# pauxy-qmc/pauxy

Measured on AMD Instinct MI355X. Metric: walker_steps_per_sec, higher is better.
Workload: dtype f64; 1 GPU; generic Cholesky AFQMC: Nbasis=100, Nchol=500, RHF trial 25+25 electrons, 256 walkers/GPU, dt=0.005, reortho/10, comb/5, energy/10 (BASELINE configs[2]); walkers_total=256, rng=device-philox, population_control=device comb (one rank)

## Files before the change

### pauxy_amd/csrc/afq_api.hip

```cpp
#include <algorithm>
#include <cmath>
#include <complex>
#include <cstdio>
#include <cstdlib>
#include <cstring>
#include "afq_internal.h"

namespace {

template <class T> int dev_alloc(afq_handle *h, T **p, size_t n) {
    if (*p) { hipFree(*p); *p = nullptr; }
    if (n == 0) return AFQ_OK;
    hipError_t e = hipMalloc((void **)p, n * sizeof(T));
    if (e != hipSuccess) { h->err = std::string("hipMalloc: ") + hipGetErrorString(e); return AFQ_ENOMEM; }
    return AFQ_OK;
}

template <class T> int dev_upload(afq_handle *h, T **p, const void *src, size_t n) {
    int rc = dev_alloc(h, p, n);
    if (rc) return rc;
    if (n) AFQ_HIP(h, hipMemcpy(*p, src, n * sizeof(T), hipMemcpyHostToDevice));
    return AFQ_OK;
}

// ... 573 lines not shown
            for (double &v : pt) v = -v;
            if ((rc = dev_upload(h, &h->msd_psicT_neg, pt.data(), kkp * M))) return rc;
        }
    }
    return AFQ_OK;
}

int afq_set_propagator(afq_handle *h, const double *BH1, const double *mf_shift, double dt, int exp_order,
                       int flags) {
    if (h) { h->greens_valid = false; h->gsum_only = false; }
    if (!h || !BH1 || !mf_shift || dt <= 0 || exp_order < 0) return AFQ_EINVAL;
    if (!h->kind) AFQ_FAIL(h, AFQ_ESTATE, "set the system before the propagator");
    hipSetDevice(h->device);
    int rc;
    if ((rc = dev_upload(h, &h->BH1, BH1, (size_t)2 * h->M * h->M))) return rc;
    h->bh1_real = true;
    h->bh1_same = memcmp(BH1, BH1 + (size_t)2 * h->M * h->M, sizeof(double) * 2 * h->M * h->M) == 0;
    for (size_t i = 0, n = (size_t)2 * h->M * h->M; i < n && h->bh1_real; ++i) h->bh1_real = BH1[2 * i + 1] == 0.0;
    if ((rc = dev_upload(h, &h->mf_shift, mf_shift, (size_t)h->K))) return rc;
    if (h->kind == AFQ_SYS_UEG && (rc = k_ueg_fast_propagator(h, BH1))) return rc;
    h->dt = dt; h->sqrt_dt = std::pow(dt, 0.5); h->exp_order = exp_order;
    if (flags & AFQ_PROP_FREE_PROJECTION) flags &= ~AFQ_PROP_FORCE_BIAS;
    const int old_nv = h->nv; const bool old_diag = h->vhs_diag;
    h->flags = flags;
    h->vhs_diag = h->kind == AFQ_SYS_HUBBARD;
    h->nv = (h->kind == AFQ_SYS_HUBBARD && (flags & AFQ_PROP_HUBBARD_SPIN)) ? 2 : 1;
    h->have_prop = true;
    if (h->nw && (old_nv != h->nv || old_diag != h->vhs_diag || !h->vhs)) {
        const size_t per = h->vhs_diag ? (size_t)2 * h->nv * h->M : (size_t)h->nv * h->M * h->M;
        if ((rc = dev_alloc(h, &h->vhs, per * h->nw))) return rc;
    }
    return AFQ_OK;
}

int afq_walkers_alloc(afq_handle *h, int nw) {
    if (h) { h->greens_valid = false; h->gsum_only = false; }
    if (!h || nw <= 0) return AFQ_EINVAL;
    if (!h->kind) AFQ_FAIL(h, AFQ_ESTATE, "set the system before allocating walkers");
    hipSetDevice(h->device);
    free_walkers(h);
    const size_t per = (size_t)h->M * h->nt, K = h->K, n = nw;
    int rc;
#define A_(ptr, cnt) if ((rc = dev_alloc(h, &(ptr), (cnt)))) return rc;
    A_(h->phi, per * n) A_(h->phi_t, per * n) A_(h->phi_t2, per * n)
    A_(h->weight, n) A_(h->unscaled, n) A_(h->detR, n) A_(h->log_detR, n)
    A_(h->ot, n) A_(h->ehyb, n) A_(h->phase, n) A_(h->eloc, n)
    A_(h->ghalf_all, per * n * h->ndet) A_(h->ovlp_old, n) A_(h->ovlp_new, n)
    h->ghalf = h->ghalf_all + (size_t)h->cur_det * n * per;
    if (h->ndet > 1) { A_(h->detd, n * h->ndet) A_(h->detd_a, n * h->ndet) A_(h->detw, n * h->ndet) A_(h->energy_all, 3 * n * h->ndet) }
    A_(h->xi, K * n) A_(h->xbar, K * n) A_(h->xs, K * n) A_(h->cmf, n) A_(h->cfb, n)
    A_(h->energy, 3 * n) A_(h->alive, n) A_(h->parent_ix, n)
    h->fb_split = 1;
    if (h->kind == AFQ_SYS_GENERIC) {
        const long tiles = (long)((nw + 31) / 32) * ((h->K + 31) / 32) * 2;
        int sp = (int)std::max(1L, std::min(8L, 1024 / std::max(1L, tiles)));
        if (nw > 32) {
            const long wgt = (long)((nw + 63) / 64) * ((h->K + 63) / 64) * 2;
            sp = (int)std::max(1L, std::min(16L, (512 + wgt - 1) / wgt));
        }
        if (h->rchol_same && h->rchol_real && h->ndet == 1 && h->na == h->nb && nw > 32 && sp > 1) sp = (sp + 1) / 2;
        const int nmax = std::max(h->na, h->nb) * h->M;
        while (sp > 1 && nmax / sp < 64) --sp;
        h->fb_split = sp;
        A_(h->vbias_all, (size_t)2 * sp * n * K * h->ndet)
        h->vbias = h->vbias_all + (size_t)h->cur_det * 2 * sp * n * K;
    } else if (h->kind == AFQ_SYS_UEG) {
        A_(h->vbias_all, n * K)
        h->vbias = h->vbias_all;
    }
    if (h->kind == AFQ_SYS_UEG) A_(h->G, (size_t)2 * h->M * h->M * n)
    {
        const size_t pv = h->kind == AFQ_SYS_HUBBARD ? (size_t)4 * h->M : (size_t)h->M * h->M;
        A_(h->vhs, pv * n)
    }
#undef A_
    AFQ_HIP(h, hipMalloc(&h->pack_tmp, std::max((size_t)nw * 2 * sizeof(int), (size_t)4096)));
    h->nw = nw;
    h->cap_frac = 0.0; h->cap_total = -1.0;
    {
        double sc0[AFQ_NSCAL] = {0};
        sc0[0] = (double)nw * k_comm_size(h);
        AFQ_HIP(h, hipMemcpy(h->scal, sc0, sizeof(sc0), hipMemcpyHostToDevice));
    }
    std::vector<double> one(nw, 1.0), zero2(2 * (size_t)nw, 0.0), one2(2 * (size_t)nw, 0.0);
    for (int i = 0; i < nw; ++i) one2[2 * i] = 1.0;
    AFQ_HIP(h, hipMemcpy(h->weight, one.data(), sizeof(double) * nw, hipMemcpyHostToDevice));
    AFQ_HIP(h, hipMemcpy(h->unscaled, one.data(), sizeof(double) * nw, hipMemcpyHostToDevice));
    AFQ_HIP(h, hipMemcpy(h->detR, one.data(), sizeof(double) * nw, hipMemcpyHostToDevice));
    AFQ_HIP(h, hipMemset(h->log_detR, 0, sizeof(double) * nw));
    AFQ_HIP(h, hipMemcpy(h->ot, one2.data(), sizeof(cplx) * nw, hipMemcpyHostToDevice));
    AFQ_HIP(h, hipMemcpy(h->phase, one2.data(), sizeof(cplx) * nw, hipMemcpyHostToDevice));
    AFQ_HIP(h, hipMemcpy(h->ehyb, zero2.data(), sizeof(cplx) * nw, hipMemcpyHostToDevice));
    AFQ_HIP(h, hipMemcpy(h->eloc, zero2.data(), sizeof(cplx) * nw, hipMemcpyHostToDevice));
    AFQ_HIP(h, hipMemset(h->phi, 0, sizeof(cplx) * per * n));
    AFQ_HIP(h, hipMemset(h->ghalf, 0, sizeof(cplx) * per * n));
    AFQ_HIP(h, hipMemset(h->energy, 0, sizeof(cplx) * 3 * n));
    AFQ_HIP(h, hipMemset(h->xi, 0, sizeof(double) * K * n));
    return AFQ_OK;
}

static int field_info(afq_handle *h, int field, void **base, size_t *bytes) {
    const size_t per = (size_t)h->M * h->nt;
    switch (field) {
    case AFQ_F_PHI: *base = h->phi; *bytes = per * sizeof(cplx); break;
    case AFQ_F_WEIGHT: *base = h->weight; *bytes = sizeof(double); break;
    case AFQ_F_UNSCALED_WEIGHT: *base = h->unscaled; *bytes = sizeof(double); break;
    case AFQ_F_OT: *base = h->ot; *bytes = sizeof(cplx); break;
    case AFQ_F_HYBRID_ENERGY: *base = h->ehyb; *bytes = sizeof(cplx); break;
    case AFQ_F_PHASE: *base = h->phase; *bytes = sizeof(cplx); break;
    case AFQ_F_DETR: *base = h->detR; *bytes = sizeof(double); break;
    case AFQ_F_ELOC: *base = h->eloc; *bytes = sizeof(cplx); break;
    case AFQ_F_GHALF: *base = h->ghalf; *bytes = per * sizeof(cplx); break;
    case AFQ_F_G: *base = h->G; *bytes = (size_t)2 * h->M * h->M * sizeof(cplx); break;
    case AFQ_F_XBAR: *base = h->xbar; *bytes = (size_t)h->K * sizeof(cplx); break;
    case AFQ_F_XSHIFTED: *base = h->xs; *bytes = (size_t)h->K * sizeof(cplx); break;
    case AFQ_F_ENERGY: *base = h->energy; *bytes = 3 * sizeof(cplx); break;
    case AFQ_F_LOG_DETR: *base = h->log_detR; *bytes = sizeof(double); break;
    default: AFQ_FAIL(h, AFQ_EINVAL, "unknown walker field");
    }
    if (!*base) AFQ_FAIL(h, AFQ_ESTATE, "walker field not allocated (afq_walkers_alloc / afq_greens first)");
    return AFQ_OK;
}

static int ensure_spin_ghalf(afq_handle *h);

int afq_walkers_set(afq_handle *h, int field, const void *host, int first, int count) {
    if (h && (field == AFQ_F_PHI || field == AFQ_F_GHALF)) { h->greens_valid = false; h->gsum_only = false; ++h->ghalf_version; }
    if (!h || !host) return AFQ_EINVAL;
    if (!h->nw) AFQ_FAIL(h, AFQ_ESTATE, "no walkers allocated");
    if (first < 0 || count < 0 || first + count > h->nw) AFQ_FAIL(h, AFQ_EINVAL, "walker range out of bounds");
    hipSetDevice(h->device);
    void *base; size_t bytes;
    int rc = field_info(h, field, &base, &bytes);
    if (rc) return rc;
    AFQ_HIP(h, hipMemcpyAsync((char *)base + bytes * first, host, bytes * count, hipMemcpyHostToDevice, h->stream));
    AFQ_HIP(h, hipStreamSynchronize(h->stream));
    return AFQ_OK;
}

int afq_walkers_get(afq_handle *h, int field, void *host, int first, int count) {
    if (!h || !host) return AFQ_EINVAL;
    if (!h->nw) AFQ_FAIL(h, AFQ_ESTATE, "no walkers allocated");
    if (first < 0 || count < 0 || first + count > h->nw) AFQ_FAIL(h, AFQ_EINVAL, "walker range out of bounds");
    hipSetDevice(h->device);
    void *base; size_t bytes;
    int rc = field_info(h, field, &base, &bytes);
    if (rc) return rc;
    if (field == AFQ_F_GHALF && (rc = ensure_spin_ghalf(h))) return rc;
    AFQ_HIP(h, hipMemcpyAsync(host, (char *)base + bytes * first, bytes * count, hipMemcpyDeviceToHost, h->stream));
    AFQ_HIP(h, hipStreamSynchronize(h->stream));
    return AFQ_OK;
}

int afq_walkers_device_ptr(afq_handle *h, int field, void **dev_ptr, int64_t *bytes_per_walker) {
    if (!h || !dev_ptr) return AFQ_EINVAL;
    void *base; size_t bytes;
    int rc = field_info(h, field, &base, &bytes);
    if (rc) return rc;
    if (field == AFQ_F_GHALF && h->gsum_only) {
        hipSetDevice(h->device);
        if ((rc = ensure_spin_ghalf(h))) return rc;
    }
    h->greens_valid = false; h->gsum_only = false; h->greens_cache = false;
    *dev_ptr = base;
    if (bytes_per_walker) *bytes_per_walker = (int64_t)bytes;
    return AFQ_OK;
}

static int greens_any(afq_handle *h, cplx *det_out, bool with_ghalf);

static int need_ready(afq_handle *h, bool prop) {
    if (!h->kind || !h->have_trial || !h->nw) AFQ_FAIL(h, AFQ_ESTATE, "system, trial and walkers must be set");
    if (prop && !h->have_prop) AFQ_FAIL(h, AFQ_ESTATE, "propagator not set");
    if (h->prop_pending) AFQ_FAIL(h, AFQ_ESTATE, "a step is half done: afq_propagate_finish first");
    hipSetDevice(h->device);
    return AFQ_OK;
}

static int ensure_spin_ghalf(afq_handle *h) {
    if (!h->gsum_only) return AFQ_OK;
    h->gsum_only = false;
    const int rc = greens_any(h, h->ovlp_new, true);
    h->greens_valid = rc == AFQ_OK;
    return rc;
}

static int ensure_G(afq_handle *h) {
    if (!h->G) {
        int rc = dev_alloc(h, &h->G, (size_t)2 * h->M * h->M * h->nw);
        if (rc) return rc;
    }
    return AFQ_OK;
}

static int copy_out(afq_handle *h, void *host, const void *dev, size_t bytes) {
    if (!host) return AFQ_OK;
    AFQ_HIP(h, hipMemcpyAsync(host, dev, bytes, hipMemcpyDeviceToHost, h->stream));
    AFQ_HIP(h, hipStreamSynchronize(h->stream));
    return AFQ_OK;
}

int afq_greens(afq_handle *h, int want_G, double *ovlp_out) {
    AFQ_API(h, "afq_greens");
    if (h) { h->greens_valid = false; h->gsum_only = false; }
    if (!h) return AFQ_EINVAL;
    int rc = need_ready(h, false);
    if (rc) return rc;
    {
        PhaseTimer t(h, T_GREENS);
        if ((rc = greens_any(h, h->ovlp_old, true))) return rc;
        if (want_G || h->kind == AFQ_SYS_UEG) {
            if ((rc = ensure_G(h))) return rc;
            if ((rc = k_full_G(h))) return rc;
        }
    }
    return copy_out(h, ovlp_out, h->ovlp_old, sizeof(cplx) * h->nw);
}

int afq_inverse_overlap(afq_handle *h, double *oinv_out, double *ovlp_out) {
    if (h) { h->greens_valid = false; h->gsum_only = false; }
    if (!h || !oinv_out) return AFQ_EINVAL;
    int rc = need_ready(h, false);
    if (rc) return rc;
    if (h->ndet > 1) AFQ_FAIL(h, AFQ_EUNSUPPORTED, "inverse overlaps: single-determinant trials");
    const size_t nmax = h->na > h->nb ? h->na : h->nb, n = (size_t)h->nw * 2 * nmax * nmax;
    cplx *tmp = nullptr;
    if ((rc = dev_alloc(h, &tmp, n))) return rc;
    AFQ_HIP(h, hipMemsetAsync(tmp, 0, sizeof(cplx) * n, h->stream));
    if ((rc = k_alive(h))) { dev_free(tmp); return rc; }
    std::vector<int> ones(h->nw, 1);
    AFQ_HIP(h, hipMemcpyAsync(h->alive, ones.data(), sizeof(int) * h->nw, hipMemcpyHostToDevice, h->stream));
    rc = k_inverse_overlap(h, tmp, h->ovlp_new);
    if (!rc) rc = copy_out(h, oinv_out, tmp, sizeof(cplx) * n);
    if (!rc && ovlp_out) rc = copy_out(h, ovlp_out, h->ovlp_new, sizeof(cplx) * h->nw);
    dev_free(tmp);
    if (!rc) rc = k_alive(h);
    return rc;
}

int afq_calc_overlap(afq_handle *h, double *ovlp_out) {
    AFQ_API(h, "afq_calc_overlap");
    if (h) { h->greens_valid = false; h->gsum_only = false; }
    if (!h) return AFQ_EINVAL;
    int rc = need_ready(h, false);
    if (rc) return rc;
    {
        PhaseTimer t(h, T_OVLP);
        if ((rc = greens_any(h, h->ovlp_new, false))) return rc;
    }
    return copy_out(h, ovlp_out, h->ovlp_new, sizeof(cplx) * h->nw);
}

static int greens_any(afq_handle *h, cplx *det_out, bool with_ghalf) {
    int rc;
    if (h->ndet <= 1) return with_ghalf ? k_greens(h, det_out) : k_overlap(h, det_out);
    for (int d = 0; d < h->ndet; ++d) {
        select_det(h, d);
        cplx *dd = h->detd + (size_t)d * h->nw;
        h->det_a_out = with_ghalf ? h->detd_a + (size_t)d * h->nw : nullptr;
        rc = with_ghalf ? k_greens(h, dd) : k_overlap(h, dd);
        h->det_a_out = nullptr;
        if (rc) { select_det(h, 0); return rc; }
    }
    select_det(h, 0);
    return k_msd_combine(h, det_out, with_ghalf);
}

static int force_bias(afq_handle *h, bool with_xbar = true) {
    int rc;
    if (h->flags & AFQ_PROP_FORCE_BIAS) {
        if (h->kind == AFQ_SYS_GENERIC) {
            h->msd_fb_gbar = false;
            if (k_msd_gbar_wanted(h) && !(h->msd_fb_mode == 0 && k_msd_vbias_current(h))) {
                if ((rc = k_force_bias_msd_gbar(h))) return rc;
                h->msd_fb_gbar = true;
            } else {
                for (int d = 0; d < h->ndet; ++d) {
                    select_det(h, d);
                    if ((rc = k_force_bias_generic(h))) { select_det(h, 0); return rc; }
                }
                select_det(h, 0);
            }
        }
        else if (h->kind == AFQ_SYS_UEG) { if ((rc = k_vbias_ueg(h))) return rc; }
    }
    return with_xbar ? k_xbar(h) : AFQ_OK;
}

static int build_vhs(afq_handle *h) {
    if (h->kind == AFQ_SYS_GENERIC) return k_vhs_generic(h);
    if (h->kind == AFQ_SYS_HUBBARD) return k_vhs_hubbard(h);
    return k_vhs_ueg(h);
}

static int local_energy(afq_handle *h);
static int local_energy_dets(afq_handle *h);

static int apply_exp(afq_handle *h, const cplx *vhs) {
    if (h->vhs_diag) return k_apply_exponential_diag(h, vhs);
    return k_apply_exponential(h, vhs);
}

int afq_propagate(afq_handle *h, const double *xi, double eshift_re, double eshift_im) {
    const int rc = afq_propagate_begin(h, xi);
    return rc ? rc : afq_propagate_finish(h, eshift_re, eshift_im);
}

int afq_propagate_begin(afq_handle *h, const double *xi) {
    AFQ_API(h, "afq_propagate");
    if (!h) return AFQ_EINVAL;
    int rc = need_ready(h, true);
    if (rc) return rc;
    if (h->hirsch) AFQ_FAIL(h, AFQ_ESTATE, "discrete Hirsch propagator set: use afq_propagate_hirsch");
    const bool hubbard_fused = h->vhs_diag;
    const bool hubbard_fused_fields = hubbard_fused && h->K == h->M;
    if (xi) {
        if ((rc = k_alive(h))) return rc;
        AFQ_HIP(h, hipMemcpyAsync(h->xi, xi, sizeof(double) * (size_t)h->nw * h->K, hipMemcpyHostToDevice, h->stream));
    } else if (k_prop_fused_supported(h) || k_ueg_fast_supported(h) || hubbard_fused_fields) {
        h->rng_inline = true;
        h->rng_inline_counter = h->rng_counter++;
    } else {
        if ((rc = k_rng_normal(h))) return rc;
    }
    const bool fp = (h->flags & AFQ_PROP_FREE_PROJECTION) != 0;
    if (!fp || (h->flags & AFQ_PROP_FORCE_BIAS)) {
        PhaseTimer t(h, T_GREENS);
        const bool sum_ok = h->gsum_only && (h->flags & AFQ_PROP_HYBRID) && !h->rdm_on &&
                            (h->kind == AFQ_SYS_GENERIC ||
                             (h->kind == AFQ_SYS_HUBBARD && h->gdiag && h->gdiag_version == h->ghalf_version));
        if (h->greens_valid || sum_ok) std::swap(h->ovlp_old, h->ovlp_new);
        else if ((rc = greens_any(h, h->ovlp_old, true))) return rc;
        h->greens_valid = false; h->gsum_only = false;
        const bool le = !fp && !(h->flags & AFQ_PROP_HYBRID);
        if ((h->kind == AFQ_SYS_UEG && ((h->flags & AFQ_PROP_FORCE_BIAS) || le) && !k_ueg_fast_supported(h)) ||
            (h->rdm_on && h->ndet == 1)) {
            if ((rc = ensure_G(h))) return rc;
            if ((rc = k_full_G(h))) return rc;
        }
        if (le) {
            PhaseTimer te(h, T_ENERGY);
            if (h->ndet > 1) { if ((rc = local_energy_dets(h))) return rc; }
            else if ((rc = local_energy(h))) return rc;
        }
    }
    if (k_ueg_fast_supported(h)) {
        { PhaseTimer t(h, T_EXP); if ((rc = k_ueg_step(h))) return rc; }
        h->prop_pending = true;
        return AFQ_OK;
    }
    if (hubbard_fused) {
        cplx *fac = h->vhs + (size_t)h->nw * h->nv * h->M;
        const bool fields_make_factors = hubbard_fused_fields;
        {
            PhaseTimer t(h, T_FB);
            if ((rc = force_bias(h, false))) return rc;
            if ((rc = k_xbar_fields(h, fields_make_factors ? fac : nullptr))) return rc;
        }
        if (!fields_make_factors) {
            { PhaseTimer t(h, T_VHS); if ((rc = build_vhs(h))) return rc; }
            { PhaseTimer t(h, T_EXP); if ((rc = k_exp_diag_factors(h, h->vhs, fac))) return rc; }
        }
        if (h->rng_inline) AFQ_FAIL(h, AFQ_ESTATE, "internal: the inline field draw of this step was not consumed by the field kernel");
        { PhaseTimer t(h, T_ONEBODY); if ((rc = k_onebody(h, fac))) return rc; }
        { PhaseTimer t(h, T_ONEBODY); if ((rc = k_onebody(h))) return rc; }
        h->prop_pending = true;
        return AFQ_OK;
    }
    const bool fused = k_prop_fused_supported(h);
    h->closed_large = !fused && h->kind == AFQ_SYS_GENERIC && h->nv == 1 && h->bh1_same && h->na == h->nb && h->na > 0 &&
                      h->M > 128 && h->nt > 32 && h->nw >= 64;
    struct ClosedLargeOff { afq_handle *h; ~ClosedLargeOff() { h->closed_large = false; } } closed_large_off{h};
    if (h->closed_large && (rc = k_closed_flags(h))) return rc;
    if (!fused) { PhaseTimer t(h, T_ONEBODY); if ((rc = k_onebody(h))) return rc; }
    {
        PhaseTimer t(h, T_FB);
        if ((rc = force_bias(h, false))) return rc;
        if ((rc = k_xbar_fields(h))) return rc;
    }
    h->vhs_upper = fused && h->hs_sym;
    { PhaseTimer t(h, T_VHS); rc = build_vhs(h); }
    if (rc) { h->vhs_upper = false; return rc; }
    if (fused) {
        PhaseTimer t(h, T_EXP);
        rc = k_prop_fused(h);
        h->vhs_upper = false;
        if (rc) return rc;
    } else {
        { PhaseTimer t(h, T_EXP); if ((rc = apply_exp(h, h->vhs))) return rc; }
        { PhaseTimer t(h, T_ONEBODY); if ((rc = k_onebody(h))) return rc; }
        if (h->closed_large && (rc = k_closed_copy_beta(h))) return rc;
    }
    h->prop_pending = true;
    return AFQ_OK;
}

int afq_propagate_finish(afq_handle *h, double eshift_re, double eshift_im) {
    AFQ_API(h, "afq_propagate");
    if (!h) return AFQ_EINVAL;
    if (!h->prop_pending) AFQ_FAIL(h, AFQ_ESTATE, "afq_propagate_finish without afq_propagate_begin");
    hipSetDevice(h->device);
    h->prop_pending = false;
    int rc;
    const bool fp = (h->flags & AFQ_PROP_FREE_PROJECTION) != 0;
    {
        PhaseTimer t(h, T_OVLP);
        const bool le_msd = h->ndet > 1 && !fp && !(h->flags & AFQ_PROP_HYBRID);
        h->fuse_weight_done = false;
        h->fuse_weight_req = h->ndet == 1 && !le_msd;
        h->fuse_eshift = cmake(eshift_re, eshift_im);
        if (h->greens_cache && !fp) {
            const bool fb_sum = h->kind == AFQ_SYS_GENERIC && k_fb_use_sum(h);
            const bool fb_diag = h->kind == AFQ_SYS_HUBBARD && !h->hirsch && h->psicT && k_greens_big_supported(h);
            h->ghalf_skip_store = h->fuse_est_req && h->ndet == 1 && (fb_sum || fb_diag) &&
                                  (h->flags & AFQ_PROP_HYBRID) && (h->flags & AFQ_PROP_FORCE_BIAS) && !h->rdm_on &&
                                  h->nbp == 0 && h->psi_stride == 0;
            h->ghalf_skipped = false;
            rc = greens_any(h, h->ovlp_new, true);
            h->fuse_weight_req = false;
            h->ghalf_skip_store = false;
            if (rc) return rc;
            h->greens_valid = !h->ghalf_skipped;
            h->gsum_only = h->ghalf_skipped;
        } else {
            rc = greens_any(h, h->ovlp_new, false);
            h->fuse_weight_req = false;
            if (rc) return rc;
        }
        if (h->ndet > 1 && !fp && !(h->flags & AFQ_PROP_HYBRID)) {
            if ((rc = k_msd_energy_combine(h))) return rc;
        }
        if ((rc = k_update_weight(h, cmake(eshift_re, eshift_im)))) return rc;
        if (h->nbp > 0 && !fp && (rc = k_bp_push(h))) return rc;
    }
    if (h->fuse_est_req) {
        h->fuse_est_req = false;
        h->est_acc_pending = true;
    }
    return AFQ_OK;
}

int afq_estimates_fuse_next(afq_handle *h) {
    if (!h) return AFQ_EINVAL;
    if (!h->nw) AFQ_FAIL(h, AFQ_ESTATE, "no walkers");
    if (h->rdm_on) AFQ_FAIL(h, AFQ_EUNSUPPORTED, "afq_estimates_fuse_next with the one-body RDM accumulation on");
    if (h->hirsch) AFQ_FAIL(h, AFQ_EUNSUPPORTED, "afq_estimates_fuse_next: continuous propagator only");
    hipSetDevice(h->device);
    if (!h->est_acc) {
        int rc = dev_alloc(h, &h->est_acc, (size_t)6 * h->nw);
        if (rc) return rc;
        AFQ_HIP(h, hipMemsetAsync(h->est_acc, 0, sizeof(double) * 6 * h->nw, h->stream));
    }
    h->fuse_est_req = true;
    return AFQ_OK;
}

int afq_set_log_shift(afq_handle *h, int on, double log_shift, double detR_shift) {
    AFQ_API(h, "afq_set_log_shift");
    if (!h) return AFQ_EINVAL;
    if (on && h->ndet > 1) AFQ_FAIL(h, AFQ_EUNSUPPORTED, "use_log_shift: single-determinant walkers only");
    h->log_shift_on = on != 0;
    h->log_shift = on ? log_shift : 0.0;
    h->detR_shift = on ? detR_shift : 0.0;
    return AFQ_OK;
}

int afq_log_ovlp_sums(afq_handle *h, double *sums3) {
    AFQ_API(h, "afq_log_ovlp_sums");
    if (!h || !sums3) return AFQ_EINVAL;
    int rc = need_ready(h, false);
    if (rc) return rc;
    return k_log_ovlp_sums(h, sums3);
}

int afq_reortho(afq_handle *h, double *detR_out) {
    AFQ_API(h, "afq_reortho");
    if (!h) return AFQ_EINVAL;
    int rc = need_ready(h, false);
    if (rc) { h->greens_valid = false; h->gsum_only = false; return rc; }
    const bool keep = (h->greens_valid || h->gsum_only) && h->ndet == 1;
    const bool sum_only = h->gsum_only;
    h->greens_valid = false; h->gsum_only = false;
    bool scaled = false;
    { PhaseTimer t(h, T_QR); if ((rc = k_reortho(h, keep ? h->ovlp_new : nullptr, &scaled))) return rc; }
    if (keep) {
        if (!scaled && (rc = k_scale_by_inverse(h, h->ovlp_new, h->detR))) return rc;
        h->greens_valid = !sum_only; h->gsum_only = sum_only;
    }
    if (h->log_shift_on && (rc = k_log_shift_reortho(h))) return rc;
    return copy_out(h, detR_out, h->detR, sizeof(double) * h->nw);
}

static int local_energy_dets(afq_handle *h) {
    cplx *final_e = h->energy;
    int rc = AFQ_OK;
    for (int d = 0; d < h->ndet && !rc; ++d) {
        select_det(h, d);
        h->energy = h->energy_all + (size_t)d * 3 * h->nw;
        rc = k_energy_generic(h);
    }
    h->energy = final_e;
    select_det(h, 0);
    return rc;
}

static int local_energy(afq_handle *h) {
    if (h->kind == AFQ_SYS_GENERIC && h->ndet > 1) {
        int rc = local_energy_dets(h);
        if (rc) return rc;
        return k_msd_energy_combine(h);
    }
    if (h->kind == AFQ_SYS_GENERIC) return k_energy_generic(h);
    if (h->kind == AFQ_SYS_HUBBARD) return k_energy_hubbard(h);
    if (!h->G) AFQ_FAIL(h, AFQ_ESTATE, "afq_greens must run before afq_local_energy");
    return k_energy_ueg(h);
}

int afq_local_energy(afq_handle *h, double *E_out) {
    AFQ_API(h, "afq_local_energy");
    if (!h) return AFQ_EINVAL;
    int rc = need_ready(h, false);
    if (rc) return rc;
    if (!h->rH1 && h->kind != AFQ_SYS_UEG) AFQ_FAIL(h, AFQ_ESTATE, "half-rotated H1 missing (set trial)");
    if ((rc = ensure_spin_ghalf(h))) return rc;
    { PhaseTimer t(h, T_ENERGY); if ((rc = local_energy(h))) return rc; }
    return copy_out(h, E_out, h->energy, sizeof(cplx) * 3 * h->nw);
}

int afq_set_exchange_algorithm(afq_handle *h, int mode) {
    if (!h || mode < 0 || mode > 2) return AFQ_EINVAL;
    h->exx_mode = mode;
    return AFQ_OK;
}

int afq_set_msd_force_bias(afq_handle *h, int mode) {
    if (!h || mode < 0 || mode > 2) return AFQ_EINVAL;
    h->msd_fb_mode = mode;
    return AFQ_OK;
}

int afq_msd_force_bias(afq_handle *h, int *mode) {
    if (!h || !mode) return AFQ_EINVAL;
    if (h->kind != AFQ_SYS_GENERIC || !h->have_trial || !h->nw) AFQ_FAIL(h, AFQ_ESTATE, "generic system, trial and walkers must be set");
    *mode = h->ndet <= 1 ? 0 : k_msd_gbar_wanted(h) ? 2 : 1;
    return AFQ_OK;
}

int afq_exchange_algorithm(afq_handle *h, int *mode) {
    if (!h || !mode) return AFQ_EINVAL;
    if (h->kind != AFQ_SYS_GENERIC || !h->have_trial) AFQ_FAIL(h, AFQ_ESTATE, "generic system and trial must be set");
    *mode = k_exchange_uses_quadratic(h) ? 2 : 1;
    return AFQ_OK;
}

int afq_force_bias(afq_handle *h, double *xbar_out) {
    if (!h) return AFQ_EINVAL;
    int rc = need_ready(h, true);
    if (rc) return rc;
    if ((rc = force_bias(h))) return rc;
    return copy_out(h, xbar_out, h->xbar, sizeof(cplx) * (size_t)h->nw * h->K);
}

int afq_shift_fields(afq_handle *h, const double *xi, const double *xbar, double *xs_out, double *cmf_out,
                     double *cfb_out) {
    if (!h || !xi || !xbar) return AFQ_EINVAL;
    int rc = need_ready(h, true);
    if (rc) return rc;
    const size_t n = (size_t)h->nw * h->K;
    AFQ_HIP(h, hipMemcpyAsync(h->xi, xi, sizeof(double) * n, hipMemcpyHostToDevice, h->stream));
    AFQ_HIP(h, hipMemcpyAsync(h->xbar, xbar, sizeof(cplx) * n, hipMemcpyHostToDevice, h->stream));
    if ((rc = k_fields_explicit(h, h->xi, h->xbar, h->xs, h->cmf, h->cfb))) return rc;
    if ((rc = copy_out(h, xs_out, h->xs, sizeof(cplx) * n))) return rc;
    if ((rc = copy_out(h, cmf_out, h->cmf, sizeof(cplx) * h->nw))) return rc;
    return copy_out(h, cfb_out, h->cfb, sizeof(cplx) * h->nw);
}

int afq_vhs_count(afq_handle *h, int *nv) {
    if (!h || !nv) return AFQ_EINVAL;
    *nv = h->nv;
    return AFQ_OK;
}

int afq_vhs(afq_handle *h, const double *xs, double *vhs_out) {
    if (!h || !xs || !vhs_out) return AFQ_EINVAL;
    int rc = need_ready(h, true);
    if (rc) return rc;
    const size_t n = (size_t)h->nw * h->K;
    AFQ_HIP(h, hipMemcpyAsync(h->xs, xs, sizeof(cplx) * n, hipMemcpyHostToDevice, h->stream));
    if ((rc = build_vhs(h))) return rc;
    const size_t mm = (size_t)h->M * h->M;
    if (!h->vhs_diag) return copy_out(h, vhs_out, h->vhs, sizeof(cplx) * mm * h->nv * h->nw);
    std::vector<double> d((size_t)2 * h->nw * h->nv * h->M);
    if ((rc = copy_out(h, d.data(), h->vhs, sizeof(cplx) * (size_t)h->nw * h->nv * h->M))) return rc;
    std::memset(vhs_out, 0, sizeof(cplx) * mm * h->nv * h->nw);
    for (size_t b = 0; b < (size_t)h->nw * h->nv; ++b)
        for (int p = 0; p < h->M; ++p) {
            vhs_out[2 * (b * mm + (size_t)p * h->M + p)] = d[2 * (b * h->M + p)];
            vhs_out[2 * (b * mm + (size_t)p * h->M + p) + 1] = d[2 * (b * h->M + p) + 1];
        }
    return AFQ_OK;
}

int afq_apply_exponential(afq_handle *h, const double *vhs) {
    if (h) { h->greens_valid = false; h->gsum_only = false; }
    if (!h || !vhs) return AFQ_EINVAL;
    int rc = need_ready(h, true);
    if (rc) return rc;
    if ((rc = k_alive(h))) return rc;
    const size_t mm = (size_t)h->M * h->M;
    if (!h->vhs_diag) {
        AFQ_HIP(h, hipMemcpyAsync(h->vhs, vhs, sizeof(cplx) * mm * h->nv * h->nw, hipMemcpyHostToDevice, h->stream));
    } else {
        std::vector<double> d((size_t)2 * h->nw * h->nv * h->M);
        for (size_t b = 0; b < (size_t)h->nw * h->nv; ++b)
            for (int p = 0; p < h->M; ++p) {
                d[2 * (b * h->M + p)] = vhs[2 * (b * mm + (size_t)p * h->M + p)];
                d[2 * (b * h->M + p) + 1] = vhs[2 * (b * mm + (size_t)p * h->M + p) + 1];
            }
        AFQ_HIP(h, hipMemcpy(h->vhs, d.data(), sizeof(double) * d.size(), hipMemcpyHostToDevice));
    }
    if ((rc = apply_exp(h, h->vhs))) return rc;
    return afq_sync(h);
}

int afq_kinetic(afq_handle *h) {
    if (h) { h->greens_valid = false; h->gsum_only = false; }
    if (!h) return AFQ_EINVAL;
    int rc = need_ready(h, true);
    if (rc) return rc;
    if ((rc = k_alive(h))) return rc;
    if ((rc = k_onebody(h))) return rc;
    return afq_sync(h);
}

int afq_set_weight_cap(afq_handle *h, double frac, double total_weight) {
    if (!h) return AFQ_EINVAL;
    h->cap_frac = frac > 0.0 ? frac : 0.0;
    h->cap_total = total_weight;
    return AFQ_OK;
}

int afq_cap_weights(afq_handle *h, double frac, double total_weight) {
    if (!h) return AFQ_EINVAL;
    int rc = need_ready(h, false);
    if (rc) return rc;
    return k_cap_weights(h, frac, total_weight);
}

int afq_popcontrol_comb(afq_handle *h, double r, double target_weight, int32_t *parent_ix,
                        double *total_weight_out) {
    if (h) h->scal_cache_valid = false;
    AFQ_API(h, "afq_popcontrol_comb");
    if (!h) return AFQ_EINVAL;
    int rc = need_ready(h, false);
    if (rc) { h->greens_valid = false; h->gsum_only = false; return rc; }
    const int nranks = k_comm_size(h);
    if (h->nw * nranks == 1) return AFQ_OK;
    const bool keep = h->greens_valid && h->ndet == 1;
    h->greens_valid = false; h->gsum_only = false;
    if ((rc = k_comb(h, r, target_weight, keep))) return rc;
    h->greens_valid = keep; h->gsum_only = false;
    if (!parent_ix && !total_weight_out) return AFQ_OK;
    double sc[8];
    if ((rc = copy_out(h, sc, h->scal, sizeof(sc)))) return rc;
    if (total_weight_out) *total_weight_out = sc[0];
    if (sc[1] < 0) AFQ_FAIL(h, AFQ_EWEIGHT, "total walker weight below 1e-8");
    if (sc[3] != 0.0) AFQ_FAIL(h, AFQ_EOVERFLOW, "more walkers moved between two ranks than the exchange slots hold");
    if (sc[6] != 0.0) AFQ_FAIL(h, AFQ_ECOMM, "communicator: a peer rank never signalled (the wait budget of afq_comm_set_timeout ran out on the device)");
    if (!parent_ix) return AFQ_OK;
    if (h->comm) return afq_comm_parent_ix(h, parent_ix);
    return copy_out(h, parent_ix, h->parent_ix, sizeof(int) * h->nw);
}

int afq_walkers_scale_weights(afq_handle *h, double scale) {
    if (!h || scale == 0.0) return AFQ_EINVAL;
    int rc = need_ready(h, false);
    if (rc) return rc;
    return k_scale_weights(h, scale);
}

int afq_walkers_reset_weights(afq_handle *h) {
    if (!h) return AFQ_EINVAL;
    int rc = need_ready(h, false);
    if (rc) return rc;
    return k_reset_weights(h);
}
// ... 889 lines not shown
```

### pauxy_amd/csrc/afq_internal.h

```cpp
#pragma once
#include <hip/hip_runtime.h>
#include <stdint.h>
#include <cstdlib>
#include <string>
#include <vector>
#include "../../include/afqmc_hip.h"

typedef double2 cplx;

__host__ __device__ inline cplx cmake(double r, double i) { return make_double2(r, i); }
__host__ __device__ inline cplx cadd(cplx a, cplx b) { return cmake(a.x + b.x, a.y + b.y); }
__host__ __device__ inline cplx csub(cplx a, cplx b) { return cmake(a.x - b.x, a.y - b.y); }
__host__ __device__ inline cplx cmul(cplx a, cplx b) {
    return cmake(a.x * b.x - a.y * b.y, a.x * b.y + a.y * b.x);
}
__host__ __device__ inline cplx cconj(cplx a) { return cmake(a.x, -a.y); }
__host__ __device__ inline cplx cscale(cplx a, double s) { return cmake(a.x * s, a.y * s); }
__host__ __device__ inline void cfma(cplx &a, cplx b, cplx c) {
    a.x = fma(b.x, c.x, a.x); a.x = fma(-b.y, c.y, a.x);
    a.y = fma(b.x, c.y, a.y); a.y = fma(b.y, c.x, a.y);
}
__host__ __device__ inline double cabs2(cplx a) { return a.x * a.x + a.y * a.y; }
__device__ inline cplx cdiv(cplx a, cplx b) {
    if (fabs(b.x) >= fabs(b.y)) {
        double r = b.y / b.x, d = b.x + b.y * r;
        return cmake((a.x + a.y * r) / d, (a.y - a.x * r) / d);
    } else {
        double r = b.x / b.y, d = b.x * r + b.y;
        return cmake((a.x * r + a.y) / d, (a.y * r - a.x) / d);
    }
}

#define AFQ_NSCAL 12
enum { AFQ_HS_HERMITIAN = 1, AFQ_HS_GENERAL = 2 };
enum { T_GREENS = 0, T_ONEBODY, T_FB, T_VHS, T_EXP, T_OVLP, T_QR, T_ENERGY, T_COUNT };

#define AFQ_NCOUNTERS 8

struct afq_handle {
    int device = 0;
    hipStream_t stream = nullptr;
    std::string err;

    int kind = 0;
    int M = 0, K = 0, na = 0, nb = 0, nt = 0;
    double ecore = 0.0;
    double *hs_pot = nullptr;
    bool hs_sym = false;
    double *L_full = nullptr;
    int2 *hs_pair = nullptr;
    int hs_cplx = 0;
    double *hs_pot_im = nullptr;
    int2 *hs_pair_im = nullptr;
    long ld_hs_im = 0;
    cplx *L_full_c = nullptr;
    long ld_hs = 0, ld_rc = 0;
    bool rchol_real = true;
    double *rchol_re = nullptr;
    double *rchol_im = nullptr;
    double *rchol_frag[2] = {nullptr, nullptr};
    double *rchol_frag_im[2] = {nullptr, nullptr};
    void *atil[2] = {nullptr, nullptr};
    bool atil_unavailable = false;
    bool rchol_same = false;
    int exx_mode = 0;
    cplx *exq_y = nullptr;
    size_t exq_y_len = 0;
    cplx *H1 = nullptr;
    cplx *rH1 = nullptr;
    double U = 0.0;
    int nq = 0;
    int64_t nnzA = 0, nnzB = 0;
    int64_t *iA_colptr = nullptr, *iA_row = nullptr; cplx *iA_val = nullptr;
    int64_t *iB_colptr = nullptr, *iB_row = nullptr; cplx *iB_val = nullptr;
    int64_t *iA_rowptr = nullptr, *iA_col = nullptr; cplx *iA_rval = nullptr;
    int64_t *iB_rowptr = nullptr, *iB_col = nullptr; cplx *iB_rval = nullptr;
    int ell_len = 0; int *ell_row = nullptr; cplx *ell_val = nullptr;
    int ueg_nrows = 0; int *ueg_rmap = nullptr; int *ueg_rows = nullptr;
    int *ueg_kp = nullptr, *ueg_pm = nullptr, *ueg_koff = nullptr, *ueg_poff = nullptr;
    int64_t *kpq_off = nullptr, *kpq_i = nullptr, *kpq_kpq = nullptr;
    int64_t *pmq_off = nullptr, *pmq_i = nullptr, *pmq_pmq = nullptr;
    double *vqvec = nullptr; double vol = 1.0; double *H1diag = nullptr;
    void *ueg_fast = nullptr;

    bool have_trial = false;
    cplx *psi = nullptr;
    cplx *psic = nullptr;
    cplx *psicT = nullptr;
    long psi_stride = 0;
    bool psi_real = false;
    bool psi_closed = false;
    unsigned long long *closed_bad = nullptr;
    unsigned long long closed_epoch = 0, closed_checked_version = 0;
    unsigned long long closed_epoch_pub = 0;
    bool exx_open_hint = false;
    int *closed_w = nullptr;
    int closed_w_n = 0;
    bool closed_large = false;

    struct DetOps {
        cplx *psi = nullptr, *psic = nullptr, *rH1 = nullptr;
        double *rchol_re = nullptr, *rchol_im = nullptr;
        double *rchol_frag[2] = {nullptr, nullptr}, *rchol_frag_im[2] = {nullptr, nullptr};
        void *atil[2] = {nullptr, nullptr};
        bool rchol_same = false;
        unsigned long long vbias_version = 0;
    };
    int ndet = 1, cur_det = 0;
    std::vector<DetOps> dets;
    cplx *coeffs = nullptr;
    cplx *detd = nullptr;
    cplx *detd_a = nullptr;
    cplx *det_a_out = nullptr;
    cplx *detw = nullptr;
    cplx *ghalf_all = nullptr;
    cplx *vbias_all = nullptr;
    cplx *energy_all = nullptr;
    int msd_fb_mode = 0;
    bool msd_fb_gbar = false;
    cplx *msd_psicT = nullptr;
    cplx *msd_gs = nullptr;
    cplx *msd_S = nullptr;
    double *hs_pk = nullptr;
    cplx *msd_psicT_neg = nullptr;
    cplx *msd_D = nullptr;
    double *hs_pk_im = nullptr;

    int nbp = 0;
    cplx *bp_hist = nullptr;
    int *bp_n = nullptr;
    int *bp_flag = nullptr;
    double *bp_cos = nullptr;
    cplx *bp_ph = nullptr;
    cplx *phi_old = nullptr;
    cplx *phi_bp = nullptr;
    cplx *BH1dag = nullptr;
    cplx *bp_xs = nullptr;
    cplx *bp_est = nullptr;
    int bpo_two = 0, bpo_ekt = 0;
    int bpo_nL = 0;
    cplx *bpo_h1 = nullptr;
    cplx *bpo_L = nullptr;
    cplx *bpo_wt = nullptr;
    cplx *bpo_out = nullptr;
    cplx *bpo_ws = nullptr;
    size_t bpo_ws_len = 0;
    int bpo_nc = 0, bpo_ncy = 0;
    int it_nmax = 0, it_neqlb = 0, it_stable = 1, it_restore = 0;
    cplx *it_ws = nullptr;
    size_t it_ws_len = 0;

    bool hirsch = false;
    cplx hs_delta[2][2];
    cplx hs_wfac[2];
    cplx hs_auxf[2][2];
    cplx hs_gamma;
    bool hs_charge = false;
    bool hs_direct = false;
    double *hs_fbfac = nullptr;
    cplx *hs_oinv = nullptr;
    double *hs_u = nullptr;
    int *hs_fields = nullptr;
    int *hs_used = nullptr;
    int *hs_alive0 = nullptr;

    bool have_prop = false;
    cplx *BH1 = nullptr;
    double cap_frac = 0.0, cap_total = -1.0;
    bool vhs_upper = false;
    bool bh1_same = false;
    bool bh1_real = false;
    cplx *mf_shift = nullptr;
    double dt = 0.0, sqrt_dt = 0.0;
    int exp_order = 6;
    int flags = AFQ_PROP_HYBRID | AFQ_PROP_FORCE_BIAS;
    int nv = 1;
    bool vhs_diag = false;

    int nw = 0;
    cplx *phi = nullptr;
    cplx *phi_t = nullptr;
    cplx *phi_t2 = nullptr;
    double *weight = nullptr, *unscaled = nullptr, *detR = nullptr;
    double *log_detR = nullptr;
    bool log_shift_on = false;
    double log_shift = 0.0, detR_shift = 0.0;
    cplx *ot = nullptr, *ehyb = nullptr, *phase = nullptr, *eloc = nullptr;
    cplx *ghalf = nullptr;
    cplx *G = nullptr;
    cplx *ovlp_old = nullptr, *ovlp_new = nullptr;
    double *xi = nullptr;
    int fb_split = 1;
    cplx *vbias = nullptr;
    cplx *ghalf_sum = nullptr;
    unsigned long long ghalf_version = 1, gsum_version = 0;
    unsigned long long vbias_version = 0;
    cplx *gdiag = nullptr;
    int gdiag_parts = 0;
    unsigned long long gdiag_version = 0;
    cplx *xbar = nullptr, *xs = nullptr;
    cplx *cmf = nullptr, *cfb = nullptr;
    cplx *vhs = nullptr;
    cplx *lu_ws = nullptr;
    cplx *big_ws = nullptr;
    cplx *big_ws2 = nullptr;
    cplx *detm = nullptr;
    int *dete = nullptr;
    double *qr_logd = nullptr;
    int *qr_fail = nullptr;
    cplx *energy = nullptr;
    cplx *exx_part = nullptr;
    int64_t exx_part_len = 0;
    double *gfrag = nullptr;
    size_t gfrag_bytes = 0;
    bool prop_pending = false;
    double *est_stage = nullptr;
    unsigned long long est_seq = 0;
    double scal_cache[AFQ_NSCAL] = {0};
    bool scal_cache_valid = false;
    bool est_pending = false;
    unsigned ktrace_mask = 0;
    std::vector<hipEvent_t> ktrace_ev[AFQ_K_COUNT];
    double issued_flops[AFQ_K_COUNT] = {0, 0, 0, 0, 0};
    double prop_issued_open = 0.0, prop_issued_closed = 0.0;
    int ktrace_used[AFQ_K_COUNT] = {0, 0, 0, 0, 0};
    int ktrace_stride[AFQ_K_COUNT] = {1, 1, 1, 1, 1}, ktrace_seen[AFQ_K_COUNT] = {0, 0, 0, 0, 0};
    bool ltrace_on = false, ltrace_open = false;
    std::vector<hipEvent_t> ltrace_ev;
    std::vector<const char *> ltrace_name;
    int *gj_flag = nullptr;
    cplx *estimates = nullptr;
    bool rdm_on = false;
    double *rdm_acc = nullptr;
    unsigned long long *counters = nullptr;
    int *alive = nullptr;
    int *parent_ix = nullptr;
    double *scal = nullptr;
    void *pack_tmp = nullptr;
    void *zero_page = nullptr;
    bool greens_valid = false;
    bool greens_cache = true;

    bool fuse_weight_req = false, fuse_weight_done = false;
    double *est_acc = nullptr;
    bool fuse_est_req = false, est_acc_pending = false;
    bool gsum_only = false, ghalf_skip_store = false, ghalf_skipped = false;
    cplx fuse_eshift;

    uint64_t rng_seed = 0, rng_stream = 0, rng_counter = 0;
    bool rng_inline = false;
    uint64_t rng_inline_counter = 0;

    const char *crumb_name[64] = {nullptr};
    const char *crumb_api = "";
    volatile unsigned long long n_launch = 0;
    bool debug_sync = false;
    bool debug_markers = false;
    volatile unsigned long long *retired = nullptr;

    void *comm = nullptr;

    bool timers_on = false;
    double t_ms[T_COUNT] = {0};
    hipEvent_t ev0 = nullptr, ev1 = nullptr;
    double last_energy_ms = 0.0;
};

#define AFQ_HIP(h, call)                                                        \
    do {                                                                        \
        hipError_t e_ = (call);                                                 \
        if (e_ != hipSuccess) {                                                 \
            (h)->err = std::string(#call) + ": " + hipGetErrorString(e_);       \
            return AFQ_EHIP;                                                    \
        }                                                                       \
    } while (0)

void afq_launch_trace_mark(afq_handle *h, const char *name);
inline void afq_note_launch(afq_handle *h, const char *name) {
    h->crumb_name[h->n_launch & 63] = name;
    h->n_launch = h->n_launch + 1;
    if (h->ltrace_on) afq_launch_trace_mark(h, name);
}
hipError_t afq_post_launch(afq_handle *h);
#define AFQ_LAUNCH(h, kern, ...) do { afq_note_launch((h), #kern); hipLaunchKernelGGL(kern, __VA_ARGS__); } while (0)
#define AFQ_POST(h)                                                              \
    do {                                                                        \
        hipError_t e_ = afq_post_launch(h);                                     \
        if (e_ != hipSuccess) {                                                 \
            (h)->err = std::string("kernel ") + (h)->crumb_name[((h)->n_launch - 1) & 63] + ": " + hipGetErrorString(e_); \
            return AFQ_EHIP;                                                    \
        }                                                                       \
    } while (0)
#define AFQ_GEMM(h, call) AFQ_GEMM_AS(h, __func__, call)
#define AFQ_GEMM_AS(h, name, call)                                              \
    do {                                                                        \
        afq_note_launch((h), name);                                             \
        hipError_t e_ = (call);                                                 \
        if (e_ == hipSuccess) e_ = afq_post_launch(h);                          \
        if (e_ != hipSuccess) {                                                 \
            (h)->err = std::string("GEMM of ") + __func__ + ": " + hipGetErrorString(e_); \
            return AFQ_EHIP;                                                    \
        }                                                                       \
    } while (0)

#define AFQ_MAX_DEVICES 16
inline hipError_t afq_raise_lds(const void *kern, size_t lds, size_t (&set)[AFQ_MAX_DEVICES]) {
    int d = 0;
    if (hipGetDevice(&d) != hipSuccess || d < 0 || d >= AFQ_MAX_DEVICES) d = -1;
    if (d >= 0 && lds <= set[d]) return hipSuccess;
    hipError_t e = hipFuncSetAttribute(kern, hipFuncAttributeMaxDynamicSharedMemorySize, (int)lds);
    if (e == hipSuccess && d >= 0) set[d] = lds;
    return e;
}

#define AFQ_FAIL(h, code, msg) do { (h)->err = (msg); return (code); } while (0)

struct PhaseTimer {
    afq_handle *h; int slot;
    PhaseTimer(afq_handle *h_, int s) : h(h_), slot(s) {
        if (h->timers_on) hipEventRecord(h->ev0, h->stream);
    }
    ~PhaseTimer() {
        if (h->timers_on) {
            hipEventRecord(h->ev1, h->stream);
            hipEventSynchronize(h->ev1);
            float ms = 0; hipEventElapsedTime(&ms, h->ev0, h->ev1);
            h->t_ms[slot] += ms;
        }
    }
};

struct KernelTrace {
    afq_handle *h; int kind, idx;
    KernelTrace(afq_handle *h_, int k) : h(h_), kind(k), idx(-1) {
        if (!(h->ktrace_mask >> k & 1) || h->ktrace_used[k] >= 4096) return;
        if (h->ktrace_seen[k]++ % h->ktrace_stride[k]) return;
        idx = h->ktrace_used[k];
        std::vector<hipEvent_t> &ev = h->ktrace_ev[k];
        while ((int)ev.size() < 2 * idx + 2) { hipEvent_t e; hipEventCreate(&e); ev.push_back(e); }
        hipEventRecord(ev[2 * idx], h->stream);
    }
    ~KernelTrace() {
        if (idx < 0) return;
        hipEventRecord(h->ktrace_ev[kind][2 * idx + 1], h->stream);
        h->ktrace_used[kind] = idx + 1;
    }
};

int k_onebody(afq_handle *h, const cplx *rowscale = nullptr);
int k_force_bias_generic(afq_handle *h);
bool k_msd_vbias_current(afq_handle *h);
bool k_msd_gbar_wanted(afq_handle *h);
int k_force_bias_msd_gbar(afq_handle *h);
bool k_fb_use_sum(afq_handle *h);
int k_vhs_generic(afq_handle *h);
int k_apply_exponential(afq_handle *h, const cplx *vhs);
int k_full_G(afq_handle *h);
int k_prop_fused_supported(afq_handle *h);
int k_prop_fused(afq_handle *h);
int k_hirsch_alive(afq_handle *h, int mode);
int k_hirsch_kinetic(afq_handle *h);
int k_hirsch_two_body(afq_handle *h);
int k_hirsch_eshift(afq_handle *h, double fac);
int k_hirsch_free(afq_handle *h, double eshift);
int k_rng_uniform(afq_handle *h, double *u, long n);
int k_energy_full_g(afq_handle *h, const cplx *G_dev, int ng, cplx *E_dev);
int k_fullg_expand(afq_handle *h);
int k_bp_observables(afq_handle *h, int restore, cplx *two_out, cplx *fock_out);
int k_itcf_fields(afq_handle *h, cplx *xs, int t);
int k_itcf_generic_b(afq_handle *h, const cplx *vhs, const cplx *BT2, const cplx *BT2inv, cplx *B, cplx *Binv, cplx *ws,
                     cplx *detm, int *dete);
int k_itcf_hirsch_b(afq_handle *h, int t, const cplx *BT2, const cplx *BT2inv, cplx *B, cplx *Binv, double *f);
int k_itcf_mul(afq_handle *h, const cplx *A, const cplx *B, cplx *C);
int k_itcf_propagate(afq_handle *h, const cplx *B, const cplx *src, cplx *dst);
int k_itcf_projectors(afq_handle *h, const cplx *G, cplx *P, cplx *Q);
int k_itcf_weights(afq_handle *h, int restore, cplx *wfac, cplx *denom);
int k_itcf_accumulate(afq_handle *h, const cplx *Ggr, const cplx *Gls, const cplx *wfac, cplx *spgf_tau);
int k_greens_big_supported(afq_handle *h);
struct WeightArgs;
int k_greens_big(afq_handle *h, cplx *ghalf, cplx *det, cplx *oinv = nullptr, const WeightArgs *wa = nullptr);
int k_reortho_big(afq_handle *h);
int k_gj_inverse(afq_handle *h, cplx *O, int n, int batch, cplx *detm, int *dete);
int k_alive(afq_handle *h);
int k_greens(afq_handle *h, cplx *det_out);
int k_overlap(afq_handle *h, cplx *det_out);
int k_inverse_overlap(afq_handle *h, cplx *oinv, cplx *det_out);
int k_fields(afq_handle *h);
int k_fields_explicit(afq_handle *h, const double *xi_d, const cplx *xbar_d, cplx *xs_d, cplx *cmf_d, cplx *cfb_d);
int k_xbar(afq_handle *h);
int k_bp_push(afq_handle *h);
int k_bp_fields(afq_handle *h, int i);
int k_bp_init(afq_handle *h, const cplx *phi0_dev);
int k_conj_copy(afq_handle *h, const cplx *src, cplx *dst, long n);
int k_conj_transpose(afq_handle *h, const cplx *A, cplx *At);
int k_bp_accumulate(afq_handle *h, int restore, int with_energy);
int k_bp_reset(afq_handle *h, bool first);
int k_bp_hirsch_step(afq_handle *h, int i);
int k_xbar_fields(afq_handle *h, cplx *hubbard_factors = nullptr);
int k_msd_combine(afq_handle *h, cplx *det_out, bool skip_small);
int k_msd_energy_combine(afq_handle *h);
int k_update_weight(afq_handle *h, cplx eshift);
int k_reortho(afq_handle *h, cplx *keep = nullptr, bool *keep_done = nullptr);
int k_cap_weights(afq_handle *h, double frac, double total_weight);
int k_comb(afq_handle *h, double r, double target, bool with_greens = false);
int k_clone_pairs(afq_handle *h, bool with_greens, bool reset_weights = false);
int k_closed_flags(afq_handle *h);
int k_closed_copy_beta(afq_handle *h);
int k_scale_by_inverse(afq_handle *h, cplx *x, const double *d);
int k_log_shift_reortho(afq_handle *h);
int k_log_ovlp_sums(afq_handle *h, double *out3);
int k_scale_weights(afq_handle *h, double scale);
int k_reset_weights(afq_handle *h, bool after_comb = false);
struct EstPublish {
    double *host_out = nullptr;
    unsigned long long *host_seq = nullptr;
    unsigned long long seq = 0;
    const double *scal = nullptr;
    const unsigned long long *closed_bad = nullptr;
    int nest = 0, zero = 0;
};
int k_estimates(afq_handle *h, int have_energy, bool fold_only = false, const EstPublish *pub = nullptr);
int k_rdm_accumulate(afq_handle *h);
int k_rng_normal(afq_handle *h);
int k_rng_normal_into(afq_handle *h, double *out_d, long n);
int k_philox_raw(afq_handle *h, const unsigned int *in_d, unsigned int *out_d, int n);
int k_ueg_fast_system(afq_handle *h, int M, int nq, const int64_t *Acp, const int64_t *Arow, const double *Aval,
                      const int64_t *Bcp, const int64_t *Brow, const double *Bval);
int k_ueg_fast_trial(afq_handle *h, const double *psi);
int k_ueg_fast_propagator(afq_handle *h, const double *BH1);
int k_ueg_fast_supported(afq_handle *h);
int k_ueg_fields(afq_handle *h);
int k_prop_ueg(afq_handle *h);
int k_ueg_step(afq_handle *h);
void k_ueg_fast_free(afq_handle *h);
int k_comm_size(afq_handle *h);
void k_comm_destroy(afq_handle *h);
int k_comm_popcontrol(afq_handle *h, double r, double target, bool with_greens);
int k_energy_generic(afq_handle *h);
int k_prepare_energy_operands(afq_handle *h, const double *rchol_host);
int k_exchange_uses_quadratic(afq_handle *h);
void k_free_atil(void *(&atil)[2]);
int k_vhs_hubbard(afq_handle *h);
int k_apply_exponential_diag(afq_handle *h, const cplx *vhs_diag);
int k_exp_diag_factors(afq_handle *h, const cplx *vhs_diag, cplx *out);
int k_energy_hubbard(afq_handle *h);
int k_vbias_ueg(afq_handle *h);
int k_vhs_ueg(afq_handle *h);
int k_energy_ueg(afq_handle *h);
```

### pauxy_amd/csrc/k_fused.hip

```cpp
#include <cstdlib>
#include <type_traits>

#include "mfma_gemm_wg.h"

#define PF_D 3
#ifndef PF_NW
#define PF_NW 8
#endif
#define PF_NT (64 * PF_NW)
#ifndef PF_LW
#define PF_LW PF_NW
#endif
#define PF_FPW (16 / PF_LW)

struct PropFusedArgs {
    int M, na, nb, nt, order;
    int vhs_upper;
    int same_b;
    int b_real;
    int rem4;
    int hyb;
    int symcols;
    int closed_try;
    int contig;
    const cplx *BH1;
    const cplx *vhs;
    cplx *phi;
    const int *alive;
    const void *zero16;
    unsigned long long *n_closed;
};

__device__ inline d2_t lds_read_c(unsigned addr) { return lds_read_b128(addr); }

template <int OFF> __device__ inline d2_t lds_read_off(unsigned addr) {
    d2_t v;
    asm volatile("ds_read_b128 %0, %1 offset:%2" : "=v"(v) : "v"(addr), "n"(OFF));
    return v;
}
__device__ __attribute__((always_inline)) inline d2_t lds_read_frag(unsigned base, int idx) {
    switch (idx) {
    case 0: return lds_read_off<0>(base);
    case 1: return lds_read_off<1024>(base);
    case 2: return lds_read_off<2048>(base);
    case 3: return lds_read_off<3072>(base);
    case 4: return lds_read_off<4096>(base);
    case 5: return lds_read_off<5120>(base);
    case 6: return lds_read_off<6144>(base);
    default: return lds_read_off<7168>(base);
    }
}

template <int OFF> __device__ inline double lds_read_re_off(unsigned addr) {
    double v;
    asm volatile("ds_read_b64 %0, %1 offset:%2" : "=v"(v) : "v"(addr), "n"(OFF));
    return v;
}
__device__ __attribute__((always_inline)) inline double lds_read_frag_re(unsigned base, int idx) {
    switch (idx) {
    case 0: return lds_read_re_off<0>(base);
    case 1: return lds_read_re_off<1024>(base);
    case 2: return lds_read_re_off<2048>(base);
    case 3: return lds_read_re_off<3072>(base);
    case 4: return lds_read_re_off<4096>(base);
    case 5: return lds_read_re_off<5120>(base);
    case 6: return lds_read_re_off<6144>(base);
    default: return lds_read_re_off<7168>(base);
    }
}

__device__ inline void lds_barrier() {
    asm volatile("s_waitcnt lgkmcnt(0)" ::: "memory");
    __builtin_amdgcn_s_barrier();
    asm volatile("" ::: "memory");
}

template <bool NARROW, int FULL>
__global__ __launch_bounds__(PF_NT) void prop_fused_kernel(PropFusedArgs a) {
    extern __shared__ __align__(16) unsigned char smem[];
    const int w = blockIdx.x;
    if (!a.alive[w]) return;
    const int tid = threadIdx.x, lane = tid & 63, wave = __builtin_amdgcn_readfirstlane(tid >> 6);
    const int lr = lane & 15, lk = lane >> 4;
    const int M = a.M, nt = a.nt;
    const int NCH = (M + 7) >> 3;
    const int nrt = (M + 15) >> 4;
    unsigned char *Tf = smem;
    unsigned char *ring = smem + (size_t)NCH * 8192;
    const unsigned tf_l = lds_addr(Tf), ring_l = lds_addr(ring);
    cplx *phi = a.phi + (long)w * M * nt;
    const cplx *vhs = a.vhs + (long)w * M * M;

    const int nob = a.same_b ? 1 : 2;
    const int nphase = 2 * nob + a.order;
    const int G = nphase * NCH;
    const long MM = (long)M * M;
    int gi = 0, gi_phase = 0, gi_c = 0, gi_slot = 0;
    const void *nsrc[PF_FPW];
    bool prepared = false;
    const bool refills = wave >= PF_NW - PF_LW;
    const int lw = wave - (PF_NW - PF_LW);
    const int p_row0 = (lw >> 1) * 16 + lr;
    const int p_kl = 2 * lk + (lw & 1);
    auto prepare = [&]() __attribute__((always_inline)) {
        if (!refills) { prepared = true; return; }
        const bool in_v = gi_phase >= nob && gi_phase < nob + a.order;
        const int spin = gi_phase < nob ? gi_phase : gi_phase - nob - a.order;
        const cplx *A = in_v ? vhs : a.BH1 + (spin == 1 ? MM : 0L);
        const bool sym_phase = a.vhs_upper && in_v;
        const bool live = gi < G;
        const int k = gi_c * 8 + p_kl;
#pragma unroll
        for (int t = 0; t < PF_FPW; ++t) {
            const int row = p_row0 + t * (PF_LW / 2) * 16;
            const int off = (sym_phase && k < row) ? k * M + row : row * M + k;
            nsrc[t] = (live && row < M && k < M) ? (const void *)(A + off) : a.zero16;
            asm volatile("" : "+v"(nsrc[t]));
        }
        ++gi;
        const bool wrap = gi_c + 1 == NCH;
        gi_c = wrap ? 0 : gi_c + 1;
        gi_phase += wrap ? 1 : 0;
        prepared = true;
    };
    auto issueA = [&]() __attribute__((always_inline)) {
        if (!refills) return;
        if (!prepared) prepare();
        unsigned char *dst = ring + (size_t)gi_slot * 16384;
#pragma unroll
        for (int t = 0; t < PF_FPW; ++t) glds16(nsrc[t], dst + (lw + t * PF_LW) * 1024);
        if (++gi_slot == PF_D) gi_slot = 0;
        prepared = false;
    };
    issueA(); issueA();
    prepare();
    bool closed = false;
    if (a.closed_try) {
        bool same = true;
        for (int p = tid >> 5; p < M; p += PF_NT / 32) {
            const int c = tid & 31;
            if (c < a.na) {
                const cplx x = phi[p * nt + c], y = phi[p * nt + a.na + c];
                same = same && __double_as_longlong(x.x) == __double_as_longlong(y.x) &&
                       __double_as_longlong(x.y) == __double_as_longlong(y.y);
            }
        }
        closed = __builtin_amdgcn_readfirstlane(__syncthreads_and(same ? 1 : 0)) != 0;
        if (closed && tid == 0) atomicAdd(a.n_closed, 1ULL);
    }
    const bool relayout = closed && a.contig;
    const int contig = relayout ? 0 : a.contig, hyb = relayout ? 0 : a.hyb;
    const int sym_n = (a.symcols && !relayout) ? a.na : 0;
    auto wcol = [&](const int c) -> int {
        if (!sym_n) return c;
        if (c < 16) return c;
        if (c < 32) return sym_n + (c - 16);
        if (c < 40) return 16 + (c - 32);
        if (c < 48) return sym_n + 16 + (c - 40);
        const int e = c - 48, extra = sym_n - 24;
        return e < extra ? 24 + e : sym_n + 24 + (e - extra);
    };

    for (int e = tid; e < NCH * 512; e += PF_NT) {
        const int j = e & 15, kk = (e >> 4) & 3, pb = (e >> 6) & 1, slot = (e >> 7) & 3, ch = e >> 9;
        const int p = ch * 8 + 2 * kk + pb, sp = contig ? 0 : slot >> 1, col = (contig ? slot : slot & 1) * 16 + j;
        const int ns_ = contig ? nt : sp ? a.nb : a.na, off_ = sp ? a.na : 0;
        const bool ok = p < M && col < ns_;
        const cplx v = phi[ok ? p * nt + off_ + wcol(col) : 0];
        ((d2_t *)Tf)[e] = ok ? (d2_t){v.x, v.y} : (d2_t){0.0, 0.0};
    }
    __syncthreads();

    auto t_ok = [&](int ti, int r) -> bool { return 2 * ti + (r >> 1) < NCH; };
    const unsigned t_lane = (unsigned)((lk & 1) * 1024 + ((lk >> 1) * 16 + lr) * 16);
    auto t_addr = [&](int ti, int r, int cs) -> unsigned {
        unsigned base = t_lane;
        asm volatile("" : "+v"(base));
        return base + (unsigned)(((2 * ti * 4 + cs) * 2) * 1024) + (unsigned)((r >> 1) * 8192 + (r & 1) * 512);
    };

    int ring_slot = 0;
    auto next_chunk = [&]() __attribute__((always_inline)) -> unsigned {
        asm volatile("s_waitcnt vmcnt(%0)" ::"n"((PF_D - 2) * PF_FPW) : "memory");
        __builtin_amdgcn_s_barrier();
        issueA();
        const unsigned sl = ring_l + ring_slot * 16384;
        if (++ring_slot == PF_D) ring_slot = 0;
        return sl;
    };
    auto next_chunk_sync = [&]() __attribute__((always_inline)) -> unsigned {
        asm volatile("s_waitcnt vmcnt(%0)" ::"n"((PF_D - 2) * PF_FPW) : "memory");
        __builtin_amdgcn_s_barrier();
        const unsigned sl = ring_l + ring_slot * 16384;
        ring_slot = ring_slot + 1 == PF_D ? 0 : ring_slot + 1;
        return sl;
    };

    auto one_body = [&](auto nsl_tag, int slot0, bool to_global, auto real_tag, const int rt) __attribute__((always_inline)) {
        constexpr int NSL = decltype(nsl_tag)::value;
        constexpr bool BR = decltype(real_tag)::value;
        constexpr int SS = (NARROW && FULL) ? 2 : 1;
        d4_t P1[NSL], P2[NSL], P3[NSL];
        bool cv[NSL];
#pragma unroll
        for (int j = 0; j < NSL; ++j) {
            P1[j] = (d4_t){0, 0, 0, 0}; P2[j] = (d4_t){0, 0, 0, 0}; P3[j] = (d4_t){0, 0, 0, 0};
            const int cs = slot0 + j * SS;
            cv[j] = rt < nrt && (cs & 1) < ((((cs >> 1) ? a.nb : a.na) + 15) >> 4);
        }
        auto load_frags = [&](unsigned sl, int c, d2_t (&av)[2], d2_t (&bv)[NSL][2]) {
            const unsigned abase = sl + rt * 2048 + lane * 16;
            const unsigned bbase = tf_l + (c * 4 + slot0) * 2048 + lane * 16;
#pragma unroll
            for (int ss = 0; ss < 2; ++ss) {
                if (BR) av[ss][0] = lds_read_frag_re(abase, ss);
                else av[ss] = lds_read_frag(abase, ss);
#pragma unroll
                for (int j = 0; j < NSL; ++j) bv[j][ss] = lds_read_frag(bbase, j * SS * 2 + ss);
            }
        };
        auto mfmas = [&](d2_t (&av)[2], d2_t (&bv)[NSL][2]) {
            __builtin_amdgcn_sched_barrier(0);
#pragma unroll
            for (int ss = 0; ss < 2; ++ss)
#pragma unroll
                for (int j = 0; j < NSL; ++j)
                    if (FULL || cv[j]) {
                        if (BR) {
                            P1[j] = mfma16(av[ss][0], bv[j][ss][0], P1[j]);
                            P2[j] = mfma16(av[ss][0], bv[j][ss][1], P2[j]);
                        } else {
                            P1[j] = mfma16(av[ss][0], bv[j][ss][0], P1[j]);
                            P2[j] = mfma16(av[ss][1], bv[j][ss][1], P2[j]);
                            P3[j] = mfma16(av[ss][0] + av[ss][1], bv[j][ss][0] + bv[j][ss][1], P3[j]);
                        }
                    }
            __builtin_amdgcn_sched_barrier(0);
            if (!prepared) prepare();
            asm volatile("s_waitcnt lgkmcnt(0)" ::: "memory");
        };
#if PF_NW == 8
        if (FULL) {
            constexpr int NR = 1 + NSL;
            constexpr int RPG = NSL > 1 ? (NR + NSL - 2) / (NSL > 1 ? NSL - 1 : 1) : NR;
            d2_t a0, a1, b0[NSL], b1[NSL];
            auto half = [&](d2_t &ax, d2_t (&bx)[NSL], d2_t &ay, d2_t (&by)[NSL], const unsigned abase, const unsigned bbase,
                            const int ys, const bool fetch, const bool refill) __attribute__((always_inline)) {
                __builtin_amdgcn_sched_barrier(0);
#pragma unroll
                for (int j = 0; j < NSL; ++j) {
                    if (BR) {
                        P1[j] = mfma16(ax[0], bx[j][0], P1[j]);
                        P2[j] = mfma16(ax[0], bx[j][1], P2[j]);
                    } else {
                        P1[j] = mfma16(ax[0], bx[j][0], P1[j]);
                        P2[j] = mfma16(ax[1], bx[j][1], P2[j]);
                        P3[j] = mfma16(ax[0] + ax[1], bx[j][0] + bx[j][1], P3[j]);
                    }
                    __builtin_amdgcn_sched_barrier(0);
                    if (j == 0 && refill) issueA();
                    if (j == 0 && !refill && !prepared) prepare();
                    if (fetch && (j < NSL - 1 || NSL == 1)) {
#pragma unroll
                        for (int q = 0; q < RPG; ++q) {
                            const int r = j * RPG + q;
                            if (r < NR) {
                                if (r == 0) {
                                    if (BR) ay[0] = lds_read_frag_re(abase, ys);
                                    else ay = lds_read_frag(abase, ys);
                                }
                                else by[r - 1] = lds_read_frag(bbase, (r - 1) * SS * 2 + ys);
                            }
                        }
                    }
                    __builtin_amdgcn_sched_barrier(0);
                }
                asm volatile("s_waitcnt lgkmcnt(0)" ::: "memory");
            };
            unsigned sl = next_chunk_sync();
            {
                const unsigned abase = sl + rt * 2048 + lane * 16, bbase = tf_l + slot0 * 2048 + lane * 16;
                if (BR) a0[0] = lds_read_frag_re(abase, 0);
                else a0 = lds_read_frag(abase, 0);
#pragma unroll
                for (int j = 0; j < NSL; ++j) b0[j] = lds_read_frag(bbase, j * SS * 2);
                __builtin_amdgcn_sched_barrier(0);
                issueA();
                asm volatile("s_waitcnt lgkmcnt(0)" ::: "memory");
            }
            for (int c = 0; c < NCH; ++c) {
                const bool more = c + 1 < NCH;
                half(a0, b0, a1, b1, sl + rt * 2048 + lane * 16, tf_l + (c * 4 + slot0) * 2048 + lane * 16, 1, true, false);
                if (more) sl = next_chunk_sync();
                half(a1, b1, a0, b0, sl + rt * 2048 + lane * 16, tf_l + ((c + 1) * 4 + slot0) * 2048 + lane * 16, 0, more, more);
            }
        } else
#endif
        {
#if PF_NW == 16
        d2_t avA[2], bvA[NSL][2];
        for (int c = 0; c < NCH; ++c) {
            load_frags(next_chunk(), c, avA, bvA);
            asm volatile("s_waitcnt lgkmcnt(0)" ::: "memory");
            mfmas(avA, bvA);
        }
#else
        d2_t avA[2], bvA[NSL][2], avB[2], bvB[NSL][2];
        load_frags(next_chunk(), 0, avA, bvA);
        asm volatile("s_waitcnt lgkmcnt(0)" ::: "memory");
        for (int c = 0; c < NCH; c += 2) {
            if (c + 1 < NCH) load_frags(next_chunk(), c + 1, avB, bvB);
            mfmas(avA, bvA);
            if (c + 1 < NCH) {
                if (c + 2 < NCH) load_frags(next_chunk(), c + 2, avA, bvA);
                mfmas(avB, bvB);
            }
        }
#endif
        }
        if (!to_global) __builtin_amdgcn_s_barrier();
        int lk_e = lk, lr_e = lr;
        asm volatile("" : "+v"(lk_e), "+v"(lr_e));
#pragma unroll
        for (int j = 0; j < NSL; ++j)
            if (cv[j]) {
                const int cs = slot0 + j * SS, sp = contig ? 0 : cs >> 1;
                const int ns_ = contig ? nt : sp ? a.nb : a.na, off_ = sp ? a.na : 0;
#pragma unroll
                for (int r = 0; r < 4; ++r) {
                    const double re = BR ? P1[j][r] : P1[j][r] - P2[j][r];
                    const double im = BR ? P2[j][r] : P3[j][r] - P1[j][r] - P2[j][r];
                    if (to_global) {
                        const int row = rt * 16 + lk_e + 4 * r, col = (contig ? cs : cs & 1) * 16 + lr_e;
                        if (row < M && col < ns_) phi[(long)row * nt + off_ + wcol(col)] = cmake(re, im);
                    } else if (t_ok(rt, r)) {
                        *(d2_t *)(Tf + t_addr(rt, r, cs)) = (d2_t){re, im};
                    }
                }
            }
    };
    auto one_body_col = [&](bool to_global, auto real_tag, auto rem_tag) __attribute__((always_inline)) {
        constexpr bool BR = decltype(real_tag)::value;
        constexpr bool REM = decltype(rem_tag)::value;
        constexpr int NI = 3;
        constexpr int NG = NI + (REM ? 1 : 0), NR = NI + 1 + (REM ? 1 : 0), RPG = (NR + NG - 2) / (NG - 1);
        const int c0 = wave & 3, r0 = (wave >> 2) * 3;
        const unsigned rem_t = (unsigned)((((12 * 4 + c0) * 2 + ((lane >> 4) & 1)) * 1024) + (((lane >> 5) * 16) + (lane & 15)) * 16);
        const unsigned rem_a = (unsigned)(6 * 2048 + ((lane >> 4) * 16 + (lane & 3)) * 16);
        d4_t P1[NI], P2[NI], P3[NI];
#pragma unroll
        for (int i = 0; i < NI; ++i) { P1[i] = (d4_t){0, 0, 0, 0}; P2[i] = (d4_t){0, 0, 0, 0}; P3[i] = (d4_t){0, 0, 0, 0}; }
        double Q1 = 0.0, Q2 = 0.0, Q3 = 0.0;
        d2_t a0[NI], a1[NI], b0, b1, q0 = (d2_t){0.0, 0.0}, q1 = (d2_t){0.0, 0.0};
        auto half = [&](d2_t (&ax)[NI], d2_t &bx, d2_t &qx, d2_t (&ay)[NI], d2_t &by, d2_t &qy, const unsigned abase,
                        const unsigned bbase, const unsigned qbase, const int ys, const bool fetch, const bool refill)
            __attribute__((always_inline)) {
            __builtin_amdgcn_sched_barrier(0);
#pragma unroll
            for (int gt = 0; gt < NG; ++gt) {
                if (REM && gt == 0) {
                    if (BR) {
                        Q1 = __builtin_amdgcn_mfma_f64_4x4x4f64(qx[0], bx[0], Q1, 0, 0, 0);
                        Q2 = __builtin_amdgcn_mfma_f64_4x4x4f64(qx[0], bx[1], Q2, 0, 0, 0);
                    } else {
                        Q1 = __builtin_amdgcn_mfma_f64_4x4x4f64(qx[0], bx[0], Q1, 0, 0, 0);
                        Q2 = __builtin_amdgcn_mfma_f64_4x4x4f64(qx[1], bx[1], Q2, 0, 0, 0);
                        Q3 = __builtin_amdgcn_mfma_f64_4x4x4f64(qx[0] + qx[1], bx[0] + bx[1], Q3, 0, 0, 0);
                    }
                } else {
                    const int i = REM ? gt - 1 : gt;
                    if (BR) {
                        P1[i] = mfma16(ax[i][0], bx[0], P1[i]);
                        P2[i] = mfma16(ax[i][0], bx[1], P2[i]);
                    } else {
                        P1[i] = mfma16(ax[i][0], bx[0], P1[i]);
                        P2[i] = mfma16(ax[i][1], bx[1], P2[i]);
                        P3[i] = mfma16(ax[i][0] + ax[i][1], bx[0] + bx[1], P3[i]);
                    }
                }
                __builtin_amdgcn_sched_barrier(0);
                if (gt == 0 && refill) issueA();
                if (gt == 0 && !refill && !prepared) prepare();
                if (fetch && gt < NG - 1) {
#pragma unroll
                    for (int q = 0; q < RPG; ++q) {
                        const int r = gt * RPG + q;
                        if (r < NR) {
                            if (r < NI) {
                                if (BR) ay[r][0] = lds_read_frag_re(abase, r * 2 + ys);
                                else ay[r] = lds_read_frag(abase, r * 2 + ys);
                            } else if (r == NI) {
                                by = lds_read_frag(bbase, ys);
                            } else {
                                if (BR) qy[0] = lds_read_frag_re(qbase, ys);
                                else qy = lds_read_frag(qbase, ys);
                            }
                        }
                    }
                }
                __builtin_amdgcn_sched_barrier(0);
            }
            asm volatile("s_waitcnt lgkmcnt(0)" ::: "memory");
        };
        unsigned sl = next_chunk_sync();
        {
            const unsigned abase = sl + r0 * 2048 + lane * 16, bbase = tf_l + c0 * 2048 + lane * 16;
#pragma unroll
            for (int i = 0; i < NI; ++i) {
                if (BR) a0[i][0] = lds_read_frag_re(abase, i * 2);
                else a0[i] = lds_read_frag(abase, i * 2);
            }
            b0 = lds_read_frag(bbase, 0);
            if (REM) {
                if (BR) q0[0] = lds_read_frag_re(sl + rem_a, 0);
                else q0 = lds_read_frag(sl + rem_a, 0);
            }
            __builtin_amdgcn_sched_barrier(0);
            issueA();
            asm volatile("s_waitcnt lgkmcnt(0)" ::: "memory");
        }
        for (int c = 0; c < NCH; ++c) {
            const bool more = c + 1 < NCH;
            half(a0, b0, q0, a1, b1, q1, sl + r0 * 2048 + lane * 16, tf_l + (c * 4 + c0) * 2048 + lane * 16, sl + rem_a, 1, true, false);
            if (more) sl = next_chunk_sync();
            half(a1, b1, q1, a0, b0, q0, sl + r0 * 2048 + lane * 16, tf_l + ((c + 1) * 4 + c0) * 2048 + lane * 16, sl + rem_a, 0, more, more);
        }
        int lk_e = lk, lr_e = lr, ln_e = lane;
        asm volatile("" : "+v"(lk_e), "+v"(lr_e), "+v"(ln_e));
        const int sp = contig ? 0 : c0 >> 1, ns_ = contig ? nt : sp ? a.nb : a.na, off_ = sp ? a.na : 0;
        const int cb = (contig ? c0 : c0 & 1) * 16;
#pragma unroll
        for (int i = 0; i < NI; ++i)
#pragma unroll
            for (int r = 0; r < 4; ++r) {
                const double re = BR ? P1[i][r] : P1[i][r] - P2[i][r];
                const double im = BR ? P2[i][r] : P3[i][r] - P1[i][r] - P2[i][r];
                if (to_global) {
                    const int row = (r0 + i) * 16 + lk_e + 4 * r, col = cb + lr_e;
                    if (row < M && col < ns_) phi[(long)row * nt + off_ + wcol(col)] = cmake(re, im);
                } else if (t_ok(r0 + i, r)) {
                    *(d2_t *)(Tf + t_addr(r0 + i, r, c0)) = (d2_t){re, im};
                }
            }
        if (!to_global) __builtin_amdgcn_s_barrier();
        if (REM) {
            const double re = BR ? Q1 : Q1 - Q2, im = BR ? Q2 : Q3 - Q1 - Q2;
            if (to_global) {
                const int row = 96 + (ln_e >> 4), col = cb + (ln_e & 15);
                if (row < M && col < ns_) phi[(long)row * nt + off_ + wcol(col)] = cmake(re, im);
            } else {
                *(d2_t *)(Tf + rem_t) = (d2_t){re, im};
            }
        }
    };
    auto one_body_stage = [&](bool to_global) __attribute__((always_inline)) {
        using I2 = std::integral_constant<int, 2>;
#if PF_NW == 8
        if constexpr (FULL == 7) {
            bool col_deal = a.rem4 && a.same_b;
            if (col_deal) {
                if (a.b_real) {
                    if (wave < 4) one_body_col(to_global, std::true_type{}, std::false_type{});
                    else one_body_col(to_global, std::true_type{}, std::true_type{});
                } else {
                    if (wave < 4) one_body_col(to_global, std::false_type{}, std::false_type{});
                    else one_body_col(to_global, std::false_type{}, std::true_type{});
                }
                return;
            }
        }
#endif
#if PF_NW == 16
        using I1 = std::integral_constant<int, 1>;
        const int rt = wave >> 1, h2 = wave & 1;
        if (a.same_b) {
            if (a.b_real) one_body(I2{}, 2 * h2, to_global, std::true_type{}, rt);
            else one_body(I2{}, 2 * h2, to_global, std::false_type{}, rt);
        } else if (a.b_real) {
            one_body(I1{}, h2, to_global, std::true_type{}, rt); one_body(I1{}, 2 + h2, to_global, std::true_type{}, rt);
        } else {
            one_body(I1{}, h2, to_global, std::false_type{}, rt); one_body(I1{}, 2 + h2, to_global, std::false_type{}, rt);
        }
#else
        if (NARROW && FULL) {
            using I1 = std::integral_constant<int, 1>;
            if (a.same_b) {
                if (a.b_real) one_body(I2{}, 0, to_global, std::true_type{}, wave);
                else one_body(I2{}, 0, to_global, std::false_type{}, wave);
            } else if (a.b_real) {
                one_body(I1{}, 0, to_global, std::true_type{}, wave); one_body(I1{}, 2, to_global, std::true_type{}, wave);
            } else {
                one_body(I1{}, 0, to_global, std::false_type{}, wave); one_body(I1{}, 2, to_global, std::false_type{}, wave);
            }
            return;
        }
        using I4 = std::integral_constant<int, 4>;
        if (a.same_b) {
            if (a.b_real) one_body(I4{}, 0, to_global, std::true_type{}, wave);
            else one_body(I4{}, 0, to_global, std::false_type{}, wave);
        } else if (a.b_real) {
            one_body(I2{}, 0, to_global, std::true_type{}, wave); one_body(I2{}, 2, to_global, std::true_type{}, wave);
        } else {
            one_body(I2{}, 0, to_global, std::false_type{}, wave); one_body(I2{}, 2, to_global, std::false_type{}, wave);
        }
#endif
    };

    one_body_stage(false);
    lds_barrier();

    auto taylor = [&](auto ni_tag, auto nj_tag, auto stag_tag, const int r0, const int c0, const int rcount,
                      auto rem_tag) __attribute__((always_inline)) {
        constexpr int NI = decltype(ni_tag)::value, NJ = decltype(nj_tag)::value;
        constexpr bool STAG = decltype(stag_tag)::value;
        constexpr bool REM = decltype(rem_tag)::value;
        static_assert(!REM || (FULL == 7 && NJ == 1), "row-remainder unit: waves 4-7 of the full wide deal");
        const unsigned rem_t = (unsigned)((((12 * 4 + c0) * 2 + ((lane >> 4) & 1)) * 1024) + (((lane >> 5) * 16) + (lane & 15)) * 16);
        const unsigned rem_a = (unsigned)(6 * 2048 + ((lane >> 4) * 16 + (lane & 3)) * 16);
        double RR = 0.0, RI = 0.0;
        if (REM) { const d2_t v = *(const d2_t *)(Tf + rem_t); RR = v[0]; RI = v[1]; }
        bool cv[NJ], rv[NI];
#pragma unroll
        for (int j = 0; j < NJ; ++j) {
            const int cs = c0 + j;
            cv[j] = (cs & 1) < ((((cs >> 1) ? a.nb : a.na) + 15) >> 4);
        }
#pragma unroll
        for (int i = 0; i < NI; ++i) rv[i] = i < rcount && r0 + i < nrt;
        d4_t SR[NI][NJ], SI[NI][NJ];
#pragma unroll
        for (int i = 0; i < NI; ++i)
#pragma unroll
            for (int j = 0; j < NJ; ++j)
#pragma unroll
                for (int r = 0; r < 4; ++r) {
                    d2_t v = (d2_t){0.0, 0.0};
                    if (cv[j] && rv[i] && t_ok(r0 + i, r)) v = *(const d2_t *)(Tf + t_addr(r0 + i, r, c0 + j));
                    SR[i][j][r] = v[0]; SI[i][j][r] = v[1];
                }
        auto load_frags = [&](unsigned sl, int c, d2_t (&av)[NI][2], d2_t (&bv)[NJ][2]) {
            const unsigned abase = sl + r0 * 2048 + lane * 16;
            const unsigned bbase = tf_l + (c * 4 + c0) * 2048 + lane * 16;
#pragma unroll
            for (int ss = 0; ss < 2; ++ss) {
#pragma unroll
                for (int i = 0; i < NI; ++i) av[i][ss] = lds_read_frag(abase, i * 2 + ss);
#pragma unroll
                for (int j = 0; j < NJ; ++j) bv[j][ss] = lds_read_frag(bbase, j * 2 + ss);
            }
        };
        for (int n = 1; n <= a.order; ++n) {
            double inv_n = 1.0 / n;
            asm volatile("" : "+v"(inv_n));
            d4_t P1[NI][NJ], P2[NI][NJ], P3[NI][NJ];
#pragma unroll
            for (int i = 0; i < NI; ++i)
#pragma unroll
                for (int j = 0; j < NJ; ++j) {
                    P1[i][j] = (d4_t){0, 0, 0, 0}; P2[i][j] = (d4_t){0, 0, 0, 0}; P3[i][j] = (d4_t){0, 0, 0, 0};
                }
            double Q1 = 0.0, Q2 = 0.0, Q3 = 0.0;
            auto mfma_ss = [&](d2_t (&av)[NI][2], d2_t (&bv)[NJ][2], const int ss) __attribute__((always_inline)) {
#pragma unroll
                for (int i = 0; i < NI; ++i)
#pragma unroll
                    for (int j = 0; j < NJ; ++j)
                        if (FULL || (cv[j] && rv[i])) {
                            P1[i][j] = mfma16(av[i][ss][0], bv[j][ss][0], P1[i][j]);
                            P2[i][j] = mfma16(av[i][ss][1], bv[j][ss][1], P2[i][j]);
                            P3[i][j] = mfma16(av[i][ss][0] + av[i][ss][1], bv[j][ss][0] + bv[j][ss][1], P3[i][j]);
                        }
            };
            auto mfmas = [&](d2_t (&av)[NI][2], d2_t (&bv)[NJ][2]) {
                __builtin_amdgcn_sched_barrier(0);
                mfma_ss(av, bv, 0);
                mfma_ss(av, bv, 1);
                __builtin_amdgcn_sched_barrier(0);
                if (!prepared) prepare();
                asm volatile("s_waitcnt lgkmcnt(0)" ::: "memory");
            };
#if PF_NW == 8
            if (FULL) {
                constexpr int NG = NI * NJ + (REM ? 1 : 0);
                constexpr int NR = NI + NJ + (REM ? 1 : 0);
                constexpr int RPG = NG > 1 ? (NR + NG - 2) / (NG > 1 ? NG - 1 : 1) : NR;
                d2_t a0[NI], b0[NJ], a1[NI], b1[NJ];
                d2_t q0 = (d2_t){0.0, 0.0}, q1 = (d2_t){0.0, 0.0};
                auto half = [&](d2_t (&ax)[NI], d2_t (&bx)[NJ], d2_t &qx, d2_t (&ay)[NI], d2_t (&by)[NJ], d2_t &qy,
                                const unsigned abase, const unsigned bbase, const unsigned qbase, const int ys,
                                const bool fetch, const bool refill) __attribute__((always_inline)) {
                    __builtin_amdgcn_sched_barrier(0);
#pragma unroll
                    for (int gt = 0; gt < NG; ++gt) {
                        if (REM && gt == 0) {
                            Q1 = __builtin_amdgcn_mfma_f64_4x4x4f64(qx[0], bx[0][0], Q1, 0, 0, 0);
                            Q2 = __builtin_amdgcn_mfma_f64_4x4x4f64(qx[1], bx[0][1], Q2, 0, 0, 0);
                            Q3 = __builtin_amdgcn_mfma_f64_4x4x4f64(qx[0] + qx[1], bx[0][0] + bx[0][1], Q3, 0, 0, 0);
                        }
                        const int g = REM ? (gt == 0 ? 0 : gt - 1) : gt;
                        const int i = g / NJ, j = g % NJ;
                        if (!(REM && gt == 0)) {
                        P1[i][j] = mfma16(ax[i][0], bx[j][0], P1[i][j]);
                        P2[i][j] = mfma16(ax[i][1], bx[j][1], P2[i][j]);
                        P3[i][j] = mfma16(ax[i][0] + ax[i][1], bx[j][0] + bx[j][1], P3[i][j]);
                        }
                        __builtin_amdgcn_sched_barrier(0);
                        if (gt == 0 && refill) issueA();
                        if (gt == 0 && !refill && !prepared) prepare();
                        if (fetch && (gt < NG - 1 || NG == 1)) {
#pragma unroll
                            for (int q = 0; q < RPG; ++q) {
                                const int r = gt * RPG + q;
                                if (r < NR) {
                                    if (r < NI) ay[r] = lds_read_frag(abase, r * 2 + ys);
                                    else if (r < NI + NJ) by[r - NI] = lds_read_frag(bbase, (r - NI) * 2 + ys);
                                    else qy = lds_read_frag(qbase, ys);
                                }
                            }
                        }
                        __builtin_amdgcn_sched_barrier(0);
                    }
                    asm volatile("s_waitcnt lgkmcnt(0)" ::: "memory");
                };
                unsigned sl = next_chunk_sync();
                {
                    const unsigned abase = sl + r0 * 2048 + lane * 16, bbase = tf_l + c0 * 2048 + lane * 16;
#pragma unroll
                    for (int i = 0; i < NI; ++i) a0[i] = lds_read_frag(abase, i * 2);
#pragma unroll
                    for (int j = 0; j < NJ; ++j) b0[j] = lds_read_frag(bbase, j * 2);
                    if (REM) q0 = lds_read_frag(sl + rem_a, 0);
                    __builtin_amdgcn_sched_barrier(0);
                    issueA();
                    asm volatile("s_waitcnt lgkmcnt(0)" ::: "memory");
                }
                for (int c = 0; c < NCH; ++c) {
                    const bool more = c + 1 < NCH;
                    half(a0, b0, q0, a1, b1, q1, sl + r0 * 2048 + lane * 16, tf_l + (c * 4 + c0) * 2048 + lane * 16, sl + rem_a, 1, true, false);
                    if (more) sl = next_chunk_sync();
                    half(a1, b1, q1, a0, b0, q0, sl + r0 * 2048 + lane * 16, tf_l + ((c + 1) * 4 + c0) * 2048 + lane * 16, sl + rem_a, 0, more, more);
                }
            } else
#endif
            {
#if PF_NW == 16
            d2_t avA[NI][2], bvA[NJ][2];
            for (int c = 0; c < NCH; ++c) {
                load_frags(next_chunk(), c, avA, bvA);
                asm volatile("s_waitcnt lgkmcnt(0)" ::: "memory");
                mfmas(avA, bvA);
            }
#else
            d2_t avA[NI][2], bvA[NJ][2], avB[NI][2], bvB[NJ][2];
            if (STAG) {
                auto half = [&](d2_t (&ax)[NI][2], d2_t (&bx)[NJ][2], d2_t (&ay)[NI][2], d2_t (&by)[NJ][2], const int c)
                    __attribute__((always_inline)) {
                    unsigned sl = 0;
                    if (c + 1 < NCH) sl = next_chunk();
                    __builtin_amdgcn_sched_barrier(0);
                    mfma_ss(ax, bx, 1);
                    __builtin_amdgcn_sched_barrier(0);
                    if (!prepared) prepare();
                    if (c + 1 < NCH) {
                        load_frags(sl, c + 1, ay, by);
                        asm volatile("s_waitcnt lgkmcnt(0)" ::: "memory");
                        __builtin_amdgcn_sched_barrier(0);
                        mfma_ss(ay, by, 0);
                        __builtin_amdgcn_sched_barrier(0);
                    }
                };
                load_frags(next_chunk(), 0, avA, bvA);
                asm volatile("s_waitcnt lgkmcnt(0)" ::: "memory");
                __builtin_amdgcn_sched_barrier(0);
                mfma_ss(avA, bvA, 0);
                __builtin_amdgcn_sched_barrier(0);
                for (int c = 0; c < NCH; c += 2) {
                    half(avA, bvA, avB, bvB, c);
                    if (c + 1 < NCH) half(avB, bvB, avA, bvA, c + 1);
                }
            } else {
                load_frags(next_chunk(), 0, avA, bvA);
                asm volatile("s_waitcnt lgkmcnt(0)" ::: "memory");
                for (int c = 0; c < NCH; c += 2) {
                    if (c + 1 < NCH) load_frags(next_chunk(), c + 1, avB, bvB);
                    mfmas(avA, bvA);
                    if (c + 1 < NCH) {
                        if (c + 2 < NCH) load_frags(next_chunk(), c + 2, avA, bvA);
                        mfmas(avB, bvB);
                    }
                }
            }
#endif
            }
            const bool store_first = PF_NW == 8 && FULL != 0 && 2 * (r0 + NI) <= NCH - 1;
            if (!store_first) __builtin_amdgcn_s_barrier();
            const bool last = n == a.order;
#pragma unroll
            for (int i = 0; i < NI; ++i)
#pragma unroll
                for (int j = 0; j < NJ; ++j)
                    if (FULL || (cv[j] && rv[i])) {
#pragma unroll
                        for (int r = 0; r < 4; ++r) {
                            const double re = (P1[i][j][r] - P2[i][j][r]) * inv_n;
                            const double im = (P3[i][j][r] - P1[i][j][r] - P2[i][j][r]) * inv_n;
                            SR[i][j][r] += re; SI[i][j][r] += im;
                            if (!last && t_ok(r0 + i, r)) *(d2_t *)(Tf + t_addr(r0 + i, r, c0 + j)) = (d2_t){re, im};
                        }
                    }
            if (last) {
#pragma unroll
                for (int i = 0; i < NI; ++i)
#pragma unroll
                    for (int j = 0; j < NJ; ++j)
                        if (FULL || (cv[j] && rv[i])) {
#pragma unroll
                            for (int r = 0; r < 4; ++r)
                                if (t_ok(r0 + i, r))
                                    *(d2_t *)(Tf + t_addr(r0 + i, r, c0 + j)) = (d2_t){SR[i][j][r], SI[i][j][r]};
                        }
            }
            if (store_first) __builtin_amdgcn_s_barrier();
            if (REM) {
                const double re = (Q1 - Q2) * inv_n, im = (Q3 - Q1 - Q2) * inv_n;
                RR += re; RI += im;
                *(d2_t *)(Tf + rem_t) = last ? (d2_t){RR, RI} : (d2_t){re, im};
            }
            asm volatile("s_waitcnt lgkmcnt(0)" ::: "memory");
        }
    };

    auto taylor_h = [&](auto hf_tag, auto rem_tag, auto nu_tag, const int r0, const int cf, const int cu, const int cr)
        __attribute__((always_inline)) {
        constexpr bool HF = decltype(hf_tag)::value;
        constexpr bool HR = decltype(rem_tag)::value;
        constexpr int NU = decltype(nu_tag)::value;
        constexpr int NI = 2, NRU = HR ? 2 : 0;
        static_assert(FULL == 7, "hybrid tiling: the full wide deal");
        const unsigned u_rd = (unsigned)((lane >> 4) * 256 + (lane & 3) * 16);
        const int ui = lane >> 4, ub = (lane >> 2) & 3;
        const unsigned u_wr = (unsigned)((ub >> 1) * 8192 + (ui & 1) * 1024 + ((2 * (ub & 1) + (ui >> 1)) * 16 + (lane & 3)) * 16);
        auto u_addr = [&](int ti, int u) -> unsigned {
            unsigned base = u_wr;
            asm volatile("" : "+v"(base));
            return base + (unsigned)((2 * ti * 4 + cu) * 2048 + u * 64);
        };
        const unsigned rem_a = (unsigned)(6 * 2048 + ((lane >> 4) * 16 + (lane & 3)) * 16);
        auto rem_t = [&](int t) -> unsigned {
            return (unsigned)((((12 * 4 + cr + t) * 2 + ((lane >> 4) & 1)) * 1024) + (((lane >> 5) * 16) + (lane & 15)) * 16);
        };
        d4_t SR[NI], SI[NI];
        double UR[NI][NU], UI[NI][NU], RR[2] = {0.0, 0.0}, RI[2] = {0.0, 0.0};
#pragma unroll
        for (int i = 0; i < NI; ++i) {
#pragma unroll
            for (int r = 0; r < 4; ++r) {
                d2_t v = (d2_t){0.0, 0.0};
                if (HF) v = *(const d2_t *)(Tf + t_addr(r0 + i, r, cf));
                SR[i][r] = v[0]; SI[i][r] = v[1];
            }
#pragma unroll
            for (int u = 0; u < NU; ++u) { const d2_t v = *(const d2_t *)(Tf + u_addr(r0 + i, u)); UR[i][u] = v[0]; UI[i][u] = v[1]; }
        }
        if (HR) {
#pragma unroll
            for (int t = 0; t < 2; ++t) { const d2_t v = *(const d2_t *)(Tf + rem_t(t)); RR[t] = v[0]; RI[t] = v[1]; }
        }
        struct Frag { d2_t a[NI]; d2_t bf; d2_t bu[NU]; d2_t q; d2_t br[2]; };
        constexpr int NG = NI * NU + NRU + (HF ? NI : 0);
        constexpr int NR = NI + NU + (HF ? 1 : 0) + (HR ? 3 : 0);
        constexpr int NGAP = HF ? NG - 1 : NG - 3;
        constexpr int RPG = (NR + NGAP - 1) / NGAP;
        for (int n = 1; n <= a.order; ++n) {
            double inv_n = 1.0 / n;
            asm volatile("" : "+v"(inv_n));
            d4_t P1[NI], P2[NI], P3[NI];
            double U1[NI][NU], U2[NI][NU], U3[NI][NU], Q1[2] = {0.0, 0.0}, Q2[2] = {0.0, 0.0}, Q3[2] = {0.0, 0.0};
#pragma unroll
            for (int i = 0; i < NI; ++i) {
                P1[i] = (d4_t){0, 0, 0, 0}; P2[i] = (d4_t){0, 0, 0, 0}; P3[i] = (d4_t){0, 0, 0, 0};
#pragma unroll
                for (int u = 0; u < NU; ++u) { U1[i][u] = 0.0; U2[i][u] = 0.0; U3[i][u] = 0.0; }
            }
            auto read_one = [&](Frag &f, const int r, const unsigned sl, const int c, const int ys) __attribute__((always_inline)) {
                const unsigned abase = sl + r0 * 2048 + lane * 16;
                if (r < NI) { f.a[r] = lds_read_frag(abase, r * 2 + ys); return; }
                if (r < NI + NU) {
                    const int u = r - NI;
                    const unsigned ubase = tf_l + (c * 4 + cu) * 2048 + u_rd + ys * 1024;
                    f.bu[u] = u == 0 ? lds_read_off<0>(ubase) : u == 1 ? lds_read_off<64>(ubase) : lds_read_off<128>(ubase);
                    return;
                }
                int k = r - NI - NU;
                if (HF) {
                    if (k == 0) { f.bf = lds_read_frag(tf_l + (c * 4 + cf) * 2048 + lane * 16, ys); return; }
                    --k;
                }
                if (HR) {
                    if (k == 0) f.q = lds_read_frag(sl + rem_a, ys);
                    else f.br[k - 1] = lds_read_frag(tf_l + (c * 4 + cr + k - 1) * 2048 + lane * 16, ys);
                }
            };
            auto half = [&](Frag &x, Frag &y, const unsigned sl, const int c, const int ys, const bool fetch, const bool refill)
                __attribute__((always_inline)) {
                __builtin_amdgcn_sched_barrier(0);
#pragma unroll
                for (int g = 0; g < NG; ++g) {
                    if (g < NI * NU) {
                        const int i = g / NU, u = g % NU;
                        U1[i][u] = __builtin_amdgcn_mfma_f64_4x4x4f64(x.a[i][0], x.bu[u][0], U1[i][u], 0, 0, 0);
                        U2[i][u] = __builtin_amdgcn_mfma_f64_4x4x4f64(x.a[i][1], x.bu[u][1], U2[i][u], 0, 0, 0);
                        U3[i][u] = __builtin_amdgcn_mfma_f64_4x4x4f64(x.a[i][0] + x.a[i][1], x.bu[u][0] + x.bu[u][1], U3[i][u], 0, 0, 0);
                    } else if (g < NI * NU + NRU) {
                        const int t = g - NI * NU;
                        Q1[t] = __builtin_amdgcn_mfma_f64_4x4x4f64(x.q[0], x.br[t][0], Q1[t], 0, 0, 0);
                        Q2[t] = __builtin_amdgcn_mfma_f64_4x4x4f64(x.q[1], x.br[t][1], Q2[t], 0, 0, 0);
                        Q3[t] = __builtin_amdgcn_mfma_f64_4x4x4f64(x.q[0] + x.q[1], x.br[t][0] + x.br[t][1], Q3[t], 0, 0, 0);
                    } else {
                        const int i = g - NI * NU - NRU;
                        P1[i] = mfma16(x.a[i][0], x.bf[0], P1[i]);
                        P2[i] = mfma16(x.a[i][1], x.bf[1], P2[i]);
                        P3[i] = mfma16(x.a[i][0] + x.a[i][1], x.bf[0] + x.bf[1], P3[i]);
                    }
                    __builtin_amdgcn_sched_barrier(0);
                    if (g == 0 && refill) issueA();
                    if (g == 0 && !refill && !prepared) prepare();
                    if (fetch && g < NGAP) {
#pragma unroll
                        for (int q = 0; q < RPG; ++q)
                            if (g * RPG + q < NR) read_one(y, g * RPG + q, sl, c, ys);
                    }
                    __builtin_amdgcn_sched_barrier(0);
                }
                asm volatile("s_waitcnt lgkmcnt(0)" ::: "memory");
            };
            Frag f0, f1;
            f0.q = (d2_t){0.0, 0.0}; f1.q = (d2_t){0.0, 0.0};
            unsigned sl = next_chunk_sync();
#pragma unroll
            for (int r = 0; r < NR; ++r) read_one(f0, r, sl, 0, 0);
            __builtin_amdgcn_sched_barrier(0);
            issueA();
            asm volatile("s_waitcnt lgkmcnt(0)" ::: "memory");
            for (int c = 0; c < NCH; ++c) {
                const bool more = c + 1 < NCH;
                half(f0, f1, sl, c, 1, true, false);
                if (more) sl = next_chunk_sync();
                half(f1, f0, sl, c + 1, 0, more, more);
            }
            const bool last = n == a.order;
#pragma unroll
            for (int i = 0; i < NI; ++i) {
                if (HF) {
#pragma unroll
                    for (int r = 0; r < 4; ++r) {
                        const double re = (P1[i][r] - P2[i][r]) * inv_n, im = (P3[i][r] - P1[i][r] - P2[i][r]) * inv_n;
                        SR[i][r] += re; SI[i][r] += im;
                        *(d2_t *)(Tf + t_addr(r0 + i, r, cf)) = last ? (d2_t){SR[i][r], SI[i][r]} : (d2_t){re, im};
                    }
                }
#pragma unroll
                for (int u = 0; u < NU; ++u) {
                    const double re = (U1[i][u] - U2[i][u]) * inv_n, im = (U3[i][u] - U1[i][u] - U2[i][u]) * inv_n;
                    UR[i][u] += re; UI[i][u] += im;
                    *(d2_t *)(Tf + u_addr(r0 + i, u)) = last ? (d2_t){UR[i][u], UI[i][u]} : (d2_t){re, im};
                }
            }
            __builtin_amdgcn_s_barrier();
            if (HR) {
#pragma unroll
                for (int t = 0; t < 2; ++t) {
                    const double re = (Q1[t] - Q2[t]) * inv_n, im = (Q3[t] - Q1[t] - Q2[t]) * inv_n;
                    RR[t] += re; RI[t] += im;
                    *(d2_t *)(Tf + rem_t(t)) = last ? (d2_t){RR[t], RI[t]} : (d2_t){re, im};
                }
            }
            asm volatile("s_waitcnt lgkmcnt(0)" ::: "memory");
        }
    };

    auto mirror_spin = [&]() __attribute__((always_inline)) {
        lds_barrier();
        for (int e = tid; e < NCH * 256; e += PF_NT) {
            const int ch = e >> 8, i = e & 255;
            ((d2_t *)Tf)[ch * 512 + 256 + i] = ((const d2_t *)Tf)[ch * 512 + i];
        }
        asm volatile("s_waitcnt lgkmcnt(0)" ::: "memory");
    };
#if PF_NW == 16
    {
        using I1 = std::integral_constant<int, 1>;
        using I2 = std::integral_constant<int, 2>;
        const int g = wave >> 2;
        if (g & 1) taylor(I2{}, I1{}, std::true_type{}, 2 * g, wave & 3, g == 3 ? 1 : 2, std::false_type{});
        else taylor(I2{}, I1{}, std::false_type{}, 2 * g, wave & 3, 2, std::false_type{});
    }
#else
    if (NARROW && FULL) {
        using I1 = std::integral_constant<int, 1>;
        using I2 = std::integral_constant<int, 2>;
        if (closed) {
            taylor(I1{}, I1{}, std::false_type{}, wave < 6 ? wave : wave - 6, 0, 1, std::false_type{});
            mirror_spin();
        }
        else if (wave < 4) taylor(I2{}, I1{}, std::false_type{}, 2 * (wave & 1), 2 * (wave >> 1), 2, std::false_type{});
        else taylor(I1{}, I1{}, std::false_type{}, 4 + (wave & 1), 2 * ((wave - 4) >> 1), 1, std::false_type{});
    }
    else if (NARROW) {
        using I1 = std::integral_constant<int, 1>;
        using I2 = std::integral_constant<int, 2>;
        if (wave < 4) taylor(I2{}, I1{}, std::false_type{}, 2 * (wave & 1), 2 * (wave >> 1), 2, std::false_type{});
        else if (nrt <= 6) taylor(I2{}, I1{}, std::true_type{}, 4 + (wave & 1), 2 * ((wave - 4) >> 1), 1, std::false_type{});
        else taylor(I2{}, I1{}, std::true_type{}, (wave & 1) ? 6 : 4, 2 * ((wave - 4) >> 1), (wave & 1) ? 1 : 2, std::false_type{});
    }
    else if (FULL == 7 && contig) {
        if constexpr (FULL == 7) {
            using I1 = std::integral_constant<int, 1>;
            using I2 = std::integral_constant<int, 2>;
            auto deal = [&](auto nu) __attribute__((always_inline)) {
                if (wave == 0 || wave == 2) taylor(I2{}, I2{}, std::false_type{}, wave, 0, 2, std::false_type{});
                else if (wave == 1 || wave == 3) taylor_h(std::true_type{}, std::false_type{}, nu, wave - 1, 2, 3, 0);
                else if (wave == 4 || wave == 6) taylor(I1{}, I1{}, std::true_type{}, 4, (wave - 4) >> 1, 1, std::true_type{});
                else if (wave == 5) taylor(I1{}, I2{}, std::true_type{}, 5, 0, 1, std::false_type{});
                else taylor_h(std::true_type{}, std::true_type{}, nu, 4, 2, 3, 2);
            };
            if (hyb == 2) deal(I2{});
            else deal(I1{});
        }
    }
    else if (FULL >= 5 && closed) {
        using I1 = std::integral_constant<int, 1>;
        using I2 = std::integral_constant<int, 2>;
        const int cs = wave & 1;
        if (wave < 4) taylor(I2{}, I1{}, std::false_type{}, 2 * (wave >> 1), cs, 2, std::false_type{});
        else if constexpr (FULL == 7) {
            if (a.rem4) {
                if (wave < 6) taylor(I1{}, I1{}, std::true_type{}, 4, cs, 1, std::true_type{});
                else taylor(I1{}, I1{}, std::true_type{}, 5, cs, 1, std::false_type{});
            } else {
                if (wave < 6) taylor(I2{}, I1{}, std::true_type{}, 4, cs, 2, std::false_type{});
                else taylor(I1{}, I1{}, std::true_type{}, 6, cs, 1, std::false_type{});
            }
        }
        else taylor(I1{}, I1{}, std::true_type{}, (FULL == 6 && wave >= 6) ? 5 : 4, cs, 1, std::false_type{});
        mirror_spin();
    }
    else if (wave < 4) taylor(std::integral_constant<int, 2>{}, std::integral_constant<int, 2>{}, std::false_type{}, 2 * (wave >> 1), 2 * (wave & 1), 2, std::false_type{});
    else if constexpr (FULL == 7) {
        if (a.rem4) taylor(std::integral_constant<int, 2>{}, std::integral_constant<int, 1>{}, std::true_type{}, 4, wave - 4, 2, std::true_type{});
        else taylor(std::integral_constant<int, 3>{}, std::integral_constant<int, 1>{}, std::true_type{}, 4, wave - 4, 3, std::false_type{});
    }
    else if (FULL >= 5) taylor(std::integral_constant<int, FULL >= 5 ? FULL - 4 : 1>{}, std::integral_constant<int, 1>{}, std::true_type{}, 4, wave - 4, FULL - 4, std::false_type{});
    else taylor(std::integral_constant<int, 3>{}, std::integral_constant<int, 1>{}, std::true_type{}, 4, wave - 4, 3, std::false_type{});
#endif
    if (a.order == 0) lds_barrier();

    one_body_stage(true);
    asm volatile("s_waitcnt vmcnt(0)" ::: "memory");
}

int k_prop_fused_supported(afq_handle *h) {
    return !h->vhs_diag && h->nv == 1 && h->M <= 104 && h->na <= 32 && h->nb <= 32 && h->nb > 0;
}

int k_prop_fused(afq_handle *h) {
    PropFusedArgs a;
    a.M = h->M; a.na = h->na; a.nb = h->nb; a.nt = h->nt; a.order = h->exp_order;
    a.vhs_upper = h->vhs_upper ? 1 : 0;
    a.same_b = h->bh1_same ? 1 : 0;
    a.b_real = h->bh1_real ? 1 : 0;
    a.rem4 = (h->M > 96 && h->M <= 100) ? 1 : 0;
    a.hyb = 0;
    a.contig = 0; a.symcols = 0;
    if (a.rem4 && a.same_b && h->na > 16 && h->nb > 16 && h->nt > 48 && h->nt <= 56 && PF_NW == 8) {
        a.contig = 1;
        a.hyb = (h->nt - 48 + 3) / 4;
    }
    a.symcols = (a.contig && h->na == h->nb) ? 1 : 0;
    a.closed_try = 0;
    a.BH1 = h->BH1; a.vhs = h->vhs; a.phi = h->phi; a.alive = h->alive; a.zero16 = h->zero_page;
    a.n_closed = h->counters + 3;
    const int NCH = (h->M + 7) / 8;
    const size_t lds = (size_t)NCH * 8192 + (size_t)PF_D * 16384;
    static size_t lds_set[6][AFQ_MAX_DEVICES] = {{0}, {0}, {0}, {0}, {0}, {0}};
    const bool narrow = h->na <= 16 && h->nb <= 16;
    KernelTrace kt(h, AFQ_K_PROPAGATOR);
    {
        const int nrt_ = (h->M + 15) / 16, ct = (h->na + 15) / 16 + (h->nb + 15) / 16;
        const double ksteps = 2.0 * NCH;
        const double per_pass = ksteps * (2048.0 * (a.rem4 ? nrt_ - 1 : nrt_) * ct + 512.0 * (a.rem4 ? ct : 0));
        const double taylor_pass = a.contig ? ksteps * (2048.0 * (nrt_ - 1) * 3 + 512.0 * (nrt_ - 1) * a.hyb + 512.0 * 4) : per_pass;
        h->issued_flops[AFQ_K_PROPAGATOR] = (3.0 * h->exp_order * taylor_pass + 2.0 * (a.b_real ? 2.0 : 3.0) * per_pass) * h->nw;
        h->prop_issued_open = h->issued_flops[AFQ_K_PROPAGATOR] / h->nw;
        const int cta = (h->na + 15) / 16;
        const double closed_pass = ksteps * (2048.0 * (a.rem4 ? nrt_ - 1 : nrt_) * cta + 512.0 * (a.rem4 ? cta : 0));
        h->prop_issued_closed = 3.0 * h->exp_order * closed_pass + 2.0 * (a.b_real ? 2.0 : 3.0) * per_pass;
    }
    const int nrt = (h->M + 15) / 16;
    const bool nofull = PF_NW != 8;
    const int full = nofull ? 0 : narrow ? (nrt == 6 ? 6 : 0) : (nrt >= 5 && h->na > 16 && h->nb > 16 ? nrt : 0);
    a.closed_try = (a.same_b && h->na == h->nb && h->exp_order > 0 && full != 0 && PF_NW == 8 &&
                    (!a.contig || a.symcols)) ? 1 : 0;
#define PF_LAUNCH_(NARROW_, FULL_, SLOT_)                                                                     \
    do {                                                                                                      \
        AFQ_HIP(h, afq_raise_lds((const void *)prop_fused_kernel<NARROW_, FULL_>, lds, lds_set[SLOT_]));      \
        AFQ_LAUNCH(h, (prop_fused_kernel<NARROW_, FULL_>), dim3(h->nw), dim3(PF_NT), lds, h->stream, a);      \
    } while (0)
    if (narrow && full) PF_LAUNCH_(true, 6, 0);
    else if (narrow) PF_LAUNCH_(true, 0, 1);
    else if (full == 7) PF_LAUNCH_(false, 7, 2);
    else if (full == 6) PF_LAUNCH_(false, 6, 3);
    else if (full == 5) PF_LAUNCH_(false, 5, 4);
    else PF_LAUNCH_(false, 0, 5);
#undef PF_LAUNCH_
    AFQ_POST(h);
    return AFQ_OK;
}
```

### pauxy_amd/csrc/k_small.hip

```cpp
#include <cstdlib>
#include <cstring>
#include <type_traits>
#include "mfma_gemm.h"
#include "gj_wave.h"
#include "lds_dma.h"

#include "block_scan.h"
#define NTHR 256

__global__ void alive_kernel(const double *weight, int *alive, int nw) {
    const int w = blockIdx.x * blockDim.x + threadIdx.x;
    if (w < nw) alive[w] = fabs(weight[w]) > 1e-8 ? 1 : 0;
}

int k_alive(afq_handle *h) {
    AFQ_LAUNCH(h, alive_kernel, dim3((h->nw + 255) / 256), dim3(256), 0, h->stream, h->weight,
                       h->alive, h->nw);
    AFQ_POST(h);
    return AFQ_OK;
}

__device__ inline void lu_factor(cplx *O, int n, int *perm, int *piv_s, cplx *ph, double *la) {
    const int tid = threadIdx.x;
    for (int i = tid; i < n; i += NTHR) perm[i] = i;
    if (tid == 0) { *ph = cmake(1.0, 0.0); *la = 0.0; }
    __syncthreads();
    for (int k = 0; k < n; ++k) {
        if (tid < 64) {
            double best = -1.0; int bi = k;
            for (int i = k + tid; i < n; i += 64) {
                const cplx v = O[(long)i * n + k];
                const double m = fabs(v.x) + fabs(v.y);
                if (m > best) { best = m; bi = i; }
            }
            for (int off = 32; off > 0; off >>= 1) {
                const double ob = __shfl_down(best, off);
                const int oi = __shfl_down(bi, off);
                if (ob > best || (ob == best && oi < bi)) { best = ob; bi = oi; }
            }
            if (tid == 0) *piv_s = bi;
        }
        __syncthreads();
        const int p = *piv_s;
        if (p != k) {
            for (int j = tid; j < n; j += NTHR) {
                const cplx t = O[(long)k * n + j];
                O[(long)k * n + j] = O[(long)p * n + j];
                O[(long)p * n + j] = t;
            }
            if (tid == 0) { const int t = perm[k]; perm[k] = perm[p]; perm[p] = t; }
        }
        __syncthreads();
        const cplx d = O[(long)k * n + k];
        if (tid == 0) {
            const double a = hypot(d.x, d.y);
            cplx u = cmake(d.x / a, d.y / a);
            if (p != k) u = cmake(-u.x, -u.y);
            *ph = cmul(*ph, u);
            *la += log(a);
        }
        for (int i = k + 1 + tid; i < n; i += NTHR) O[(long)i * n + k] = cdiv(O[(long)i * n + k], d);
        __syncthreads();
        const int m = n - k - 1;
        for (int e = tid; e < m * m; e += NTHR) {
            const int i = k + 1 + e / m, j = k + 1 + e % m;
            cplx v = O[(long)i * n + j];
            const cplx l = O[(long)i * n + k], u = O[(long)k * n + j];
            v.x = fma(-l.x, u.x, v.x); v.x = fma(l.y, u.y, v.x);
            v.y = fma(-l.x, u.y, v.y); v.y = fma(-l.y, u.x, v.y);
            O[(long)i * n + j] = v;
        }
        __syncthreads();
    }
}

struct GreensArgs {
    int M, na, nb, nt, nw;
    const cplx *phi, *psi;
    long psi_stride;
    cplx *ghalf;
    cplx *gsum;
    cplx *oinv;
    cplx *det;
    cplx *det_a;
    cplx *ws;
    int o_in_lds;
    int only_alive;
    const int *alive;
    int psi_real;
    int skip_spin;
    int psi_closed;
    unsigned long long *closed_bad;
    unsigned long long closed_epoch;
    unsigned long long *counters;
};

__global__ __launch_bounds__(NTHR) void greens_kernel(GreensArgs a) {
    extern __shared__ __align__(16) unsigned char smem[];
    __shared__ int perm[256];
    __shared__ int piv_s;
    __shared__ cplx ph_s;
    __shared__ double la_s;
    const int w = blockIdx.x, tid = threadIdx.x;
    if (a.only_alive && !a.alive[w]) return;
    const int M = a.M, nt = a.nt;
    const cplx *phi = a.phi + (long)w * M * nt;
    cplx phase = cmake(1.0, 0.0);
    double logabs = 0.0;
    for (int s = 0; s < 2; ++s) {
        const int n = s == 0 ? a.na : a.nb;
        const int off = s == 0 ? 0 : a.na;
        if (n == 0) continue;
        cplx *O = a.o_in_lds ? (cplx *)smem : a.ws + (long)w * ((a.na > a.nb ? a.na : a.nb) * (long)(a.na > a.nb ? a.na : a.nb));
        for (int e = tid; e < n * n; e += NTHR) {
            const int i = e / n, j = e % n;
            cplx acc = cmake(0.0, 0.0);
            for (int p = 0; p < M; ++p) {
                const cplx x = phi[(long)p * nt + off + i];
                const cplx y = a.psi[w * a.psi_stride + (long)p * nt + off + j];
                acc.x = fma(x.x, y.x, acc.x); acc.x = fma(x.y, y.y, acc.x);
                acc.y = fma(x.y, y.x, acc.y); acc.y = fma(-x.x, y.y, acc.y);
            }
            O[(long)i * n + j] = acc;
        }
        __syncthreads();
        lu_factor(O, n, perm, &piv_s, &ph_s, &la_s);
        if (tid == 0) { phase = cmul(phase, ph_s); logabs += la_s; }
        if (tid == 0 && s == 0 && a.det_a) { const double e0 = exp(logabs); a.det_a[w] = cmake(phase.x * e0, phase.y * e0); }
        if (a.ghalf) {
            cplx *gh = a.ghalf + ((long)w * nt + off) * M;
            for (int c = tid; c < M; c += NTHR) {
                for (int i = 0; i < n; ++i) {
                    cplx acc = phi[(long)c * nt + off + perm[i]];
                    for (int j = 0; j < i; ++j) {
                        const cplx l = O[(long)i * n + j], y = gh[(long)j * M + c];
                        acc.x = fma(-l.x, y.x, acc.x); acc.x = fma(l.y, y.y, acc.x);
                        acc.y = fma(-l.x, y.y, acc.y); acc.y = fma(-l.y, y.x, acc.y);
                    }
                    gh[(long)i * M + c] = acc;
                }
                for (int i = n - 1; i >= 0; --i) {
                    cplx acc = gh[(long)i * M + c];
                    for (int j = i + 1; j < n; ++j) {
                        const cplx u = O[(long)i * n + j], x = gh[(long)j * M + c];
                        acc.x = fma(-u.x, x.x, acc.x); acc.x = fma(u.y, x.y, acc.x);
                        acc.y = fma(-u.x, x.y, acc.y); acc.y = fma(-u.y, x.x, acc.y);
                    }
                    gh[(long)i * M + c] = cdiv(acc, O[(long)i * n + i]);
                }
            }
        }
        __syncthreads();
    }
    if (tid == 0) {
        const double e = exp(logabs);
        a.det[w] = cmake(phase.x * e, phase.y * e);
    }
}


#include "weight_update.h"


static WeightArgs weight_args(afq_handle *h, cplx eshift);
static WeightArgs no_weight_args() {
    WeightArgs a;
    memset(&a, 0, sizeof(a));
    return a;
}

__global__ void weight_kernel(WeightArgs a) {
    const int w = blockIdx.x * blockDim.x + threadIdx.x;
    if (w >= a.nw) return;
    weight_update_and_cap(a, w);
}

#define GS_KSMAX 32
template <bool INVERSE, bool WGJ>
__global__ __launch_bounds__(512) void greens_small_kernel(GreensArgs a, WeightArgs wa) {
    extern __shared__ __align__(16) unsigned char smem[];
    __shared__ cplx ph_s[2];
    __shared__ double la_s[2];
    __shared__ unsigned long long pmax_s[2][48];
    const int w = blockIdx.x, tid = threadIdx.x;
    if (a.only_alive && !a.alive[w]) return;
    const int g = __builtin_amdgcn_readfirstlane(tid >> 8), wave = __builtin_amdgcn_readfirstlane((tid >> 6) & 3);
    const int lane = tid & 63;
    unsigned long long *pmax = pmax_s[g];
    if ((tid & 255) < 48) pmax[tid & 255] = 0ull;
    const int M = a.M, nt = a.nt;
    const int nmax = a.na > a.nb ? a.na : a.nb;
    const int n = g == 0 ? a.na : a.nb, off = g == 0 ? 0 : a.na;
    cplx *O = (cplx *)smem + (long)g * (nmax * nmax + 2 * nmax);
    cplx *colk = O + nmax * nmax, *rowk = colk + nmax;
    int *piv = (int *)((cplx *)smem + 2L * (nmax * nmax + 2 * nmax)) + g * nmax;
    cplx *phi_l = (cplx *)smem + 2L * (nmax * nmax + 2 * nmax) + ((2 * nmax + 3) / 4 + 1);
    const cplx *phi_g = a.phi + (long)w * M * nt;
    const int lr = lane & 15, lk = lane >> 4;
    const int nt16 = (n + 15) >> 4;
    const int nks = (M + 3) >> 2;
    constexpr int NG = GS_KSMAX / 4;
    const int ng = (nks + 3) >> 2;
    const bool yreal = WGJ && a.psi_real != 0;
    const char *psi_w = (const char *)(a.psi + w * a.psi_stride);
    const bool has_tile = wave < nt16 * nt16;
    bool closed = false;
    auto phase01 = [&](auto yr_tag) __attribute__((always_inline)) {
        constexpr bool YR = decltype(yr_tag)::value;
        using y_t = typename std::conditional<YR, double, cplx>::type;
        y_t yf[GS_KSMAX];
        auto load_trial = [&](int tj, const int g0) __attribute__((always_inline)) {
            const int jb = tj * 16 + lr, jbc = jb < n ? jb : n - 1;
            const unsigned col = (unsigned)(off + jbc) * 16u, rowb = (unsigned)nt * 16u;
#pragma unroll
            for (int q = 0; q < 16; ++q) {
                const int ks = g0 * 4 + q, p = ks * 4 + lk;
                yf[ks] = *(const y_t *)(psi_w + ((unsigned)(p < M ? p : M - 1) * rowb + col));
            }
        };
        const int tj0 = has_tile ? wave % nt16 : 0;
        if (has_tile) {
            load_trial(tj0, 0);
            if (ng > 4) load_trial(tj0, 4);
        }
        __builtin_amdgcn_sched_barrier(0);
        {
            const unsigned total = (unsigned)(M * nt) * 16u;
            const int wave8 = __builtin_amdgcn_readfirstlane(tid >> 6);
            for (unsigned b0 = (unsigned)wave8 * 1024u; b0 < total; b0 += 8 * 1024u) {
                const unsigned bo = b0 + (unsigned)lane * 16u;
                if (bo < total) glds16((const char *)phi_g + bo, (char *)phi_l + b0);
            }
            asm volatile("s_waitcnt vmcnt(0)" ::: "memory");
        }
        __syncthreads();
        if (WGJ && a.psi_closed && a.gsum && !a.oinv && INVERSE) {
            int same = 1;
            const int na_ = a.na;
            for (int e = tid; e < M * na_; e += 512) {
                const int p_ = e / na_, i_ = e - p_ * na_;
                const cplx x = phi_l[p_ * nt + i_], y = phi_l[p_ * nt + na_ + i_];
                same &= (__double_as_longlong(x.x) == __double_as_longlong(y.x)) & (__double_as_longlong(x.y) == __double_as_longlong(y.y));
            }
            closed = __syncthreads_and(same) != 0;
            if (!closed && tid == 0 && a.closed_bad) atomicMax(a.closed_bad, a.closed_epoch);
            if (closed && tid == 0 && a.counters) atomicAdd(&a.counters[5], 1ull);
        }
        for (int t = wave; t < (closed && g == 1 ? 0 : nt16 * nt16); t += 4) {
            const int ti = t / nt16, tj = t % nt16;
            const int ia = ti * 16 + lr;
            const int iac = ia < n ? ia : n - 1;
            if (!WGJ && t != wave) {
                load_trial(tj, 0);
                if (ng > 4) load_trial(tj, 4);
            }
            d4_t accR = {0, 0, 0, 0}, accI = {0, 0, 0, 0}, acc3 = {0, 0, 0, 0};
            cplx xa[4], xb[4];
            const unsigned xcol = (unsigned)(off + iac), xrow = (unsigned)nt;
            auto readx = [&](cplx (&x)[4], const int gq) __attribute__((always_inline)) {
#pragma unroll
                for (int u = 0; u < 4; ++u) {
                    const int p = (gq * 4 + u) * 4 + lk;
                    x[u] = phi_l[xcol + (unsigned)(p < M ? p : M - 1) * xrow];
                }
            };
            auto mf = [&](const cplx (&x)[4], const int gq) __attribute__((always_inline)) {
                const bool last = gq == ng - 1;
#pragma unroll
                for (int u = 0; u < 4; ++u) {
                    const bool dead = last && (gq * 4 + u) * 4 + lk >= M;
                    if constexpr (YR) {
                        const double y = dead ? 0.0 : yf[gq * 4 + u];
                        accR = mfma16(x[u].x, y, accR);
                        acc3 = mfma16(x[u].y, y, acc3);
                    } else {
                        const cplx y = dead ? cmake(0.0, 0.0) : yf[gq * 4 + u];
                        accR = mfma16(x[u].x, y.x, accR);
                        accI = mfma16(x[u].y, y.y, accI);
                        acc3 = mfma16(x[u].x + x[u].y, y.x - y.y, acc3);
                    }
                }
            };
            readx(xa, 0);
#pragma unroll
            for (int gq = 0; gq < NG; gq += 2) {
                if (gq < ng) {
                    if (gq + 1 < ng) readx(xb, gq + 1);
                    mf(xa, gq);
                }
                if (gq + 1 < ng) {
                    if (gq + 2 < ng) readx(xa, gq + 2 < NG ? gq + 2 : 0);
                    mf(xb, gq + 1);
                }
            }
#pragma unroll
            for (int r = 0; r < 4; ++r) {
                const int i = ti * 16 + lk + 4 * r, j = tj * 16 + lr;
                if (i < n && j < n) O[i * n + j] = YR ? cmake(accR[r], acc3[r]) : cmake(accR[r] + accI[r], acc3[r] - accR[r] + accI[r]);
            }
            if (WGJ) break;
        }
    };
    if (yreal) phase01(std::true_type{});
    else phase01(std::false_type{});
    __syncthreads();
    __shared__ cplx gj_row[2][32], gj_piv[2][32];
    __shared__ int gj_prow[2][32];
    if (WGJ) {
        if (wave == g && !(closed && g == 1)) {
            cplx ph;
            int la;
            gj_wave32(O, n, lane, INVERSE, gj_row[g], gj_piv[g], gj_prow[g], ph, la);
            if (lane == 0) {
                ph_s[g] = ph; la_s[g] = (double)la;
                if (closed) { ph_s[1] = ph; la_s[1] = (double)la; }
            }
        }
    } else if (wave == 0) {
        cplx ph = cmake(1.0, 0.0);
        int la = 0;
        const int cw_shift = n <= 32 ? 5 : 6;
        const int cj = lane & ((1 << cw_shift) - 1), ri = lane >> cw_shift, rstep = 64 >> cw_shift;
        for (int k = 0; k < n; ++k) {
            unsigned long long mbits = 0;
            if (lane < n) {
                const cplx v = O[lane * n + k];
                colk[lane] = v;
                if (lane >= k) {
                    mbits = (unsigned long long)__double_as_longlong(fabs(v.x) + fabs(v.y));
                    atomicMax(&pmax[k], mbits);
                }
            }
            __builtin_amdgcn_wave_barrier();
            const unsigned long long mx = pmax[k];
            const unsigned long long hit = __ballot(lane >= k && lane < n && mbits == mx);
            const int p = hit ? __ffsll((long long)hit) - 1 : k;
            if (p != k) {
                for (int j = lane; j < n; j += 64) {
                    const cplx t = O[k * n + j];
                    O[k * n + j] = O[p * n + j];
                    O[p * n + j] = t;
                }
                if (lane == 0) { const cplx t = colk[k]; colk[k] = colk[p]; colk[p] = t; }
            }
            if (lane == 0) piv[k] = p;
            __builtin_amdgcn_wave_barrier();
            const cplx d = colk[k];
            ph = cmul(ph, p != k ? cmake(-d.x, -d.y) : d);
            {
                int e;
                (void)frexp(fmax(fabs(ph.x), fabs(ph.y)), &e);
                ph = cmake(ldexp(ph.x, -e), ldexp(ph.y, -e));
                la += e;
            }
            const double dn = 1.0 / (d.x * d.x + d.y * d.y);
            const cplx dinv = cmake(d.x * dn, -d.y * dn);
            for (int j = lane; j < n; j += 64) rowk[j] = cmul(O[k * n + j], dinv);
            __builtin_amdgcn_wave_barrier();
            if (n <= 32) {
                if (cj < n && (INVERSE || cj > k)) {
                    const cplx rk = rowk[cj];
                    cplx v[16], f[16];
#pragma unroll
                    for (int t = 0; t < 16; ++t) {
                        const int i = ri + 2 * t;
                        if (i < n) { v[t] = O[i * n + cj]; f[t] = colk[i]; }
                    }
#pragma unroll
                    for (int t = 0; t < 16; ++t) {
                        const int i = ri + 2 * t;
                        if (i < n && (INVERSE || i > k)) {
                            cplx o;
                            if (INVERSE && i == k) o = (cj == k) ? dinv : rk;
                            else if (INVERSE && cj == k) { const cplx m = cmul(f[t], dinv); o = cmake(-m.x, -m.y); }
                            else {
                                o = v[t];
                                o.x = fma(-f[t].x, rk.x, o.x); o.x = fma(f[t].y, rk.y, o.x);
                                o.y = fma(-f[t].x, rk.y, o.y); o.y = fma(-f[t].y, rk.x, o.y);
                            }
                            O[i * n + cj] = o;
                        }
                    }
                }
            } else if (INVERSE) {
                if (cj < n) {
                    const cplx rk = rowk[cj];
                    for (int i = ri; i < n; i += rstep) {
                        cplx v;
                        if (i == k) v = (cj == k) ? dinv : rk;
                        else {
                            const cplx f = colk[i];
                            if (cj == k) { const cplx t = cmul(f, dinv); v = cmake(-t.x, -t.y); }
                            else {
                                v = O[i * n + cj];
                                v.x = fma(-f.x, rk.x, v.x); v.x = fma(f.y, rk.y, v.x);
                                v.y = fma(-f.x, rk.y, v.y); v.y = fma(-f.y, rk.x, v.y);
                            }
                        }
                        O[i * n + cj] = v;
                    }
                }
            } else {
                if (cj < n && cj > k) {
                    const cplx rk = rowk[cj];
                    for (int i = k + 1 + ri; i < n; i += rstep) {
                        const cplx f = colk[i];
                        cplx v = O[i * n + cj];
                        v.x = fma(-f.x, rk.x, v.x); v.x = fma(f.y, rk.y, v.x);
                        v.y = fma(-f.x, rk.y, v.y); v.y = fma(-f.y, rk.x, v.y);
                        O[i * n + cj] = v;
                    }
                }
            }
            __builtin_amdgcn_wave_barrier();
        }
        if (INVERSE) {
            for (int k = n - 1; k >= 0; --k) {
                const int p = piv[k];
                if (p != k) {
                    for (int i = lane; i < n; i += 64) {
                        const cplx t = O[i * n + k];
                        O[i * n + k] = O[i * n + p];
                        O[i * n + p] = t;
                    }
                }
                __builtin_amdgcn_wave_barrier();
            }
        }
        if (lane == 0) { ph_s[g] = ph; la_s[g] = (double)la; }
    }
    __syncthreads();
    if (tid == 448) {
        const cplx p2 = cmul(ph_s[0], ph_s[1]);
        const int e = (int)(la_s[0] + la_s[1]);
        a.det[w] = cmake(ldexp(p2.x, e), ldexp(p2.y, e));
        if (a.det_a) a.det_a[w] = cmake(ldexp(ph_s[0].x, (int)la_s[0]), ldexp(ph_s[0].y, (int)la_s[0]));
        if (wa.weight) weight_update_and_cap(wa, w);
    }
    if (INVERSE && a.oinv) {
        cplx *oo = a.oinv + ((long)w * 2 + g) * nmax * nmax;
        for (int e = tid & 255; e < n * n; e += 256) oo[(e / n) * nmax + (e % n)] = O[e];
    }
    if (INVERSE && a.ghalf) {
        const bool both = a.gsum != nullptr;
        const int mt16 = (M + 15) >> 4, npair = (mt16 + 1) >> 1;
        const int first = both ? __builtin_amdgcn_readfirstlane(tid >> 6) : wave, stride = both ? 8 : 4;
        const int s_lo = both ? 0 : g, s_hi = both ? 2 : g + 1;
        const int nn = both ? a.na : n, nt16x = (nn + 15) >> 4;
        for (int it = first; nn > 0 && it < nt16x * npair; it += stride) {
            const int ti = it % nt16x, tc0 = 2 * (it / nt16x), tc1 = tc0 + 1;
            const bool two = tc1 < mt16;
            const int c0 = tc0 * 16 + lr, c1 = tc1 * 16 + lr;
            const int c0c = c0 < M ? c0 : M - 1, c1c = c1 < M ? c1 : M - 1;
            d4_t sra = {0, 0, 0, 0}, sia = {0, 0, 0, 0}, srb = {0, 0, 0, 0}, sib = {0, 0, 0, 0};
            for (int s = s_lo; s < (closed ? 1 : s_hi); ++s) {
                const int ns = s ? a.nb : a.na, offs = s ? a.na : 0;
                const cplx *Os = (const cplx *)smem + (long)s * (nmax * nmax + 2 * nmax);
                cplx *gh = a.ghalf + ((long)w * nt + offs) * M;
                const int nks3 = (ns + 3) >> 2;
                const int ia = ti * 16 + lr, iac = ia < ns ? ia : ns - 1;
                cplx xf[12];
#pragma unroll
                for (int ks = 0; ks < 12; ++ks) {
                    const int j = ks * 4 + lk, jc = j < ns ? j : ns - 1;
                    const cplx x = Os[iac * ns + jc];
                    xf[ks] = (ks < nks3 && j < ns && ia < ns) ? x : cmake(0.0, 0.0);
                }
                d4_t p1a = {0, 0, 0, 0}, p2a = {0, 0, 0, 0}, p3a = {0, 0, 0, 0};
                d4_t p1b = {0, 0, 0, 0}, p2b = {0, 0, 0, 0}, p3b = {0, 0, 0, 0};
#pragma unroll
                for (int ks = 0; ks < 12; ++ks) {
                    if (ks < nks3) {
                        const int j = ks * 4 + lk, jc = j < ns ? j : ns - 1;
                        const cplx y0 = phi_l[c0c * nt + offs + jc], y1 = phi_l[c1c * nt + offs + jc];
                        const cplx x = xf[ks];
                        const double xs = x.x + x.y;
                        p1a = mfma16(x.x, y0.x, p1a);
                        p2a = mfma16(x.y, y0.y, p2a);
                        p3a = mfma16(xs, y0.x + y0.y, p3a);
                        if (two) {
                            p1b = mfma16(x.x, y1.x, p1b);
                            p2b = mfma16(x.y, y1.y, p2b);
                            p3b = mfma16(xs, y1.x + y1.y, p3b);
                        }
                    }
                }
#pragma unroll
                for (int r = 0; r < 4; ++r) {
                    const int i = ti * 16 + lk + 4 * r;
                    const double ra = p1a[r] - p2a[r], ima = p3a[r] - p1a[r] - p2a[r];
                    const double rb = p1b[r] - p2b[r], imb = p3b[r] - p1b[r] - p2b[r];
                    if (i < ns && c0 < M && !a.skip_spin) gh[(long)i * M + c0] = cmake(ra, ima);
                    if (two && i < ns && c1 < M && !a.skip_spin) gh[(long)i * M + c1] = cmake(rb, imb);
                    sra[r] += ra; sia[r] += ima; srb[r] += rb; sib[r] += imb;
                    if (closed) {
                        cplx *ghb = gh + (long)a.na * M;
                        if (i < ns && c0 < M && !a.skip_spin) ghb[(long)i * M + c0] = cmake(ra, ima);
                        if (two && i < ns && c1 < M && !a.skip_spin) ghb[(long)i * M + c1] = cmake(rb, imb);
                        sra[r] += ra; sia[r] += ima; srb[r] += rb; sib[r] += imb;
                    }
                }
            }
            if (both) {
                cplx *gs = a.gsum + (long)w * a.na * M;
#pragma unroll
                for (int r = 0; r < 4; ++r) {
                    const int i = ti * 16 + lk + 4 * r;
                    if (i < a.na && c0 < M) gs[(long)i * M + c0] = cmake(sra[r], sia[r]);
                    if (two && i < a.na && c1 < M) gs[(long)i * M + c1] = cmake(srb[r], sib[r]);
                }
            }
        }
    }
}

template <bool INVERSE>
__global__ __launch_bounds__(512) void greens_tiny_kernel(GreensArgs a, WeightArgs wa) {
    extern __shared__ __align__(16) unsigned char smem[];
    __shared__ cplx O_l[2][64], oinv_l[2][64], piv_l[2][32];
    __shared__ int prow_l[2][32];
    __shared__ cplx ph_s[2];
    __shared__ int la_s[2];
    const int w = blockIdx.x, tid = threadIdx.x;
    if (a.only_alive && !a.alive[w]) return;
    const int M = a.M, nt = a.nt, na = a.na, nb = a.nb;
    cplx *phi_l = (cplx *)smem, *psi_l = phi_l + (long)M * nt;
    const int lane = tid & 63, wave8 = __builtin_amdgcn_readfirstlane(tid >> 6);
    {
        const unsigned total = (unsigned)(M * nt) * 16u;
        const char *phi_g = (const char *)(a.phi + (long)w * M * nt), *psi_g = (const char *)(a.psi + w * a.psi_stride);
        for (unsigned b0 = (unsigned)wave8 * 1024u; b0 < total; b0 += 8 * 1024u) {
            const unsigned bo = b0 + (unsigned)lane * 16u;
            if (bo < total) { glds16(phi_g + bo, (char *)phi_l + b0); glds16(psi_g + bo, (char *)psi_l + b0); }
        }
        asm volatile("s_waitcnt vmcnt(0)" ::: "memory");
    }
    __syncthreads();
    {
        const int o = tid >> 2, c4 = tid & 3;
        const int s = o >> 6, i = (o >> 3) & 7, j = o & 7;
        const int ns = s ? nb : na, off = s ? na : 0;
        const bool live = i < ns && j < ns;
        const int ic = off + (live ? i : 0), jc = off + (live ? j : 0);
        double ar = 0.0, ai = 0.0;
        const int nterm = (M - c4 + 3) >> 2;
        for (int t0 = 0; t0 < nterm; t0 += 8) {
            cplx x[8], y[8];
#pragma unroll
            for (int u = 0; u < 8; ++u) {
                const int p_ = c4 + 4 * (t0 + u), pc = p_ < M ? p_ : c4;
                x[u] = phi_l[pc * nt + ic]; y[u] = psi_l[pc * nt + jc];
                if (p_ >= M) x[u] = cmake(0.0, 0.0);
            }
#pragma unroll
            for (int u = 0; u < 8; ++u) {
                ar = fma(x[u].x, y[u].x, ar); ar = fma(x[u].y, y[u].y, ar);
                ai = fma(x[u].y, y[u].x, ai); ai = fma(-x[u].x, y[u].y, ai);
            }
        }
        ar += __shfl_xor(ar, 1); ai += __shfl_xor(ai, 1);
        ar += __shfl_xor(ar, 2); ai += __shfl_xor(ai, 2);
        if (c4 == 0) O_l[s][i * 8 + j] = live ? cmake(ar, ai) : cmake(i == j ? 1.0 : 0.0, 0.0);
        if (tid < 64) { piv_l[tid >> 5][tid & 31] = cmake(1.0, 0.0); prow_l[tid >> 5][tid & 31] = tid & 31; }
    }
    __syncthreads();
    if (wave8 < 2) {
        const int s = wave8, n = s ? nb : na;
        const int r = lane >> 3, c = lane & 7;
        cplx v = O_l[s][lane];
        double wx = v.x, wy = v.y;
        bool used = r >= n;
        int mystep = r;
#pragma unroll
        for (int k = 0; k < 8; ++k) {
            if (k < n) {
                const int src = (lane & 0x38) | k;
                const double fx = __shfl(wx, src), fy = __shfl(wy, src);
                const unsigned mb = (unsigned)__double2hiint(fabs(fx) + fabs(fy));
                const unsigned key = used ? 0u : ((((mb >> 5) + 1u) << 5) | (unsigned)(31 - r));
                const int p_ = 31 - (int)(gj_wave_max_u32(key) & 31u);
                const bool isp = r == p_;
                const double dx = __hiloint2double(__builtin_amdgcn_readlane(__double2hiint(fx), p_ * 8),
                                                   __builtin_amdgcn_readlane(__double2loint(fx), p_ * 8));
                const double dy = __hiloint2double(__builtin_amdgcn_readlane(__double2hiint(fy), p_ * 8),
                                                   __builtin_amdgcn_readlane(__double2loint(fy), p_ * 8));
                const double nn = fma(dx, dx, dy * dy);
                double dn = __builtin_amdgcn_rcp(nn);
                dn = fma(fma(-nn, dn, 1.0), dn, dn);
                dn = fma(fma(-nn, dn, 1.0), dn, dn);
                const double ix = dx * dn, iy = -dy * dn;
                const int psrc = p_ * 8 + c;
                double px = __shfl(wx, psrc), py = __shfl(wy, psrc);
                if (c == k) { px = 1.0; py = 0.0; }
                const double qx = fma(px, ix, -(py * iy)), qy = fma(px, iy, py * ix);
                if (isp) {
                    wx = qx; wy = qy; mystep = k;
                    if (c == 0) piv_l[s][k] = cmake(dx, dy);
                } else {
                    const double bx = c == k ? 0.0 : wx, by = c == k ? 0.0 : wy;
                    wx = fma(-fx, qx, bx); wx = fma(fy, qy, wx);
                    wy = fma(-fx, qy, by); wy = fma(-fy, qx, wy);
                }
                used = used || isp;
            }
        }
        if (c == 0 && r < n) prow_l[s][mystep] = r;
        __builtin_amdgcn_wave_barrier();
        if (INVERSE && r < n && c < n) oinv_l[s][mystep * 8 + prow_l[s][c]] = cmake(wx, wy);
        cplx ph;
        int la;
        gj_wave_det(n, lane, piv_l[s], prow_l[s], ph, la);
        if (lane == 0) { ph_s[s] = ph; la_s[s] = la; }
    }
    __syncthreads();
    if (tid == 448) {
        const cplx p2 = cmul(ph_s[0], ph_s[1]);
        const int e = la_s[0] + la_s[1];
        a.det[w] = cmake(ldexp(p2.x, e), ldexp(p2.y, e));
        if (a.det_a) a.det_a[w] = cmake(ldexp(ph_s[0].x, la_s[0]), ldexp(ph_s[0].y, la_s[0]));
        if (wa.weight) weight_update_and_cap(wa, w);
    }
    if (!INVERSE) return;
    const int nmax = na > nb ? na : nb;
    if (a.oinv) {
        cplx *oo = a.oinv + (long)w * 2 * nmax * nmax;
        for (int e = tid; e < 2 * nmax * nmax; e += 512) {
            const int s = e / (nmax * nmax), rem = e - s * nmax * nmax, i = rem / nmax, j = rem - i * nmax;
            const int ns = s ? nb : na;
            if (i < ns && j < ns) oo[e] = oinv_l[s][i * 8 + j];
        }
    }
    if (!a.ghalf) return;
    auto ghalf_of = [&](const int s, const int i, const int q) {
        const int ns = s ? nb : na, off = s ? na : 0;
        double gr = 0.0, gi = 0.0;
        cplx x[8], y[8];
#pragma unroll
        for (int j = 0; j < 8; ++j) {
            const int jc = j < ns ? j : 0;
            x[j] = oinv_l[s][i * 8 + jc]; y[j] = phi_l[q * nt + off + jc];
            if (j >= ns) x[j] = cmake(0.0, 0.0);
        }
#pragma unroll
        for (int j = 0; j < 8; ++j) {
            gr = fma(x[j].x, y[j].x, gr); gr = fma(-x[j].y, y[j].y, gr);
            gi = fma(x[j].x, y[j].y, gi); gi = fma(x[j].y, y[j].x, gi);
        }
        return cmake(gr, gi);
    };
    cplx *gh = a.ghalf + (long)w * nt * M;
    if (a.gsum) {
        cplx *gs = a.gsum + (long)w * na * M;
        for (int e = tid; e < na * M; e += 512) {
            const int i = e / M, q = e - i * M;
            const cplx ga = ghalf_of(0, i, q), gb = ghalf_of(1, i, q);
            if (!a.skip_spin) { gh[e] = ga; gh[(long)na * M + e] = gb; }
            gs[e] = cmake(ga.x + gb.x, ga.y + gb.y);
        }
    } else {
        for (int e = tid; e < nt * M; e += 512) {
            const int ii = e / M, q = e - ii * M;
            const int s = ii < na ? 0 : 1;
            gh[e] = ghalf_of(s, ii - (s ? na : 0), q);
        }
    }
}

static int launch_greens(afq_handle *h, cplx *ghalf, cplx *det, int only_alive, cplx *oinv = nullptr) {
    GreensArgs a;
    a.oinv = oinv; a.gsum = nullptr;
    if (ghalf) ++h->ghalf_version;
    a.M = h->M; a.na = h->na; a.nb = h->nb; a.nt = h->nt; a.nw = h->nw;
    a.phi = h->phi; a.psi = h->psi; a.psi_stride = h->psi_stride; a.ghalf = ghalf; a.det = det; a.ws = h->lu_ws;
    a.det_a = h->det_a_out;
    a.psi_real = h->psi_real && h->psi_stride == 0 && h->ndet <= 1;
    a.psi_closed = h->psi_closed && h->psi_stride == 0 && h->ndet <= 1;
    a.closed_bad = nullptr; a.closed_epoch = 0; a.counters = h->counters;
    if (ghalf == h->ghalf) h->closed_checked_version = 0;
    a.skip_spin = 0;
    const int nmax = h->na > h->nb ? h->na : h->nb;
    if (nmax > 256) AFQ_FAIL(h, AFQ_EUNSUPPORTED, "more than 256 electrons per spin");
    if (k_greens_big_supported(h)) {
        if (h->fuse_weight_req && det == h->ovlp_new && !only_alive && !oinv && h->ndet <= 1) {
            const WeightArgs wa = weight_args(h, h->fuse_eshift);
            h->fuse_weight_done = true;
            h->fuse_weight_req = false;
            return k_greens_big(h, ghalf, det, oinv, &wa);
        }
        return k_greens_big(h, ghalf, det, oinv);
    }
    const size_t lds_small = sizeof(cplx) * (2 * ((size_t)nmax * nmax + 2 * nmax) + ((2 * nmax + 3) / 4 + 1) + (size_t)h->M * h->nt);
    if (nmax <= 45 && h->M <= 4 * GS_KSMAX && lds_small <= 160 * 1024) {
        a.o_in_lds = 1; a.only_alive = only_alive; a.alive = h->alive;
        WeightArgs wa = no_weight_args();
        if (h->fuse_weight_req && det == h->ovlp_new && !only_alive && !oinv) {
            wa = weight_args(h, h->fuse_eshift);
            h->fuse_weight_done = true;
        }
        h->fuse_weight_req = false;
        if (h->M > 4 * GS_KSMAX) AFQ_FAIL(h, AFQ_EUNSUPPORTED, "fast Green's kernel supports M <= 128");
        const size_t lds = sizeof(cplx) * (2 * ((size_t)nmax * nmax + 2 * nmax) + ((2 * nmax + 3) / 4 + 1) +
                                           (size_t)h->M * h->nt);
        static size_t lds_set[4][AFQ_MAX_DEVICES] = {{0}};
        const bool wgj = nmax <= 32;
        const size_t lds_tiny = sizeof(cplx) * 2 * (size_t)h->M * h->nt;
        static size_t lds_set_tiny[2][AFQ_MAX_DEVICES] = {{0}};
        const bool tiny = nmax <= 8 && h->nt >= 1 && lds_tiny <= 150 * 1024;
        if (ghalf || oinv) {
            const bool want_sum = ghalf && ghalf == h->ghalf && !only_alive && k_fb_use_sum(h) && h->psi_stride == 0;
            if (want_sum) {
                if (!h->ghalf_sum) AFQ_HIP(h, hipMalloc(&h->ghalf_sum, sizeof(cplx) * (size_t)h->na * h->M * h->nw));
                a.gsum = h->ghalf_sum;
                if (h->ghalf_skip_store && (wgj || tiny) && !oinv) { a.skip_spin = 1; h->ghalf_skipped = true; }
            }
            if (want_sum && wgj && !tiny && a.psi_closed && !oinv) {
                a.closed_bad = h->closed_bad; a.closed_epoch = ++h->closed_epoch;
                h->closed_checked_version = h->ghalf_version;
            }
            KernelTrace kt(h, AFQ_K_GREENS);
            if (tiny) {
                AFQ_HIP(h, afq_raise_lds((const void *)greens_tiny_kernel<true>, lds_tiny, lds_set_tiny[0]));
                AFQ_LAUNCH(h, (greens_tiny_kernel<true>), dim3(h->nw), dim3(512), lds_tiny, h->stream, a, wa);
            } else if (wgj) {
                AFQ_HIP(h, afq_raise_lds((const void *)greens_small_kernel<true, true>, lds, lds_set[0]));
                AFQ_LAUNCH(h, (greens_small_kernel<true, true>), dim3(h->nw), dim3(512), lds, h->stream, a, wa);
            } else {
                AFQ_HIP(h, afq_raise_lds((const void *)greens_small_kernel<true, false>, lds, lds_set[1]));
                AFQ_LAUNCH(h, (greens_small_kernel<true, false>), dim3(h->nw), dim3(512), lds, h->stream, a, wa);
            }
            if (want_sum) h->gsum_version = h->ghalf_version;
        } else if (tiny) {
            AFQ_HIP(h, afq_raise_lds((const void *)greens_tiny_kernel<false>, lds_tiny, lds_set_tiny[1]));
            AFQ_LAUNCH(h, (greens_tiny_kernel<false>), dim3(h->nw), dim3(512), lds_tiny, h->stream, a, wa);
        } else if (wgj) {
            AFQ_HIP(h, afq_raise_lds((const void *)greens_small_kernel<false, true>, lds, lds_set[2]));
            AFQ_LAUNCH(h, (greens_small_kernel<false, true>), dim3(h->nw), dim3(512), lds, h->stream, a, wa);
        } else {
            AFQ_HIP(h, afq_raise_lds((const void *)greens_small_kernel<false, false>, lds, lds_set[3]));
            AFQ_LAUNCH(h, (greens_small_kernel<false, false>), dim3(h->nw), dim3(512), lds, h->stream, a, wa);
        }
        AFQ_POST(h);
        return AFQ_OK;
    }
    if (oinv) AFQ_FAIL(h, AFQ_EUNSUPPORTED, "inverse overlaps: the walker and both overlap matrices must fit 160 KB of LDS (N <= 45) or N > 45");
    const size_t need = sizeof(cplx) * (size_t)nmax * nmax;
    a.o_in_lds = need <= 64 * 1024;
    a.only_alive = only_alive; a.alive = h->alive;
    if (!a.o_in_lds && !h->lu_ws)
        AFQ_HIP(h, hipMalloc(&h->lu_ws, sizeof(cplx) * (size_t)h->nw * nmax * nmax));
    a.ws = h->lu_ws;
    AFQ_LAUNCH(h, greens_kernel, dim3(h->nw), dim3(NTHR), a.o_in_lds ? need : 0, h->stream, a);
    AFQ_POST(h);
    return AFQ_OK;
}

int k_greens(afq_handle *h, cplx *det_out) { return launch_greens(h, h->ghalf, det_out, 0); }
int k_overlap(afq_handle *h, cplx *det_out) { return launch_greens(h, nullptr, det_out, 0); }
int k_inverse_overlap(afq_handle *h, cplx *oinv, cplx *det_out) {
    const int nmax = h->na > h->nb ? h->na : h->nb;
    if (!k_greens_big_supported(h) && (nmax > 45 || h->M > 4 * GS_KSMAX))
        AFQ_FAIL(h, AFQ_EUNSUPPORTED, "inverse overlaps: N <= 128 per spin (N <= 45: M <= 128)");
    return launch_greens(h, nullptr, det_out, 1, oinv);
}

struct XbarArgs {
    int kind, flags, M, K, na, nb, nt, nw, nsplit, nq;
    double sqrt_dt, U;
    const cplx *vbias, *mf, *ghalf, *psi;
    const cplx *psicT;
    const cplx *gdiag;
    int gparts;
    cplx *xbar;
    int ndet;
    long det_stride;
    const cplx *detw;
    cplx *hub_fac = nullptr;
    double hub_f = 0.0;
    int hub_spin = 0, hub_order = 0;
};

__device__ inline cplx xbar_value(const XbarArgs &a, int w, int n) {
    cplx out = cmake(0.0, 0.0);
    if (a.flags & AFQ_PROP_FORCE_BIAS) {
        if (a.kind == AFQ_SYS_GENERIC) {
            cplx v = cmake(0.0, 0.0);
            if (a.ndet > 1) {
                cplx num = cmake(0.0, 0.0), den = cmake(0.0, 0.0);
                for (int d = 0; d < a.ndet; ++d) {
                    const cplx wd = a.detw[(long)w * a.ndet + d];
                    if (wd.x == 0.0 && wd.y == 0.0) continue;
                    cplx x = cmake(0.0, 0.0);
                    const cplx *vb = a.vbias + (long)d * a.det_stride;
                    for (int b = 0; b < 2 * a.nsplit; ++b) x = cadd(x, vb[((long)b * a.nw + w) * a.K + n]);
                    cfma(num, wd, x);
                    den = cadd(den, wd);
                }
                v = cdiv(num, den);
            } else {
                const int nb2 = 2 * a.nsplit;
                const cplx *vb = a.vbias + (long)w * a.K + n;
                const long bs = (long)a.nw * a.K;
                int b = 0;
                for (; b + 3 < nb2; b += 4) {
                    const cplx t0 = vb[b * bs], t1 = vb[(b + 1) * bs], t2 = vb[(b + 2) * bs], t3 = vb[(b + 3) * bs];
                    v = cadd(cadd(cadd(cadd(v, t0), t1), t2), t3);
                }
                for (; b < nb2; ++b) v = cadd(v, vb[b * bs]);
            }
            const cplx m = a.mf[n];
            out = cmake(-a.sqrt_dt * (-v.y - m.x), -a.sqrt_dt * (v.x - m.y));
        } else if (a.kind == AFQ_SYS_HUBBARD) {
            cplx g[2] = {cmake(0.0, 0.0), cmake(0.0, 0.0)};
            if (a.gdiag) {
                for (int s = 0; s < 2; ++s)
                    for (int pt = 0; pt < a.gparts; ++pt) g[s] = cadd(g[s], a.gdiag[((long)(2 * w + s) * a.gparts + pt) * a.M + n]);
            } else
            for (int s = 0; s < 2; ++s) {
                const int ns = s == 0 ? a.na : a.nb, off = s == 0 ? 0 : a.na;
                for (int i = 0; i < ns; ++i) {
                    const cplx c = a.psicT ? a.psicT[(long)(off + i) * a.M + n] : cconj(a.psi[(long)n * a.nt + off + i]);
                    cfma(g[s], c, a.ghalf[((long)w * a.nt + off + i) * a.M + n]);
                }
            }
            const cplx m = a.mf[n];
            const double su = sqrt(a.U);
            cplx vb;
            if (a.flags & AFQ_PROP_HUBBARD_SPIN) {
                vb = cmake(su * (g[0].x - g[1].x), su * (g[0].y - g[1].y));
            } else {
                const cplx t = cadd(g[0], g[1]);
                vb = cmake(-su * t.y, su * t.x);
            }
            out = cmake(-a.sqrt_dt * (vb.x - m.x), -a.sqrt_dt * (vb.y - m.y));
        } else {
            const cplx v = a.vbias[(long)w * a.K + n];
            out = cmake(-a.sqrt_dt * v.x, -a.sqrt_dt * v.y);
        }
    }
    return out;
}

__global__ void xbar_kernel(XbarArgs a) {
    const int w = blockIdx.y;
    const int n = blockIdx.x * blockDim.x + threadIdx.x;
    if (n >= a.K) return;
    a.xbar[(long)w * a.K + n] = xbar_value(a, w, n);
}

static XbarArgs xbar_args(afq_handle *h) {
    XbarArgs a;
    a.kind = h->kind; a.flags = h->flags; a.M = h->M; a.K = h->K; a.na = h->na; a.nb = h->nb;
    a.nt = h->nt; a.nw = h->nw; a.nsplit = h->fb_split; a.nq = h->nq;
    a.sqrt_dt = h->sqrt_dt; a.U = h->U;
    a.vbias = h->vbias; a.mf = h->mf_shift; a.ghalf = h->ghalf; a.psi = h->psi; a.xbar = h->xbar;
    a.psicT = (h->ndet <= 1 && h->psi_stride == 0) ? h->psicT : nullptr;
    a.gdiag = (h->kind == AFQ_SYS_HUBBARD && h->gdiag && h->gdiag_version == h->ghalf_version) ? h->gdiag : nullptr;
    a.gparts = h->gdiag_parts;
    a.ndet = h->ndet; a.detw = h->detw; a.det_stride = (long)2 * h->fb_split * h->nw * h->K;
    if (h->ndet > 1) a.vbias = h->vbias_all;
    if (h->ndet > 1 && h->msd_fb_gbar && h->kind == AFQ_SYS_GENERIC) a.ndet = 1;
    return a;
}

int k_xbar(afq_handle *h) {
    const XbarArgs a = xbar_args(h);
    AFQ_LAUNCH(h, xbar_kernel, dim3((h->K + 127) / 128, h->nw), dim3(128), 0, h->stream, a);
    AFQ_POST(h);
    return AFQ_OK;
}

__global__ void msd_combine_kernel(const cplx *detd, const cplx *detd_a, const cplx *coeffs, cplx *detw, cplx *det_out, int nw,
                                   int ndet, int skip_small, unsigned long long *counters) {
    const int w = blockIdx.x * blockDim.x + threadIdx.x;
    if (w >= nw) return;
    cplx tot = cmake(0.0, 0.0);
    for (int d = 0; d < ndet; ++d) {
        cplx dd = detd[(long)d * nw + w];
        const double mag = hypot(dd.x, dd.y);
        bool skip = skip_small && mag < 1e-16;
        if (skip_small && detd_a) {
            const cplx da = detd_a[(long)d * nw + w];
            const double ma = hypot(da.x, da.y);
            skip = skip || ma < 1e-16;
        }
        if (!(mag == mag)) { skip = true; if (counters) atomicAdd(&counters[6], 1ull); }
        if (skip) dd = cmake(0.0, 0.0);
        const cplx wd = cmul(cconj(coeffs[d]), dd);
        detw[(long)w * ndet + d] = wd;
        tot = cadd(tot, wd);
    }
    det_out[w] = tot;
}

int k_msd_combine(afq_handle *h, cplx *det_out, bool skip_small) {
    AFQ_LAUNCH(h, msd_combine_kernel, dim3((h->nw + 127) / 128), dim3(128), 0, h->stream, h->detd,
                       skip_small ? h->detd_a : nullptr, h->coeffs, h->detw, det_out, h->nw, h->ndet, skip_small ? 1 : 0, h->counters);
    AFQ_POST(h);
    return AFQ_OK;
}

__global__ void msd_energy_combine_kernel(const cplx *energy_all, const cplx *detw, cplx *energy, int nw,
                                          int ndet) {
    const int w = blockIdx.x * blockDim.x + threadIdx.x;
    if (w >= nw) return;
    cplx num[3] = {cmake(0.0, 0.0), cmake(0.0, 0.0), cmake(0.0, 0.0)}, den = cmake(0.0, 0.0);
    for (int d = 0; d < ndet; ++d) {
        const cplx wd = detw[(long)w * ndet + d];
        if (wd.x == 0.0 && wd.y == 0.0) continue;
        for (int c = 0; c < 3; ++c) cfma(num[c], wd, energy_all[((long)d * nw + w) * 3 + c]);
        den = cadd(den, wd);
    }
    for (int c = 0; c < 3; ++c) energy[(long)w * 3 + c] = cdiv(num[c], den);
}

int k_msd_energy_combine(afq_handle *h) {
    AFQ_LAUNCH(h, msd_energy_combine_kernel, dim3((h->nw + 127) / 128), dim3(128), 0, h->stream,
                       h->energy_all, h->detw, h->energy, h->nw, h->ndet);
    AFQ_POST(h);
    return AFQ_OK;
}

#include "philox.h"

__device__ inline double block_sum(double v, double *red) {
    for (int off = 32; off > 0; off >>= 1) v += __shfl_down(v, off);
    const int wave = threadIdx.x >> 6, lane = threadIdx.x & 63;
    __syncthreads();
    if (lane == 0) red[wave] = v;
    __syncthreads();
    double t = 0.0;
    for (int i = 0; i < (int)(blockDim.x >> 6); ++i) t += red[i];
    return t;
}


template <bool FUSED>
__global__ __launch_bounds__(NTHR) void fields_kernel(int K, double sqrt_dt, const double *xi, cplx *xbar,
                                                      const cplx *mf, cplx *xs, cplx *cmf, cplx *cfb,
                                                      unsigned long long *counters, const int *alive, XbarArgs xa,
                                                      FieldRng rng) {
    __shared__ double red[NTHR / 64][8];
    const int w = blockIdx.x;
    if (rng.on) {
        const bool live = fabs(rng.weight[w]) > 1e-8;
        if (threadIdx.x == 0) rng.alive_out[w] = live ? 1 : 0;
        if (!live) return;
    } else if (alive && !alive[w]) return;
    double acc[7] = {0, 0, 0, 0, 0, 0, 0};
    auto element = [&](const long e, const int n, const double xdev, cplx b, const cplx mm) {
        const double ab = hypot(b.x, b.y);
        if (ab > 1.0) { b.x /= ab; b.y /= ab; acc[6] += 1.0; }
        const double x = rng.on ? xdev : xi[e];
        const cplx sft = cmake(x - b.x, -b.y);
        {
        xbar[e] = b;
        xs[e] = sft;
        }
        if (FUSED && xa.hub_fac) {
            auto taylor = [&](const cplx d) {
                cplx acc = cmake(1.0, 0.0), t = acc;
                for (int k = 1; k <= xa.hub_order; ++k) {
                    t = cmul(d, t);
                    t = cmake(t.x / k, t.y / k);
                    acc = cadd(acc, t);
                }
                return acc;
            };
            if (!xa.hub_spin) xa.hub_fac[(long)w * K + n] = taylor(cmake(-xa.hub_f * sft.y, xa.hub_f * sft.x));
            else {
                xa.hub_fac[((long)w * 2 + 0) * K + n] = taylor(cmake(-xa.hub_f * sft.x, -xa.hub_f * sft.y));
                xa.hub_fac[((long)w * 2 + 1) * K + n] = taylor(cmake(xa.hub_f * sft.x, xa.hub_f * sft.y));
            }
        }
        acc[0] += sft.x * mm.x - sft.y * mm.y;
        acc[1] += sft.x * mm.y + sft.y * mm.x;
        acc[2] += x * b.x; acc[3] += x * b.y;
        acc[4] += b.x * b.x - b.y * b.y;
        acc[5] += 2.0 * b.x * b.y;
    };
    const long e0 = (long)w * K;
    if (K <= NTHR) {
        const int n = threadIdx.x;
        if (n < K) {
            const cplx b = FUSED ? xbar_value(xa, w, n) : xbar[e0 + n];
            const cplx mm = mf[n];
            double xn[2] = {0.0, 0.0};
            if (rng.on) philox_normal_pair((e0 + n) >> 1, rng.seed, rng.stream, rng.counter, xn[0], xn[1]);
            element(e0 + n, n, xn[(e0 + n) & 1], b, mm);
        }
    } else {
        const bool flight = FUSED && xa.kind == AFQ_SYS_GENERIC && xa.ndet <= 1 && (xa.flags & AFQ_PROP_FORCE_BIAS) && !xa.hub_fac;
        for (long pr = (e0 >> 1) + threadIdx.x; pr <= ((e0 + K - 1) >> 1); pr += NTHR) {
            cplx bb[2] = {cmake(0.0, 0.0), cmake(0.0, 0.0)}, mm[2] = {cmake(0.0, 0.0), cmake(0.0, 0.0)};
            if (flight) {
                int nn[2];
#pragma unroll
                for (int m = 0; m < 2; ++m) {
                    const int n = (int)(2 * pr + m - e0);
                    nn[m] = n < 0 ? 0 : n >= K ? K - 1 : n;
                }
                const int nb2 = 2 * xa.nsplit;
                const long bs = (long)xa.nw * K;
                const cplx *vb0 = xa.vbias + (long)w * K + nn[0], *vb1 = xa.vbias + (long)w * K + nn[1];
                mm[0] = mf[nn[0]]; mm[1] = mf[nn[1]];
                cplx v0 = cmake(0.0, 0.0), v1 = cmake(0.0, 0.0);
                int b = 0;
                for (; b + 7 < nb2; b += 8) {
                    cplx t0[8], t1[8];
#pragma unroll
                    for (int j = 0; j < 8; ++j) { t0[j] = vb0[(b + j) * bs]; t1[j] = vb1[(b + j) * bs]; }
#pragma unroll
                    for (int j = 0; j < 8; ++j) { v0 = cadd(v0, t0[j]); v1 = cadd(v1, t1[j]); }
                }
                for (; b + 3 < nb2; b += 4) {
                    cplx t0[4], t1[4];
#pragma unroll
                    for (int j = 0; j < 4; ++j) { t0[j] = vb0[(b + j) * bs]; t1[j] = vb1[(b + j) * bs]; }
#pragma unroll
                    for (int j = 0; j < 4; ++j) { v0 = cadd(v0, t0[j]); v1 = cadd(v1, t1[j]); }
                }
                for (; b < nb2; ++b) { v0 = cadd(v0, vb0[b * bs]); v1 = cadd(v1, vb1[b * bs]); }
                bb[0] = cmake(-xa.sqrt_dt * (-v0.y - mm[0].x), -xa.sqrt_dt * (v0.x - mm[0].y));
                bb[1] = cmake(-xa.sqrt_dt * (-v1.y - mm[1].x), -xa.sqrt_dt * (v1.x - mm[1].y));
            } else
#pragma unroll
            for (int m = 0; m < 2; ++m) {
                const long e = 2 * pr + m;
                const int n = (int)(e - e0);
                if (n >= 0 && n < K) { bb[m] = FUSED ? xbar_value(xa, w, n) : xbar[e]; mm[m] = mf[n]; }
            }
            double xn[2] = {0.0, 0.0};
// ... 989 lines not shown
```

Measured before the change: 1.034 million walker-steps/s.

## Defer fused propagation and merge it into the following Green's function kernel

The fused exponential propagation is deferred out of propagate_begin and then run together with the small-N Gauss-Jordan Green's function computation, with the greens body moved into a shared header so both kernels can use it. The aim is to skip one kernel launch and the global round-trip of the propagated walker, since phi can stay in LDS and be written back from the greens kernel. This adds a deferred-state flag protocol with fallback paths, which raises the risk of ordering bugs when greens is not called on the expected path.

```diff
diff --git a/pauxy_amd/csrc/afq_api.hip b/pauxy_amd/csrc/afq_api.hip
--- a/pauxy_amd/csrc/afq_api.hip
+++ b/pauxy_amd/csrc/afq_api.hip
@@ -899,8 +899,12 @@
 }
 
 int afq_propagate(afq_handle *h, const double *xi, double eshift_re, double eshift_im) {
-    const int rc = afq_propagate_begin(h, xi);
-    return rc ? rc : afq_propagate_finish(h, eshift_re, eshift_im);
+    if (h) h->prop_defer_ok = true;
+    int rc = afq_propagate_begin(h, xi);
+    if (h) h->prop_defer_ok = false;
+    if (!rc) rc = afq_propagate_finish(h, eshift_re, eshift_im);
+    if (h && h->prop_deferred) { h->prop_deferred = false; h->vhs_upper = false; }
+    return rc;
 }
 
 int afq_propagate_begin(afq_handle *h, const double *xi) {
@@ -978,7 +982,10 @@
     h->vhs_upper = fused && h->hs_sym;
     { PhaseTimer t(h, T_VHS); rc = build_vhs(h); }
     if (rc) { h->vhs_upper = false; return rc; }
-    if (fused) {
+    if (fused && h->prop_defer_ok && k_prop_fused_greens_supported(h) && h->ndet == 1 && !fp && h->greens_cache &&
+        k_greens_wgj(h)) {
+        h->prop_deferred = true;
+    } else if (fused) {
         PhaseTimer t(h, T_EXP);
         rc = k_prop_fused(h);
         h->vhs_upper = false;
diff --git a/pauxy_amd/csrc/afq_internal.h b/pauxy_amd/csrc/afq_internal.h
--- a/pauxy_amd/csrc/afq_internal.h
+++ b/pauxy_amd/csrc/afq_internal.h
@@ -214,6 +214,8 @@
     double *gfrag = nullptr;
     size_t gfrag_bytes = 0;
     bool prop_pending = false;
+    bool prop_defer_ok = false;
+    bool prop_deferred = false;
     double *est_stage = nullptr;
     unsigned long long est_seq = 0;
     double scal_cache[AFQ_NSCAL] = {0};
@@ -358,6 +360,7 @@
 int k_full_G(afq_handle *h);
 int k_prop_fused_supported(afq_handle *h);
 int k_prop_fused(afq_handle *h);
+bool k_prop_fused_greens_supported(afq_handle *h);
 int k_hirsch_alive(afq_handle *h, int mode);
 int k_hirsch_kinetic(afq_handle *h);
 int k_hirsch_two_body(afq_handle *h);
@@ -383,6 +386,7 @@
 int k_gj_inverse(afq_handle *h, cplx *O, int n, int batch, cplx *detm, int *dete);
 int k_alive(afq_handle *h);
 int k_greens(afq_handle *h, cplx *det_out);
+bool k_greens_wgj(afq_handle *h);
 int k_overlap(afq_handle *h, cplx *det_out);
 int k_inverse_overlap(afq_handle *h, cplx *oinv, cplx *det_out);
 int k_fields(afq_handle *h);
diff --git a/pauxy_amd/csrc/greens_small.h b/pauxy_amd/csrc/greens_small.h
--- /dev/null
+++ b/pauxy_amd/csrc/greens_small.h
@@ -0,0 +1,386 @@
+#pragma once
+#include <type_traits>
+#include "mfma_gemm.h"
+#include "gj_wave.h"
+#include "lds_dma.h"
+#include "weight_update.h"
+
+struct GreensArgs {
+    int M, na, nb, nt, nw;
+    const cplx *phi, *psi;
+    long psi_stride;
+    cplx *ghalf;
+    cplx *gsum;
+    cplx *oinv;
+    cplx *det;
+    cplx *det_a;
+    cplx *ws;
+    int o_in_lds;
+    int only_alive;
+    const int *alive;
+    int psi_real;
+    int skip_spin;
+    int psi_closed;
+    unsigned long long *closed_bad;
+    unsigned long long closed_epoch;
+    unsigned long long *counters;
+};
+
+#define GS_KSMAX 32
+
+int k_prop_fused_deferred(afq_handle *h, const GreensArgs *ga, const WeightArgs *wa);
+
+__device__ inline cplx *greens_small_phi_l(unsigned char *smem, const GreensArgs &a) {
+    const int nmax = a.na > a.nb ? a.na : a.nb;
+    return (cplx *)smem + 2L * (nmax * nmax + 2 * nmax) + ((2 * nmax + 3) / 4 + 1);
+}
+
+template <bool INVERSE, bool WGJ>
+__device__ __attribute__((always_inline)) inline void greens_small_body(const GreensArgs &a, const WeightArgs &wa,
+                                                                        unsigned char *smem, cplx *phi_out) {
+    __shared__ cplx ph_s[2];
+    __shared__ double la_s[2];
+    __shared__ unsigned long long pmax_s[2][48];
+    const int w = blockIdx.x, tid = threadIdx.x;
+    if (a.only_alive && !a.alive[w]) return;
+    const int g = __builtin_amdgcn_readfirstlane(tid >> 8), wave = __builtin_amdgcn_readfirstlane((tid >> 6) & 3);
+    const int lane = tid & 63;
+    unsigned long long *pmax = pmax_s[g];
+    if ((tid & 255) < 48) pmax[tid & 255] = 0ull;
+    const int M = a.M, nt = a.nt;
+    const int nmax = a.na > a.nb ? a.na : a.nb;
+    const int n = g == 0 ? a.na : a.nb, off = g == 0 ? 0 : a.na;
+    cplx *O = (cplx *)smem + (long)g * (nmax * nmax + 2 * nmax);
+    cplx *colk = O + nmax * nmax, *rowk = colk + nmax;
+    int *piv = (int *)((cplx *)smem + 2L * (nmax * nmax + 2 * nmax)) + g * nmax;
+    cplx *phi_l = greens_small_phi_l(smem, a);
+    const cplx *phi_g = a.phi + (long)w * M * nt;
+    const int lr = lane & 15, lk = lane >> 4;
+    const int nt16 = (n + 15) >> 4;
+    const int nks = (M + 3) >> 2;
+    constexpr int NG = GS_KSMAX / 4;
+    const int ng = (nks + 3) >> 2;
+    const bool yreal = WGJ && a.psi_real != 0;
+    const char *psi_w = (const char *)(a.psi + w * a.psi_stride);
+    const bool has_tile = wave < nt16 * nt16;
+    bool closed = false;
+    auto phase01 = [&](auto yr_tag) __attribute__((always_inline)) {
+        constexpr bool YR = decltype(yr_tag)::value;
+        using y_t = typename std::conditional<YR, double, cplx>::type;
+        y_t yf[GS_KSMAX];
+        auto load_trial = [&](int tj, const int g0) __attribute__((always_inline)) {
+            const int jb = tj * 16 + lr, jbc = jb < n ? jb : n - 1;
+            const unsigned col = (unsigned)(off + jbc) * 16u, rowb = (unsigned)nt * 16u;
+#pragma unroll
+            for (int q = 0; q < 16; ++q) {
+                const int ks = g0 * 4 + q, p = ks * 4 + lk;
+                yf[ks] = *(const y_t *)(psi_w + ((unsigned)(p < M ? p : M - 1) * rowb + col));
+            }
+        };
+        const int tj0 = has_tile ? wave % nt16 : 0;
+        if (has_tile) {
+            load_trial(tj0, 0);
+            if (ng > 4) load_trial(tj0, 4);
+        }
+        __builtin_amdgcn_sched_barrier(0);
+        if (!phi_out) {
+            const unsigned total = (unsigned)(M * nt) * 16u;
+            const int wave8 = __builtin_amdgcn_readfirstlane(tid >> 6);
+            for (unsigned b0 = (unsigned)wave8 * 1024u; b0 < total; b0 += 8 * 1024u) {
+                const unsigned bo = b0 + (unsigned)lane * 16u;
+                if (bo < total) glds16((const char *)phi_g + bo, (char *)phi_l + b0);
+            }
+            asm volatile("s_waitcnt vmcnt(0)" ::: "memory");
+        }
+        __syncthreads();
+        if (WGJ && a.psi_closed && a.gsum && !a.oinv && INVERSE) {
+            int same = 1;
+            const int na_ = a.na;
+            for (int e = tid; e < M * na_; e += 512) {
+                const int p_ = e / na_, i_ = e - p_ * na_;
+                const cplx x = phi_l[p_ * nt + i_], y = phi_l[p_ * nt + na_ + i_];
+                same &= (__double_as_longlong(x.x) == __double_as_longlong(y.x)) & (__double_as_longlong(x.y) == __double_as_longlong(y.y));
+            }
+            closed = __syncthreads_and(same) != 0;
+            if (!closed && tid == 0 && a.closed_bad) atomicMax(a.closed_bad, a.closed_epoch);
+            if (closed && tid == 0 && a.counters) atomicAdd(&a.counters[5], 1ull);
+        }
+        for (int t = wave; t < (closed && g == 1 ? 0 : nt16 * nt16); t += 4) {
+            const int ti = t / nt16, tj = t % nt16;
+            const int ia = ti * 16 + lr;
+            const int iac = ia < n ? ia : n - 1;
+            if (!WGJ && t != wave) {
+                load_trial(tj, 0);
+                if (ng > 4) load_trial(tj, 4);
+            }
+            d4_t accR = {0, 0, 0, 0}, accI = {0, 0, 0, 0}, acc3 = {0, 0, 0, 0};
+            cplx xa[4], xb[4];
+            const unsigned xcol = (unsigned)(off + iac), xrow = (unsigned)nt;
+            auto readx = [&](cplx (&x)[4], const int gq) __attribute__((always_inline)) {
+#pragma unroll
+                for (int u = 0; u < 4; ++u) {
+                    const int p = (gq * 4 + u) * 4 + lk;
+                    x[u] = phi_l[xcol + (unsigned)(p < M ? p : M - 1) * xrow];
+                }
+            };
+            auto mf = [&](const cplx (&x)[4], const int gq) __attribute__((always_inline)) {
+                const bool last = gq == ng - 1;
+#pragma unroll
+                for (int u = 0; u < 4; ++u) {
+                    const bool dead = last && (gq * 4 + u) * 4 + lk >= M;
+                    if constexpr (YR) {
+                        const double y = dead ? 0.0 : yf[gq * 4 + u];
+                        accR = mfma16(x[u].x, y, accR);
+                        acc3 = mfma16(x[u].y, y, acc3);
+                    } else {
+                        const cplx y = dead ? cmake(0.0, 0.0) : yf[gq * 4 + u];
+                        accR = mfma16(x[u].x, y.x, accR);
+                        accI = mfma16(x[u].y, y.y, accI);
+                        acc3 = mfma16(x[u].x + x[u].y, y.x - y.y, acc3);
+                    }
+                }
+            };
+            readx(xa, 0);
+#pragma unroll
+            for (int gq = 0; gq < NG; gq += 2) {
+                if (gq < ng) {
+                    if (gq + 1 < ng) readx(xb, gq + 1);
+                    mf(xa, gq);
+                }
+                if (gq + 1 < ng) {
+                    if (gq + 2 < ng) readx(xa, gq + 2 < NG ? gq + 2 : 0);
+                    mf(xb, gq + 1);
+                }
+            }
+#pragma unroll
+            for (int r = 0; r < 4; ++r) {
+                const int i = ti * 16 + lk + 4 * r, j = tj * 16 + lr;
+                if (i < n && j < n) O[i * n + j] = YR ? cmake(accR[r], acc3[r]) : cmake(accR[r] + accI[r], acc3[r] - accR[r] + accI[r]);
+            }
+            if (WGJ) break;
+        }
+    };
+    if (yreal) phase01(std::true_type{});
+    else phase01(std::false_type{});
+    __syncthreads();
+    __shared__ cplx gj_row[2][32], gj_piv[2][32];
+    __shared__ int gj_prow[2][32];
+    if (WGJ) {
+        if (wave == g && !(closed && g == 1)) {
+            cplx ph;
+            int la;
+            gj_wave32(O, n, lane, INVERSE, gj_row[g], gj_piv[g], gj_prow[g], ph, la);
+            if (lane == 0) {
+                ph_s[g] = ph; la_s[g] = (double)la;
+                if (closed) { ph_s[1] = ph; la_s[1] = (double)la; }
+            }
+        } else if (phi_out) {
+            const int wave8 = __builtin_amdgcn_readfirstlane(tid >> 6), sw = wave8 - 1 - (wave8 > 5 ? 1 : 0);
+            if (wave8 != 5) {
+                const int total = M * nt;
+                for (int e = sw * 64 + lane; e < total; e += 6 * 64) ((d2_t *)phi_out)[e] = ((const d2_t *)phi_l)[e];
+            }
+        }
+    } else if (wave == 0) {
+        cplx ph = cmake(1.0, 0.0);
+        int la = 0;
+        const int cw_shift = n <= 32 ? 5 : 6;
+        const int cj = lane & ((1 << cw_shift) - 1), ri = lane >> cw_shift, rstep = 64 >> cw_shift;
+        for (int k = 0; k < n; ++k) {
+            unsigned long long mbits = 0;
+            if (lane < n) {
+                const cplx v = O[lane * n + k];
+                colk[lane] = v;
+                if (lane >= k) {
+                    mbits = (unsigned long long)__double_as_longlong(fabs(v.x) + fabs(v.y));
+                    atomicMax(&pmax[k], mbits);
+                }
+            }
+            __builtin_amdgcn_wave_barrier();
+            const unsigned long long mx = pmax[k];
+            const unsigned long long hit = __ballot(lane >= k && lane < n && mbits == mx);
+            const int p = hit ? __ffsll((long long)hit) - 1 : k;
+            if (p != k) {
+                for (int j = lane; j < n; j += 64) {
+                    const cplx t = O[k * n + j];
+                    O[k * n + j] = O[p * n + j];
+                    O[p * n + j] = t;
+                }
+                if (lane == 0) { const cplx t = colk[k]; colk[k] = colk[p]; colk[p] = t; }
+            }
+            if (lane == 0) piv[k] = p;
+            __builtin_amdgcn_wave_barrier();
+            const cplx d = colk[k];
+            ph = cmul(ph, p != k ? cmake(-d.x, -d.y) : d);
+            {
+                int e;
+                (void)frexp(fmax(fabs(ph.x), fabs(ph.y)), &e);
+                ph = cmake(ldexp(ph.x, -e), ldexp(ph.y, -e));
+                la += e;
+            }
+            const double dn = 1.0 / (d.x * d.x + d.y * d.y);
+            const cplx dinv = cmake(d.x * dn, -d.y * dn);
+            for (int j = lane; j < n; j += 64) rowk[j] = cmul(O[k * n + j], dinv);
+            __builtin_amdgcn_wave_barrier();
+            if (n <= 32) {
+                if (cj < n && (INVERSE || cj > k)) {
+                    const cplx rk = rowk[cj];
+                    cplx v[16], f[16];
+#pragma unroll
+                    for (int t = 0; t < 16; ++t) {
+                        const int i = ri + 2 * t;
+                        if (i < n) { v[t] = O[i * n + cj]; f[t] = colk[i]; }
+                    }
+#pragma unroll
+                    for (int t = 0; t < 16; ++t) {
+                        const int i = ri + 2 * t;
+                        if (i < n && (INVERSE || i > k)) {
+                            cplx o;
+                            if (INVERSE && i == k) o = (cj == k) ? dinv : rk;
+                            else if (INVERSE && cj == k) { const cplx m = cmul(f[t], dinv); o = cmake(-m.x, -m.y); }
+                            else {
+                                o = v[t];
+                                o.x = fma(-f[t].x, rk.x, o.x); o.x = fma(f[t].y, rk.y, o.x);
+                                o.y = fma(-f[t].x, rk.y, o.y); o.y = fma(-f[t].y, rk.x, o.y);
+                            }
+                            O[i * n + cj] = o;
+                        }
+                    }
+                }
+            } else if (INVERSE) {
+                if (cj < n) {
+                    const cplx rk = rowk[cj];
+                    for (int i = ri; i < n; i += rstep) {
+                        cplx v;
+                        if (i == k) v = (cj == k) ? dinv : rk;
+                        else {
+                            const cplx f = colk[i];
+                            if (cj == k) { const cplx t = cmul(f, dinv); v = cmake(-t.x, -t.y); }
+                            else {
+                                v = O[i * n + cj];
+                                v.x = fma(-f.x, rk.x, v.x); v.x = fma(f.y, rk.y, v.x);
+                                v.y = fma(-f.x, rk.y, v.y); v.y = fma(-f.y, rk.x, v.y);
+                            }
+                        }
+                        O[i * n + cj] = v;
+                    }
+                }
+            } else {
+                if (cj < n && cj > k) {
+                    const cplx rk = rowk[cj];
+                    for (int i = k + 1 + ri; i < n; i += rstep) {
+                        const cplx f = colk[i];
+                        cplx v = O[i * n + cj];
+                        v.x = fma(-f.x, rk.x, v.x); v.x = fma(f.y, rk.y, v.x);
+                        v.y = fma(-f.x, rk.y, v.y); v.y = fma(-f.y, rk.x, v.y);
+                        O[i * n + cj] = v;
+                    }
+                }
+            }
+            __builtin_amdgcn_wave_barrier();
+        }
+        if (INVERSE) {
+            for (int k = n - 1; k >= 0; --k) {
+                const int p = piv[k];
+                if (p != k) {
+                    for (int i = lane; i < n; i += 64) {
+                        const cplx t = O[i * n + k];
+                        O[i * n + k] = O[i * n + p];
+                        O[i * n + p] = t;
+                    }
+                }
+                __builtin_amdgcn_wave_barrier();
+            }
+        }
+        if (lane == 0) { ph_s[g] = ph; la_s[g] = (double)la; }
+    }
+    __syncthreads();
+    if (tid == 448) {
+        const cplx p2 = cmul(ph_s[0], ph_s[1]);
+        const int e = (int)(la_s[0] + la_s[1]);
+        a.det[w] = cmake(ldexp(p2.x, e), ldexp(p2.y, e));
+        if (a.det_a) a.det_a[w] = cmake(ldexp(ph_s[0].x, (int)la_s[0]), ldexp(ph_s[0].y, (int)la_s[0]));
+        if (wa.weight) weight_update_and_cap(wa, w);
+    }
+    if (INVERSE && a.oinv) {
+        cplx *oo = a.oinv + ((long)w * 2 + g) * nmax * nmax;
+        for (int e = tid & 255; e < n * n; e += 256) oo[(e / n) * nmax + (e % n)] = O[e];
+    }
+    if (INVERSE && a.ghalf) {
+        const bool both = a.gsum != nullptr;
+        const int mt16 = (M + 15) >> 4, npair = (mt16 + 1) >> 1;
+        const int first = both ? __builtin_amdgcn_readfirstlane(tid >> 6) : wave, stride = both ? 8 : 4;
+        const int s_lo = both ? 0 : g, s_hi = both ? 2 : g + 1;
+        const int nn = both ? a.na : n, nt16x = (nn + 15) >> 4;
+        for (int it = first; nn > 0 && it < nt16x * npair; it += stride) {
+            const int ti = it % nt16x, tc0 = 2 * (it / nt16x), tc1 = tc0 + 1;
+            const bool two = tc1 < mt16;
+            const int c0 = tc0 * 16 + lr, c1 = tc1 * 16 + lr;
+            const int c0c = c0 < M ? c0 : M - 1, c1c = c1 < M ? c1 : M - 1;
+            d4_t sra = {0, 0, 0, 0}, sia = {0, 0, 0, 0}, srb = {0, 0, 0, 0}, sib = {0, 0, 0, 0};
+            for (int s = s_lo; s < (closed ? 1 : s_hi); ++s) {
+                const int ns = s ? a.nb : a.na, offs = s ? a.na : 0;
+                const cplx *Os = (const cplx *)smem + (long)s * (nmax * nmax + 2 * nmax);
+                cplx *gh = a.ghalf + ((long)w * nt + offs) * M;
+                const int nks3 = (ns + 3) >> 2;
+                const int ia = ti * 16 + lr, iac = ia < ns ? ia : ns - 1;
+                cplx xf[12];
+#pragma unroll
+                for (int ks = 0; ks < 12; ++ks) {
+                    const int j = ks * 4 + lk, jc = j < ns ? j : ns - 1;
+                    const cplx x = Os[iac * ns + jc];
+                    xf[ks] = (ks < nks3 && j < ns && ia < ns) ? x : cmake(0.0, 0.0);
+                }
+                d4_t p1a = {0, 0, 0, 0}, p2a = {0, 0, 0, 0}, p3a = {0, 0, 0, 0};
+                d4_t p1b = {0, 0, 0, 0}, p2b = {0, 0, 0, 0}, p3b = {0, 0, 0, 0};
+#pragma unroll
+                for (int ks = 0; ks < 12; ++ks) {
+                    if (ks < nks3) {
+                        const int j = ks * 4 + lk, jc = j < ns ? j : ns - 1;
+                        const cplx y0 = phi_l[c0c * nt + offs + jc], y1 = phi_l[c1c * nt + offs + jc];
+                        const cplx x = xf[ks];
+                        const double xs = x.x + x.y;
+                        p1a = mfma16(x.x, y0.x, p1a);
+                        p2a = mfma16(x.y, y0.y, p2a);
+                        p3a = mfma16(xs, y0.x + y0.y, p3a);
+                        if (two) {
+                            p1b = mfma16(x.x, y1.x, p1b);
+                            p2b = mfma16(x.y, y1.y, p2b);
+                            p3b = mfma16(xs, y1.x + y1.y, p3b);
+                        }
+                    }
+                }
+#pragma unroll
+                for (int r = 0; r < 4; ++r) {
+                    const int i = ti * 16 + lk + 4 * r;
+                    const double ra = p1a[r] - p2a[r], ima = p3a[r] - p1a[r] - p2a[r];
+                    const double rb = p1b[r] - p2b[r], imb = p3b[r] - p1b[r] - p2b[r];
+                    if (i < ns && c0 < M && !a.skip_spin) gh[(long)i * M + c0] = cmake(ra, ima);
+                    if (two && i < ns && c1 < M && !a.skip_spin) gh[(long)i * M + c1] = cmake(rb, imb);
+                    sra[r] += ra; sia[r] += ima; srb[r] += rb; sib[r] += imb;
+                    if (closed) {
+                        cplx *ghb = gh + (long)a.na * M;
+                        if (i < ns && c0 < M && !a.skip_spin) ghb[(long)i * M + c0] = cmake(ra, ima);
+                        if (two && i < ns && c1 < M && !a.skip_spin) ghb[(long)i * M + c1] = cmake(rb, imb);
+                        sra[r] += ra; sia[r] += ima; srb[r] += rb; sib[r] += imb;
+                    }
+                }
+            }
+            if (both) {
+                cplx *gs = a.gsum + (long)w * a.na * M;
+#pragma unroll
+                for (int r = 0; r < 4; ++r) {
+                    const int i = ti * 16 + lk + 4 * r;
+                    if (i < a.na && c0 < M) gs[(long)i * M + c0] = cmake(sra[r], sia[r]);
+                    if (two && i < a.na && c1 < M) gs[(long)i * M + c1] = cmake(srb[r], sib[r]);
+                }
+            }
+        }
+    }
+}
+
+template <bool INVERSE, bool WGJ>
+__global__ __launch_bounds__(512) void greens_small_kernel(GreensArgs a, WeightArgs wa) {
+    extern __shared__ __align__(16) unsigned char smem[];
+    greens_small_body<INVERSE, WGJ>(a, wa, smem, nullptr);
+}
diff --git a/pauxy_amd/csrc/k_fused.hip b/pauxy_amd/csrc/k_fused.hip
--- a/pauxy_amd/csrc/k_fused.hip
+++ b/pauxy_amd/csrc/k_fused.hip
@@ -2,6 +2,7 @@
 #include <type_traits>
 
 #include "mfma_gemm_wg.h"
+#include "greens_small.h"
 
 #define PF_D 3
 #ifndef PF_NW
@@ -75,9 +76,8 @@
     asm volatile("" ::: "memory");
 }
 
-template <bool NARROW, int FULL>
-__global__ __launch_bounds__(PF_NT) void prop_fused_kernel(PropFusedArgs a) {
-    extern __shared__ __align__(16) unsigned char smem[];
+template <bool NARROW, int FULL, bool GREENS>
+__device__ __attribute__((always_inline)) inline void prop_fused_body(const PropFusedArgs &a, unsigned char *smem, cplx *phi_l) {
     const int w = blockIdx.x;
     if (!a.alive[w]) return;
     const int tid = threadIdx.x, lane = tid & 63, wave = __builtin_amdgcn_readfirstlane(tid >> 6);
@@ -319,6 +319,7 @@
 #endif
         }
         if (!to_global) __builtin_amdgcn_s_barrier();
+        if (GREENS && to_global) __syncthreads();
         int lk_e = lk, lr_e = lr;
         asm volatile("" : "+v"(lk_e), "+v"(lr_e));
 #pragma unroll
@@ -332,7 +333,7 @@
                     const double im = BR ? P2[j][r] : P3[j][r] - P1[j][r] - P2[j][r];
                     if (to_global) {
                         const int row = rt * 16 + lk_e + 4 * r, col = (contig ? cs : cs & 1) * 16 + lr_e;
-                        if (row < M && col < ns_) phi[(long)row * nt + off_ + wcol(col)] = cmake(re, im);
+                        if (row < M && col < ns_) (GREENS ? phi_l : phi)[(long)row * nt + off_ + wcol(col)] = cmake(re, im);
                     } else if (t_ok(rt, r)) {
                         *(d2_t *)(Tf + t_addr(rt, r, cs)) = (d2_t){re, im};
                     }
@@ -425,6 +426,7 @@
             if (more) sl = next_chunk_sync();
             half(a1, b1, q1, a0, b0, q0, sl + r0 * 2048 + lane * 16, tf_l + ((c + 1) * 4 + c0) * 2048 + lane * 16, sl + rem_a, 0, more, more);
         }
+        if (GREENS && to_global) __syncthreads();
         int lk_e = lk, lr_e = lr, ln_e = lane;
         asm volatile("" : "+v"(lk_e), "+v"(lr_e), "+v"(ln_e));
         const int sp = contig ? 0 : c0 >> 1, ns_ = contig ? nt : sp ? a.nb : a.na, off_ = sp ? a.na : 0;
@@ -437,7 +439,7 @@
                 const double im = BR ? P2[i][r] : P3[i][r] - P1[i][r] - P2[i][r];
                 if (to_global) {
                     const int row = (r0 + i) * 16 + lk_e + 4 * r, col = cb + lr_e;
-                    if (row < M && col < ns_) phi[(long)row * nt + off_ + wcol(col)] = cmake(re, im);
+                    if (row < M && col < ns_) (GREENS ? phi_l : phi)[(long)row * nt + off_ + wcol(col)] = cmake(re, im);
                 } else if (t_ok(r0 + i, r)) {
                     *(d2_t *)(Tf + t_addr(r0 + i, r, c0)) = (d2_t){re, im};
                 }
@@ -447,7 +449,7 @@
             const double re = BR ? Q1 : Q1 - Q2, im = BR ? Q2 : Q3 - Q1 - Q2;
             if (to_global) {
                 const int row = 96 + (ln_e >> 4), col = cb + (ln_e & 15);
-                if (row < M && col < ns_) phi[(long)row * nt + off_ + wcol(col)] = cmake(re, im);
+                if (row < M && col < ns_) (GREENS ? phi_l : phi)[(long)row * nt + off_ + wcol(col)] = cmake(re, im);
             } else {
                 *(d2_t *)(Tf + rem_t) = (d2_t){re, im};
             }
@@ -959,11 +961,37 @@
     asm volatile("s_waitcnt vmcnt(0)" ::: "memory");
 }
 
+template <bool NARROW, int FULL>
+__global__ __launch_bounds__(PF_NT) void prop_fused_kernel(PropFusedArgs a) {
+    extern __shared__ __align__(16) unsigned char smem[];
+    prop_fused_body<NARROW, FULL, false>(a, smem, nullptr);
+}
+
+template <bool NARROW, int FULL>
+__global__ __launch_bounds__(PF_NT) void prop_fused_kernel_with_greens(PropFusedArgs a, GreensArgs ga, WeightArgs wa) {
+    extern __shared__ __align__(16) unsigned char smem[];
+    const int w = blockIdx.x;
+    const bool live = a.alive[w] != 0;
+    if (live) prop_fused_body<NARROW, FULL, true>(a, smem, greens_small_phi_l(smem, ga));
+    greens_small_body<true, true>(ga, wa, smem, live ? a.phi + (long)w * a.M * a.nt : nullptr);
+}
+
 int k_prop_fused_supported(afq_handle *h) {
     return !h->vhs_diag && h->nv == 1 && h->M <= 104 && h->na <= 32 && h->nb <= 32 && h->nb > 0;
 }
 
-int k_prop_fused(afq_handle *h) {
+static int prop_full(afq_handle *h) {
+    const int nrt = (h->M + 15) / 16;
+    const bool narrow = h->na <= 16 && h->nb <= 16;
+    if (PF_NW != 8) return 0;
+    return narrow ? (nrt == 6 ? 6 : 0) : (nrt >= 5 && h->na > 16 && h->nb > 16 ? nrt : 0);
+}
+
+bool k_prop_fused_greens_supported(afq_handle *h) {
+    return k_prop_fused_supported(h) && prop_full(h) != 0 && h->bh1_same;
+}
+
+static int prop_fused_launch(afq_handle *h, const GreensArgs *ga, const WeightArgs *wa) {
     PropFusedArgs a;
     a.M = h->M; a.na = h->na; a.nb = h->nb; a.nt = h->nt; a.order = h->exp_order;
     a.vhs_upper = h->vhs_upper ? 1 : 0;
@@ -996,9 +1024,7 @@
         const double closed_pass = ksteps * (2048.0 * (a.rem4 ? nrt_ - 1 : nrt_) * cta + 512.0 * (a.rem4 ? cta : 0));
         h->prop_issued_closed = 3.0 * h->exp_order * closed_pass + 2.0 * (a.b_real ? 2.0 : 3.0) * per_pass;
     }
-    const int nrt = (h->M + 15) / 16;
-    const bool nofull = PF_NW != 8;
-    const int full = nofull ? 0 : narrow ? (nrt == 6 ? 6 : 0) : (nrt >= 5 && h->na > 16 && h->nb > 16 ? nrt : 0);
+    const int full = prop_full(h);
     a.closed_try = (a.same_b && h->na == h->nb && h->exp_order > 0 && full != 0 && PF_NW == 8 &&
                     (!a.contig || a.symcols)) ? 1 : 0;
 #define PF_LAUNCH_(NARROW_, FULL_, SLOT_)                                                                     \
@@ -1006,13 +1032,39 @@
         AFQ_HIP(h, afq_raise_lds((const void *)prop_fused_kernel<NARROW_, FULL_>, lds, lds_set[SLOT_]));      \
         AFQ_LAUNCH(h, (prop_fused_kernel<NARROW_, FULL_>), dim3(h->nw), dim3(PF_NT), lds, h->stream, a);      \
     } while (0)
-    if (narrow && full) PF_LAUNCH_(true, 6, 0);
+#define PFG_LAUNCH_(NARROW_, FULL_, SLOT_)                                                                    \
+    do {                                                                                                      \
+        AFQ_HIP(h, afq_raise_lds((const void *)prop_fused_kernel_with_greens<NARROW_, FULL_>, lds_g, lds_set_g[SLOT_])); \
+        AFQ_LAUNCH(h, (prop_fused_kernel_with_greens<NARROW_, FULL_>), dim3(h->nw), dim3(PF_NT), lds_g, h->stream, a, *ga, *wa); \
+    } while (0)
+    if (ga) {
+        if (!full || !a.same_b) AFQ_FAIL(h, AFQ_ESTATE, "internal: the propagator with the Green's function needs a full deal and one one-body matrix");
+        const int nmax = h->na > h->nb ? h->na : h->nb;
+        const size_t lds_greens = sizeof(cplx) * (2 * ((size_t)nmax * nmax + 2 * nmax) + ((2 * nmax + 3) / 4 + 1) + (size_t)h->M * h->nt);
+        const size_t lds_g = lds > lds_greens ? lds : lds_greens;
+        static size_t lds_set_g[4][AFQ_MAX_DEVICES] = {{0}, {0}, {0}, {0}};
+        if (narrow) PFG_LAUNCH_(true, 6, 0);
+        else if (full == 7) PFG_LAUNCH_(false, 7, 1);
+        else if (full == 6) PFG_LAUNCH_(false, 6, 2);
+        else PFG_LAUNCH_(false, 5, 3);
+    }
+    else if (narrow && full) PF_LAUNCH_(true, 6, 0);
     else if (narrow) PF_LAUNCH_(true, 0, 1);
     else if (full == 7) PF_LAUNCH_(false, 7, 2);
     else if (full == 6) PF_LAUNCH_(false, 6, 3);
     else if (full == 5) PF_LAUNCH_(false, 5, 4);
     else PF_LAUNCH_(false, 0, 5);
 #undef PF_LAUNCH_
+#undef PFG_LAUNCH_
     AFQ_POST(h);
     return AFQ_OK;
 }
+
+int k_prop_fused(afq_handle *h) { return prop_fused_launch(h, nullptr, nullptr); }
+
+int k_prop_fused_deferred(afq_handle *h, const GreensArgs *ga, const WeightArgs *wa) {
+    h->prop_deferred = false;
+    const int rc = prop_fused_launch(h, ga, wa);
+    h->vhs_upper = false;
+    return rc;
+}
diff --git a/pauxy_amd/csrc/k_small.hip b/pauxy_amd/csrc/k_small.hip
--- a/pauxy_amd/csrc/k_small.hip
+++ b/pauxy_amd/csrc/k_small.hip
@@ -4,6 +4,7 @@
 #include "mfma_gemm.h"
 #include "gj_wave.h"
 #include "lds_dma.h"
+#include "greens_small.h"
 
 #include "block_scan.h"
 #define NTHR 256
@@ -74,26 +75,6 @@
     }
 }
 
-struct GreensArgs {
-    int M, na, nb, nt, nw;
-    const cplx *phi, *psi;
-    long psi_stride;
-    cplx *ghalf;
-    cplx *gsum;
-    cplx *oinv;
-    cplx *det;
-    cplx *det_a;
-    cplx *ws;
-    int o_in_lds;
-    int only_alive;
-    const int *alive;
-    int psi_real;
-    int skip_spin;
-    int psi_closed;
-    unsigned long long *closed_bad;
-    unsigned long long closed_epoch;
-    unsigned long long *counters;
-};
 
 __global__ __launch_bounds__(NTHR) void greens_kernel(GreensArgs a) {
     extern __shared__ __align__(16) unsigned char smem[];
@@ -175,344 +156,6 @@
     weight_update_and_cap(a, w);
 }
 
-#define GS_KSMAX 32
-template <bool INVERSE, bool WGJ>
-__global__ __launch_bounds__(512) void greens_small_kernel(GreensArgs a, WeightArgs wa) {
-    extern __shared__ __align__(16) unsigned char smem[];
-    __shared__ cplx ph_s[2];
-    __shared__ double la_s[2];
-    __shared__ unsigned long long pmax_s[2][48];
-    const int w = blockIdx.x, tid = threadIdx.x;
-    if (a.only_alive && !a.alive[w]) return;
-    const int g = __builtin_amdgcn_readfirstlane(tid >> 8), wave = __builtin_amdgcn_readfirstlane((tid >> 6) & 3);
-    const int lane = tid & 63;
-    unsigned long long *pmax = pmax_s[g];
-    if ((tid & 255) < 48) pmax[tid & 255] = 0ull;
-    const int M = a.M, nt = a.nt;
-    const int nmax = a.na > a.nb ? a.na : a.nb;
-    const int n = g == 0 ? a.na : a.nb, off = g == 0 ? 0 : a.na;
-    cplx *O = (cplx *)smem + (long)g * (nmax * nmax + 2 * nmax);
-    cplx *colk = O + nmax * nmax, *rowk = colk + nmax;
-    int *piv = (int *)((cplx *)smem + 2L * (nmax * nmax + 2 * nmax)) + g * nmax;
-    cplx *phi_l = (cplx *)smem + 2L * (nmax * nmax + 2 * nmax) + ((2 * nmax + 3) / 4 + 1);
-    const cplx *phi_g = a.phi + (long)w * M * nt;
-    const int lr = lane & 15, lk = lane >> 4;
-    const int nt16 = (n + 15) >> 4;
-    const int nks = (M + 3) >> 2;
-    constexpr int NG = GS_KSMAX / 4;
-    const int ng = (nks + 3) >> 2;
-    const bool yreal = WGJ && a.psi_real != 0;
-    const char *psi_w = (const char *)(a.psi + w * a.psi_stride);
-    const bool has_tile = wave < nt16 * nt16;
-    bool closed = false;
-    auto phase01 = [&](auto yr_tag) __attribute__((always_inline)) {
-        constexpr bool YR = decltype(yr_tag)::value;
-        using y_t = typename std::conditional<YR, double, cplx>::type;
-        y_t yf[GS_KSMAX];
-        auto load_trial = [&](int tj, const int g0) __attribute__((always_inline)) {
-            const int jb = tj * 16 + lr, jbc = jb < n ? jb : n - 1;
-            const unsigned col = (unsigned)(off + jbc) * 16u, rowb = (unsigned)nt * 16u;
-#pragma unroll
-            for (int q = 0; q < 16; ++q) {
-                const int ks = g0 * 4 + q, p = ks * 4 + lk;
-                yf[ks] = *(const y_t *)(psi_w + ((unsigned)(p < M ? p : M - 1) * rowb + col));
-            }
-        };
-        const int tj0 = has_tile ? wave % nt16 : 0;
-        if (has_tile) {
-            load_trial(tj0, 0);
-            if (ng > 4) load_trial(tj0, 4);
-        }
-        __builtin_amdgcn_sched_barrier(0);
-        {
-            const unsigned total = (unsigned)(M * nt) * 16u;
-            const int wave8 = __builtin_amdgcn_readfirstlane(tid >> 6);
-            for (unsigned b0 = (unsigned)wave8 * 1024u; b0 < total; b0 += 8 * 1024u) {
-                const unsigned bo = b0 + (unsigned)lane * 16u;
-                if (bo < total) glds16((const char *)phi_g + bo, (char *)phi_l + b0);
-            }
-            asm volatile("s_waitcnt vmcnt(0)" ::: "memory");
-        }
-        __syncthreads();
-        if (WGJ && a.psi_closed && a.gsum && !a.oinv && INVERSE) {
-            int same = 1;
-            const int na_ = a.na;
-            for (int e = tid; e < M * na_; e += 512) {
-                const int p_ = e / na_, i_ = e - p_ * na_;
-                const cplx x = phi_l[p_ * nt + i_], y = phi_l[p_ * nt + na_ + i_];
-                same &= (__double_as_longlong(x.x) == __double_as_longlong(y.x)) & (__double_as_longlong(x.y) == __double_as_longlong(y.y));
-            }
-            closed = __syncthreads_and(same) != 0;
-            if (!closed && tid == 0 && a.closed_bad) atomicMax(a.closed_bad, a.closed_epoch);
-            if (closed && tid == 0 && a.counters) atomicAdd(&a.counters[5], 1ull);
-        }
-        for (int t = wave; t < (closed && g == 1 ? 0 : nt16 * nt16); t += 4) {
-            const int ti = t / nt16, tj = t % nt16;
-            const int ia = ti * 16 + lr;
-            const int iac = ia < n ? ia : n - 1;
-            if (!WGJ && t != wave) {
-                load_trial(tj, 0);
-                if (ng > 4) load_trial(tj, 4);
-            }
-            d4_t accR = {0, 0, 0, 0}, accI = {0, 0, 0, 0}, acc3 = {0, 0, 0, 0};
-            cplx xa[4], xb[4];
-            const unsigned xcol = (unsigned)(off + iac), xrow = (unsigned)nt;
-            auto readx = [&](cplx (&x)[4], const int gq) __attribute__((always_inline)) {
-#pragma unroll
-                for (int u = 0; u < 4; ++u) {
-                    const int p = (gq * 4 + u) * 4 + lk;
-                    x[u] = phi_l[xcol + (unsigned)(p < M ? p : M - 1) * xrow];
-                }
-            };
-            auto mf = [&](const cplx (&x)[4], const int gq) __attribute__((always_inline)) {
-                const bool last = gq == ng - 1;
-#pragma unroll
-                for (int u = 0; u < 4; ++u) {
-                    const bool dead = last && (gq * 4 + u) * 4 + lk >= M;
-                    if constexpr (YR) {
-                        const double y = dead ? 0.0 : yf[gq * 4 + u];
-                        accR = mfma16(x[u].x, y, accR);
-                        acc3 = mfma16(x[u].y, y, acc3);
-                    } else {
-                        const cplx y = dead ? cmake(0.0, 0.0) : yf[gq * 4 + u];
-                        accR = mfma16(x[u].x, y.x, accR);
-                        accI = mfma16(x[u].y, y.y, accI);
-                        acc3 = mfma16(x[u].x + x[u].y, y.x - y.y, acc3);
-                    }
-                }
-            };
-            readx(xa, 0);
-#pragma unroll
-            for (int gq = 0; gq < NG; gq += 2) {
-                if (gq < ng) {
-                    if (gq + 1 < ng) readx(xb, gq + 1);
-                    mf(xa, gq);
-                }
-                if (gq + 1 < ng) {
-                    if (gq + 2 < ng) readx(xa, gq + 2 < NG ? gq + 2 : 0);
-                    mf(xb, gq + 1);
-                }
-            }
-#pragma unroll
-            for (int r = 0; r < 4; ++r) {
-                const int i = ti * 16 + lk + 4 * r, j = tj * 16 + lr;
-                if (i < n && j < n) O[i * n + j] = YR ? cmake(accR[r], acc3[r]) : cmake(accR[r] + accI[r], acc3[r] - accR[r] + accI[r]);
-            }
-            if (WGJ) break;
-        }
-    };
-    if (yreal) phase01(std::true_type{});
-    else phase01(std::false_type{});
-    __syncthreads();
-    __shared__ cplx gj_row[2][32], gj_piv[2][32];
-    __shared__ int gj_prow[2][32];
-    if (WGJ) {
-        if (wave == g && !(closed && g == 1)) {
-            cplx ph;
-            int la;
-            gj_wave32(O, n, lane, INVERSE, gj_row[g], gj_piv[g], gj_prow[g], ph, la);
-            if (lane == 0) {
-                ph_s[g] = ph; la_s[g] = (double)la;
-                if (closed) { ph_s[1] = ph; la_s[1] = (double)la; }
-            }
-        }
-    } else if (wave == 0) {
-        cplx ph = cmake(1.0, 0.0);
-        int la = 0;
-        const int cw_shift = n <= 32 ? 5 : 6;
-        const int cj = lane & ((1 << cw_shift) - 1), ri = lane >> cw_shift, rstep = 64 >> cw_shift;
-        for (int k = 0; k < n; ++k) {
-            unsigned long long mbits = 0;
-            if (lane < n) {
-                const cplx v = O[lane * n + k];
-                colk[lane] = v;
-                if (lane >= k) {
-                    mbits = (unsigned long long)__double_as_longlong(fabs(v.x) + fabs(v.y));
-                    atomicMax(&pmax[k], mbits);
-                }
-            }
-            __builtin_amdgcn_wave_barrier();
-            const unsigned long long mx = pmax[k];
-            const unsigned long long hit = __ballot(lane >= k && lane < n && mbits == mx);
-            const int p = hit ? __ffsll((long long)hit) - 1 : k;
-            if (p != k) {
-                for (int j = lane; j < n; j += 64) {
-                    const cplx t = O[k * n + j];
-                    O[k * n + j] = O[p * n + j];
-                    O[p * n + j] = t;
-                }
-                if (lane == 0) { const cplx t = colk[k]; colk[k] = colk[p]; colk[p] = t; }
-            }
-            if (lane == 0) piv[k] = p;
-            __builtin_amdgcn_wave_barrier();
-            const cplx d = colk[k];
-            ph = cmul(ph, p != k ? cmake(-d.x, -d.y) : d);
-            {
-                int e;
-                (void)frexp(fmax(fabs(ph.x), fabs(ph.y)), &e);
-                ph = cmake(ldexp(ph.x, -e), ldexp(ph.y, -e));
-                la += e;
-            }
-            const double dn = 1.0 / (d.x * d.x + d.y * d.y);
-            const cplx dinv = cmake(d.x * dn, -d.y * dn);
-            for (int j = lane; j < n; j += 64) rowk[j] = cmul(O[k * n + j], dinv);
-            __builtin_amdgcn_wave_barrier();
-            if (n <= 32) {
-                if (cj < n && (INVERSE || cj > k)) {
-                    const cplx rk = rowk[cj];
-                    cplx v[16], f[16];
-#pragma unroll
-                    for (int t = 0; t < 16; ++t) {
-                        const int i = ri + 2 * t;
-                        if (i < n) { v[t] = O[i * n + cj]; f[t] = colk[i]; }
-                    }
-#pragma unroll
-                    for (int t = 0; t < 16; ++t) {
-                        const int i = ri + 2 * t;
-                        if (i < n && (INVERSE || i > k)) {
-                            cplx o;
-                            if (INVERSE && i == k) o = (cj == k) ? dinv : rk;
-                            else if (INVERSE && cj == k) { const cplx m = cmul(f[t], dinv); o = cmake(-m.x, -m.y); }
-                            else {
-                                o = v[t];
-                                o.x = fma(-f[t].x, rk.x, o.x); o.x = fma(f[t].y, rk.y, o.x);
-                                o.y = fma(-f[t].x, rk.y, o.y); o.y = fma(-f[t].y, rk.x, o.y);
-                            }
-                            O[i * n + cj] = o;
-                        }
-                    }
-                }
-            } else if (INVERSE) {
-                if (cj < n) {
-                    const cplx rk = rowk[cj];
-                    for (int i = ri; i < n; i += rstep) {
-                        cplx v;
-                        if (i == k) v = (cj == k) ? dinv : rk;
-                        else {
-                            const cplx f = colk[i];
-                            if (cj == k) { const cplx t = cmul(f, dinv); v = cmake(-t.x, -t.y); }
-                            else {
-                                v = O[i * n + cj];
-                                v.x = fma(-f.x, rk.x, v.x); v.x = fma(f.y, rk.y, v.x);
-                                v.y = fma(-f.x, rk.y, v.y); v.y = fma(-f.y, rk.x, v.y);
-                            }
-                        }
-                        O[i * n + cj] = v;
-                    }
-                }
-            } else {
-                if (cj < n && cj > k) {
-                    const cplx rk = rowk[cj];
-                    for (int i = k + 1 + ri; i < n; i += rstep) {
-                        const cplx f = colk[i];
-                        cplx v = O[i * n + cj];
-                        v.x = fma(-f.x, rk.x, v.x); v.x = fma(f.y, rk.y, v.x);
-                        v.y = fma(-f.x, rk.y, v.y); v.y = fma(-f.y, rk.x, v.y);
-                        O[i * n + cj] = v;
-                    }
-                }
-            }
-            __builtin_amdgcn_wave_barrier();
-        }
-        if (INVERSE) {
-            for (int k = n - 1; k >= 0; --k) {
-                const int p = piv[k];
-                if (p != k) {
-                    for (int i = lane; i < n; i += 64) {
-                        const cplx t = O[i * n + k];
-                        O[i * n + k] = O[i * n + p];
-                        O[i * n + p] = t;
-                    }
-                }
-                __builtin_amdgcn_wave_barrier();
-            }
-        }
-        if (lane == 0) { ph_s[g] = ph; la_s[g] = (double)la; }
-    }
-    __syncthreads();
-    if (tid == 448) {
-        const cplx p2 = cmul(ph_s[0], ph_s[1]);
-        const int e = (int)(la_s[0] + la_s[1]);
-        a.det[w] = cmake(ldexp(p2.x, e), ldexp(p2.y, e));
-        if (a.det_a) a.det_a[w] = cmake(ldexp(ph_s[0].x, (int)la_s[0]), ldexp(ph_s[0].y, (int)la_s[0]));
-        if (wa.weight) weight_update_and_cap(wa, w);
-    }
-    if (INVERSE && a.oinv) {
-        cplx *oo = a.oinv + ((long)w * 2 + g) * nmax * nmax;
-        for (int e = tid & 255; e < n * n; e += 256) oo[(e / n) * nmax + (e % n)] = O[e];
-    }
-    if (INVERSE && a.ghalf) {
-        const bool both = a.gsum != nullptr;
-        const int mt16 = (M + 15) >> 4, npair = (mt16 + 1) >> 1;
-        const int first = both ? __builtin_amdgcn_readfirstlane(tid >> 6) : wave, stride = both ? 8 : 4;
-        const int s_lo = both ? 0 : g, s_hi = both ? 2 : g + 1;
-        const int nn = both ? a.na : n, nt16x = (nn + 15) >> 4;
-        for (int it = first; nn > 0 && it < nt16x * npair; it += stride) {
-            const int ti = it % nt16x, tc0 = 2 * (it / nt16x), tc1 = tc0 + 1;
-            const bool two = tc1 < mt16;
-            const int c0 = tc0 * 16 + lr, c1 = tc1 * 16 + lr;
-            const int c0c = c0 < M ? c0 : M - 1, c1c = c1 < M ? c1 : M - 1;
-            d4_t sra = {0, 0, 0, 0}, sia = {0, 0, 0, 0}, srb = {0, 0, 0, 0}, sib = {0, 0, 0, 0};
-            for (int s = s_lo; s < (closed ? 1 : s_hi); ++s) {
-                const int ns = s ? a.nb : a.na, offs = s ? a.na : 0;
-                const cplx *Os = (const cplx *)smem + (long)s * (nmax * nmax + 2 * nmax);
-                cplx *gh = a.ghalf + ((long)w * nt + offs) * M;
-                const int nks3 = (ns + 3) >> 2;
-                const int ia = ti * 16 + lr, iac = ia < ns ? ia : ns - 1;
-                cplx xf[12];
-#pragma unroll
-                for (int ks = 0; ks < 12; ++ks) {
-                    const int j = ks * 4 + lk, jc = j < ns ? j : ns - 1;
-                    const cplx x = Os[iac * ns + jc];
-                    xf[ks] = (ks < nks3 && j < ns && ia < ns) ? x : cmake(0.0, 0.0);
-                }
-                d4_t p1a = {0, 0, 0, 0}, p2a = {0, 0, 0, 0}, p3a = {0, 0, 0, 0};
-                d4_t p1b = {0, 0, 0, 0}, p2b = {0, 0, 0, 0}, p3b = {0, 0, 0, 0};
-#pragma unroll
-                for (int ks = 0; ks < 12; ++ks) {
-                    if (ks < nks3) {
-                        const int j = ks * 4 + lk, jc = j < ns ? j : ns - 1;
-                        const cplx y0 = phi_l[c0c * nt + offs + jc], y1 = phi_l[c1c * nt + offs + jc];
-                        const cplx x = xf[ks];
-                        const double xs = x.x + x.y;
-                        p1a = mfma16(x.x, y0.x, p1a);
-                        p2a = mfma16(x.y, y0.y, p2a);
-                        p3a = mfma16(xs, y0.x + y0.y, p3a);
-                        if (two) {
-                            p1b = mfma16(x.x, y1.x, p1b);
-                            p2b = mfma16(x.y, y1.y, p2b);
-                            p3b = mfma16(xs, y1.x + y1.y, p3b);
-                        }
-                    }
-                }
-#pragma unroll
-                for (int r = 0; r < 4; ++r) {
-                    const int i = ti * 16 + lk + 4 * r;
-                    const double ra = p1a[r] - p2a[r], ima = p3a[r] - p1a[r] - p2a[r];
-                    const double rb = p1b[r] - p2b[r], imb = p3b[r] - p1b[r] - p2b[r];
-                    if (i < ns && c0 < M && !a.skip_spin) gh[(long)i * M + c0] = cmake(ra, ima);
-                    if (two && i < ns && c1 < M && !a.skip_spin) gh[(long)i * M + c1] = cmake(rb, imb);
-                    sra[r] += ra; sia[r] += ima; srb[r] += rb; sib[r] += imb;
-                    if (closed) {
-                        cplx *ghb = gh + (long)a.na * M;
-                        if (i < ns && c0 < M && !a.skip_spin) ghb[(long)i * M + c0] = cmake(ra, ima);
-                        if (two && i < ns && c1 < M && !a.skip_spin) ghb[(long)i * M + c1] = cmake(rb, imb);
-                        sra[r] += ra; sia[r] += ima; srb[r] += rb; sib[r] += imb;
-                    }
-                }
-            }
-            if (both) {
-                cplx *gs = a.gsum + (long)w * a.na * M;
-#pragma unroll
-                for (int r = 0; r < 4; ++r) {
-                    const int i = ti * 16 + lk + 4 * r;
-                    if (i < a.na && c0 < M) gs[(long)i * M + c0] = cmake(sra[r], sia[r]);
-                    if (two && i < a.na && c1 < M) gs[(long)i * M + c1] = cmake(srb[r], sib[r]);
-                }
-            }
-        }
-    }
-}
 
 template <bool INVERSE>
 __global__ __launch_bounds__(512) void greens_tiny_kernel(GreensArgs a, WeightArgs wa) {
@@ -666,6 +309,14 @@
     }
 }
 
+bool k_greens_wgj(afq_handle *h) {
+    const int nmax = h->na > h->nb ? h->na : h->nb;
+    const size_t lds_small = sizeof(cplx) * (2 * ((size_t)nmax * nmax + 2 * nmax) + ((2 * nmax + 3) / 4 + 1) + (size_t)h->M * h->nt);
+    const size_t lds_tiny = sizeof(cplx) * 2 * (size_t)h->M * h->nt;
+    const bool tiny = nmax <= 8 && h->nt >= 1 && lds_tiny <= 150 * 1024;
+    return !k_greens_big_supported(h) && nmax <= 32 && h->M <= 4 * GS_KSMAX && lds_small <= 160 * 1024 && !tiny;
+}
+
 static int launch_greens(afq_handle *h, cplx *ghalf, cplx *det, int only_alive, cplx *oinv = nullptr) {
     GreensArgs a;
     a.oinv = oinv; a.gsum = nullptr;
@@ -680,6 +331,12 @@
     a.skip_spin = 0;
     const int nmax = h->na > h->nb ? h->na : h->nb;
     if (nmax > 256) AFQ_FAIL(h, AFQ_EUNSUPPORTED, "more than 256 electrons per spin");
+    const bool take_prop = h->prop_deferred && ghalf && det == h->ovlp_new && !only_alive && !oinv && h->fuse_weight_req &&
+                           h->ndet <= 1 && k_greens_wgj(h);
+    if (h->prop_deferred && !take_prop) {
+        const int rc = k_prop_fused_deferred(h, nullptr, nullptr);
+        if (rc) return rc;
+    }
     if (k_greens_big_supported(h)) {
         if (h->fuse_weight_req && det == h->ovlp_new && !only_alive && !oinv && h->ndet <= 1) {
             const WeightArgs wa = weight_args(h, h->fuse_eshift);
@@ -717,16 +374,21 @@
                 a.closed_bad = h->closed_bad; a.closed_epoch = ++h->closed_epoch;
                 h->closed_checked_version = h->ghalf_version;
             }
-            KernelTrace kt(h, AFQ_K_GREENS);
-            if (tiny) {
-                AFQ_HIP(h, afq_raise_lds((const void *)greens_tiny_kernel<true>, lds_tiny, lds_set_tiny[0]));
-                AFQ_LAUNCH(h, (greens_tiny_kernel<true>), dim3(h->nw), dim3(512), lds_tiny, h->stream, a, wa);
-            } else if (wgj) {
-                AFQ_HIP(h, afq_raise_lds((const void *)greens_small_kernel<true, true>, lds, lds_set[0]));
-                AFQ_LAUNCH(h, (greens_small_kernel<true, true>), dim3(h->nw), dim3(512), lds, h->stream, a, wa);
+            if (take_prop) {
+                const int rc = k_prop_fused_deferred(h, &a, &wa);
+                if (rc) return rc;
             } else {
-                AFQ_HIP(h, afq_raise_lds((const void *)greens_small_kernel<true, false>, lds, lds_set[1]));
-                AFQ_LAUNCH(h, (greens_small_kernel<true, false>), dim3(h->nw), dim3(512), lds, h->stream, a, wa);
+                KernelTrace kt(h, AFQ_K_GREENS);
+                if (tiny) {
+                    AFQ_HIP(h, afq_raise_lds((const void *)greens_tiny_kernel<true>, lds_tiny, lds_set_tiny[0]));
+                    AFQ_LAUNCH(h, (greens_tiny_kernel<true>), dim3(h->nw), dim3(512), lds_tiny, h->stream, a, wa);
+                } else if (wgj) {
+                    AFQ_HIP(h, afq_raise_lds((const void *)greens_small_kernel<true, true>, lds, lds_set[0]));
+                    AFQ_LAUNCH(h, (greens_small_kernel<true, true>), dim3(h->nw), dim3(512), lds, h->stream, a, wa);
+                } else {
+                    AFQ_HIP(h, afq_raise_lds((const void *)greens_small_kernel<true, false>, lds, lds_set[1]));
+                    AFQ_LAUNCH(h, (greens_small_kernel<true, false>), dim3(h->nw), dim3(512), lds, h->stream, a, wa);
+                }
             }
             if (want_sum) h->gsum_version = h->ghalf_version;
         } else if (tiny) {
```

New measurement: 1.049 million walker-steps/s, median of 6. 1.4% higher.
